# haowenz/chromap

Measured on NVIDIA H100. Metric: paired-end reads mapped/sec (hg38-scale, 2x50bp), higher is better.
Workload: dtype u64

## Files before the change

chromap_b200/csrc/cta_pair_candidates.cuh:

```cuda
#pragma once
#include "pipeline_kernels.cuh"

__device__ __forceinline__ int cta_scan_add(int v, int *s_warp, int *total) {
  const int NT = blockDim.x;
  const int lane = threadIdx.x & 31, wid = threadIdx.x >> 5;
  int x = v;
#pragma unroll
  for (int o = 1; o < 32; o <<= 1) { const int y = __shfl_up_sync(0xffffffffu, x, o); if (lane >= o) x += y; }
  if (lane == 31) s_warp[wid] = x;
  __syncthreads();
  int base = 0, tot = 0;
for (int i = 0; i < (NT >> 5); ++i) { const int w = s_warp[i]; if (i < wid) base += w; tot += w; }
  __syncthreads();
  *total = tot;
  return base + x - v;
}
__device__ __forceinline__ int cta_scan_max(int v, int *s_warp, int *total) {
  const int NT = blockDim.x;
  const int lane = threadIdx.x & 31, wid = threadIdx.x >> 5;
  int x = v;
#pragma unroll
  for (int o = 1; o < 32; o <<= 1) { const int y = __shfl_up_sync(0xffffffffu, x, o); if (lane >= o) x = max(x, y); }
  if (lane == 31) s_warp[wid] = x;
  __syncthreads();
// ... 96 lines not shown
  for (int i = a0; i < a1; ++i) {
    const u8 f = f1[i];
    if (f == 1) run = max(run, (int)c1[i]);
    else if (f == 2) { if ((int)c1[i] >= run) ++nq1; else f1[i] = 0; }
  }
  int run2 = max(6, pm2), nq2 = 0;
  for (int j = b0; j < b1; ++j) {
    const u8 f = f2[j];
    if (f == 1) run2 = max(run2, (int)c2[j]);
    else if (f == 2) { if ((int)c2[j] >= run2) ++nq2; else f2[j] = 0; }
  }
  int totq;
  const int pq = cta_scan_add(nq1 | (nq2 << 16), s_warp, &totq);
  int paired_before = pp & 0xffff, qual_before = pq & 0xffff;
  for (int i = a0; i < a1; ++i) {
    const u8 f = f1[i];
    if (f == 1) { const int at = paired_before + min(qual_before, 5); o1p[at] = p1[i]; o1c[at] = c1[i]; ++paired_before; }
    else if (f == 2) { if (qual_before < 5) { const int at = paired_before + qual_before; o1p[at] = p1[i]; o1c[at] = c1[i]; } ++qual_before; }
  }
  paired_before = pp >> 16; qual_before = pq >> 16;
  for (int j = b0; j < b1; ++j) {
    const u8 f = f2[j];
    if (f == 1) { const int at = paired_before + min(qual_before, 5); o2p[at] = p2[j]; o2c[at] = c2[j]; ++paired_before; }
    else if (f == 2) { if (qual_before < 5) { const int at = paired_before + qual_before; o2p[at] = p2[j]; o2c[at] = c2[j]; } ++qual_before; }
  }
  *na = (tot & 0xffff) + min(totq & 0xffff, 5);
  *nb = (tot >> 16) + min(totq >> 16, 5);
  __syncthreads();
}

#define RESCUE_MAXWIN 300
#define PC_CTA_NT_MAX 512
struct RescueShared {
  u64 win_lo[RESCUE_MAXWIN], win_hi[RESCUE_MAXWIN];
  int i[8];
  int warp[PC_CTA_NT_MAX / 32];
};
__device__ inline int cta_rescue(const DevParams &P, const DevIndex &ix, int strand, u32 range, int n_mm, const u64 *mmv, const u32 *mmp,
                                 const u64 *mate_pos, const u8 *mate_cnt, int n_mate, u32 *rep_len, u64 *hits, int cap, u64 *sm, int sm_cap,
                                 RescueShared &R, int *nh_out) {
  const int NT = blockDim.x;
  const int tid = threadIdx.x, lane = tid & 31, wid = tid >> 5;
  int mx = 0;
  for (int i = tid; i < n_mate; i += NT) mx = max(mx, (int)mate_cnt[i]);
  int max_cnt;
  cta_scan_max(mx, R.warp, &max_cnt);
  int nb = 0;
  for (int i = tid; i < n_mate; i += NT) nb += mate_cnt[i] == max_cnt;
  int n_best;
  cta_scan_add(nb, R.warp, &n_best);
  *nh_out = 0;
  if (n_best >= 300 || n_mate > P.f0 || (max_cnt <= P.min_seeds && n_best >= 200)) return -max_cnt;
  if (tid == 0) {
    int nw = 0;
    for (int i = 0; i < n_mate; ++i) {
      if (mate_cnt[i] != max_cnt) continue;
      const u64 lo = mate_pos[i] < range ? 0 : mate_pos[i] - range, hi = mate_pos[i] + range;
      if (nw > 0 && !(R.win_hi[nw - 1] < lo)) R.win_hi[nw - 1] = hi;
      else { R.win_lo[nw] = lo; R.win_hi[nw] = hi; ++nw; }
    }
    R.i[2] = nw;
    R.i[3] = 0;
  }
  __syncthreads();
  const int nw = R.i[2];
  for (int mi = tid; mi < n_mm; mi += NT) {
    if ((mmp[mi] >> 30) != 1) continue;
    bool same;
    const u64 cp = hit_to_candidate(P.k, mmv[mi], (mmp[mi] & 0x3FFFFFFFu) >> 1, mmp[mi] & 1u, &same);
    if ((same && strand == 0) || (!same && strand == 1)) { const int at = atomicAdd(&R.i[3], 1); if (at < cap) hits[at] = cp; }
  }
  for (int mi = wid; mi < n_mm; mi += (NT >> 5)) {
    if ((mmp[mi] >> 30) != 2) continue;
    const u64 val = mmv[mi];
    const u64 *O = ix.occ + (u32)(val >> 32);
    const int n = (int)(u32)val;
    const u32 rpos = (mmp[mi] & 0x3FFFFFFFu) >> 1, rstrand = mmp[mi] & 1u;
    int c_lb = 0, c_e = 0, c_s = 0;
    for (int b0 = 0; b0 < nw; b0 += 32) {
      const int b = b0 + lane;
      const bool live = b < nw;
      int lb = 0, eq = 0, ub = 0;
      if (live) {
        const u64 lo = R.win_lo[b], hi = R.win_hi[b];
        int a = 0, z = n;
        while (a < z) { const int m = (a + z) >> 1; if ((__ldg(&O[m]) >> 1) < lo) a = m + 1; else z = m; }
        lb = a;
        eq = (lb < n && (__ldg(&O[lb]) >> 1) == lo) ? 1 : 0;
        int step = 1, lo_i = lb + eq, hi_i = lb + eq;
        while (hi_i < n && (__ldg(&O[hi_i]) >> 1) <= hi) { lo_i = hi_i + 1; hi_i += step; step <<= 1; }
        if (hi_i > n) hi_i = n;
        while (lo_i < hi_i) { const int m = (lo_i + hi_i) >> 1; if ((__ldg(&O[m]) >> 1) <= hi) lo_i = m + 1; else hi_i = m; }
        ub = lo_i;
      }
      int p_lb = __shfl_up_sync(0xffffffffu, lb, 1), p_e = __shfl_up_sync(0xffffffffu, eq, 1);
      if (lane == 0) { p_lb = c_lb; p_e = c_e; }
      u32 f = 2u;
      if (live) {
        int o0, o1;
        if (b == 0) o0 = o1 = rescue_replay(0, n, lb, lb + eq);
        else {
          o1 = rescue_replay(p_lb, n, lb, lb + eq);
          o0 = p_e ? o1 : rescue_replay(max(p_lb - 1, 0), n, lb, lb + eq);
        }
        f = (o0 == lb ? 1u : 0u) | (o1 == lb ? 2u : 0u);
      }
#pragma unroll
      for (int o = 1; o < 32; o <<= 1) {
        const u32 g = __shfl_up_sync(0xffffffffu, f, o);
        if (lane >= o) f = (((f >> (g & 1u)) & 1u)) | (((f >> ((g >> 1) & 1u)) & 1u) << 1);
      }
      const int s_out = (int)((f >> c_s) & 1u);
      if (live) {
        const int first = lb - 1 + s_out, end = max(first, ub);
        for (int oi = first; oi < end; ++oi) {
          bool same;
          const u64 cp = hit_to_candidate(P.k, __ldg(&O[oi]), rpos, rstrand, &same);
          if ((same && strand == 0) || (!same && strand == 1)) { const int at = atomicAdd(&R.i[3], 1); if (at < cap) hits[at] = cp; }
        }
      }
      c_lb = __shfl_sync(0xffffffffu, lb, 31); c_e = __shfl_sync(0xffffffffu, eq, 31); c_s = __shfl_sync(0xffffffffu, s_out, 31);
    }
  }
  __syncthreads();
  const int nh = R.i[3];
  *nh_out = nh;
  if (tid == 0) {
    RepStats st = {0u, 0xFFFFFFFFu, 0};
    for (int mi = 0; mi < n_mm; ++mi)
      if ((mmp[mi] >> 30) == 2 && (u32)mmv[mi] >= (u32)P.f0) rep_update(P.k, P.w, (mmp[mi] & 0x3FFFFFFFu) >> 1, st);
    *rep_len = st.len;
  }
  __syncthreads();
  if (nh <= cap) cta_sort_keys(hits, nh, sm, sm_cap);
  return max_cnt;
}

__host__ __device__ inline size_t pair_candidates_cta_smem(int sm_cap, int lcap, int maxmm, int fcap) {
  return (size_t)sm_cap * 11 + (size_t)lcap * 4 * 9 + (size_t)maxmm * 12 + (size_t)fcap * 2 + 64;
}
__device__ inline void pair_candidates_cta_pair(const DevParams &P, const DevIndex &ix, const Scratch &S, Counters *ctr, int sm_cap, int lcap, int fcap,
                                                int slot, u64 *sm, RescueShared &RS) {
  const Caps c = S.caps;
  u8 *aux = (u8 *)(sm + sm_cap);
  u64 *s_lp = (u64 *)(aux + 3 * (size_t)sm_cap);
  u64 *s_mmv = s_lp + 4 * (size_t)lcap;
  u32 *s_mmp = (u32 *)(s_mmv + c.maxmm);
  u8 *s_lc = (u8 *)(s_mmp + c.maxmm);
  u8 *fl_a = s_lc + 4 * (size_t)lcap, *fl_b = fl_a + fcap;
  const int NT = blockDim.x, tid = threadIdx.x;
  PairMeta &pm = S.pmeta[slot];
  if (pm.status != ST_OK) return;
  ReadMeta *rm = S.rmeta + 2 * slot;
  auto CP = [&](int mate, int set, int strand) { return S.cand_pos + ((((size_t)(2 * slot + mate)) * 3 + set) * 2 + strand) * c.cc; };
  auto CC = [&](int mate, int set, int strand) { return S.cand_cnt + ((((size_t)(2 * slot + mate)) * 3 + set) * 2 + strand) * c.cc; };
  if (P.se) {
    const int a1 = rm[0].n_cand[0] + rm[0].n_cand[1];
    __syncthreads();
    if (tid == 0) { if (rm[0].n_mm == 0 || a1 == 0) pm.status = ST_DROP; else atomicAdd(&ctr->n_candidates, (u64)a1); }
    return;
  }
  if (rm[0].n_mm == 0 || rm[1].n_mm == 0) { __syncthreads(); if (tid == 0) pm.status = ST_DROP; return; }
  if (P.split) {
    const int a1 = rm[0].n_cand[0] + rm[0].n_cand[1], a2 = rm[1].n_cand[0] + rm[1].n_cand[1];
    __syncthreads();
    if (tid == 0) { if (!(a1 > 0 && a2 > 0)) pm.status = ST_DROP; else atomicAdd(&ctr->n_candidates, (u64)(a1 + a2)); }
    return;
  }
  int nq[4];
  const u64 *lp[4];
  const u8 *lc[4];
  const int n_mm2[2] = {rm[0].n_mm, rm[1].n_mm};
  auto stage = [&]() {
#pragma unroll
    for (int q = 0; q < 4; ++q) {
      nq[q] = rm[q >> 1].n_cand[q & 1];
      const u64 *gp = CP(q >> 1, 0, q & 1);
      const u8 *gc = CC(q >> 1, 0, q & 1);
      if (nq[q] <= lcap) {
        for (int i = tid; i < nq[q]; i += NT) { s_lp[q * lcap + i] = gp[i]; s_lc[q * lcap + i] = gc[i]; }
        lp[q] = s_lp + q * lcap; lc[q] = s_lc + q * lcap;
      } else { lp[q] = gp; lc[q] = gc; }
    }
    __syncthreads();
  };
  stage();
  bool need[2];
#pragma unroll
  for (int mate = 0; mate < 2; ++mate) {
    const u32 half = (u32)n_mm2[mate] / 2;
    int hit = 0;
#pragma unroll
    for (int s = 0; s < 2; ++s)
      for (int i = tid; i < nq[mate * 2 + s]; i += NT) hit |= lc[mate * 2 + s][i] >= half;
    need[mate] = !__syncthreads_or(hit);
  }
  const u32 range = 2u * (u32)P.max_insert;
  int ret = 0;
  for (int mate = 0; mate < 2; ++mate) {
    if (!need[mate]) continue;
    ReadMeta &me = rm[mate];
    const int n_mm = n_mm2[mate];
    const size_t sr = 2 * slot + mate;
    {
      const size_t mb0 = mm_base(S, slot, mate);
      const int ms = mm_stride(S);
      for (int i = tid; i < n_mm; i += NT) { s_mmv[i] = S.mm_val[mb0 + (size_t)i * ms]; s_mmp[i] = S.mm_pos[mb0 + (size_t)i * ms]; }
    }
    __syncthreads();
    u64 *hp = S.hits + (sr * 2 + 0) * c.hc, *hn = S.hits + (sr * 2 + 1) * c.hc;
    int pr = 0, nr = 0;
    bool ovf = false;
    const int o0 = (1 - mate) * 2;
    if (nq[o0] > 0) {
      int nh;
      pr = cta_rescue(P, ix, 1, range, n_mm, s_mmv, s_mmp, lp[o0], lc[o0], nq[o0], &me.rep_len, hn, c.hc, sm, sm_cap, RS, &nh);
      if (nh > c.hc) ovf = true;
      else {
        const int na = cta_cluster_par(P.e, 1, (u32)n_mm, hn, nh, CP(mate, 2, 1), CC(mate, 2, 1), c.cc, sm, sm_cap, aux, &RS.i[4]);
        if (na > c.cc) ovf = true; else if (tid == 0) me.n_aug[1] = na;
      }
    }
    if (!ovf && nq[o0 + 1] > 0) {
      int nh;
      nr = cta_rescue(P, ix, 0, range, n_mm, s_mmv, s_mmp, lp[o0 + 1], lc[o0 + 1], nq[o0 + 1], &me.rep_len, hp, c.hc, sm, sm_cap, RS, &nh);
      if (nh > c.hc) ovf = true;
      else {
        const int na = cta_cluster_par(P.e, 1, (u32)n_mm, hp, nh, CP(mate, 2, 0), CC(mate, 2, 0), c.cc, sm, sm_cap, aux, &RS.i[4]);
        if (na > c.cc) ovf = true; else if (tid == 0) me.n_aug[0] = na;
      }
    }
    if (ovf) { __syncthreads(); if (tid == 0) pm.status = ST_OVERFLOW; return; }
    if (((pr < 0 && nr > 0 && -pr >= nr) || (pr > 0 && nr < 0 && pr <= -nr)) && nq[mate * 2] + nq[mate * 2 + 1] == 0) ret = 1;
    __syncthreads();
  }
  bool merged = false;
  for (int q = 0; q < 4; ++q) {
    const int mate = q >> 1, s = q & 1;
    if (!need[mate]) continue;
    const int n2 = rm[mate].n_aug[s];
    if (n2 <= 0) continue;
    const int m = nq[q] + n2;
    u64 *mp;
    u8 *mc, *kf;
    if (m <= sm_cap) { mp = sm; mc = aux; kf = aux + sm_cap; }
    else { mp = CP(mate, 1, 0); mc = CC(mate, 1, 0); kf = fl_a; }
    const int n = (m > 2 * c.cc || (m > sm_cap && m > fcap)) ? c.cc + 1
                                                             : cta_merge_cands(P.e, lp[q], lc[q], nq[q], CP(mate, 2, s), CC(mate, 2, s), n2, mp, mc, kf,
                                                                               CP(mate, 0, s), CC(mate, 0, s), c.cc, RS.warp);
    if (n > c.cc) { __syncthreads(); if (tid == 0) pm.status = ST_OVERFLOW; return; }
    if (tid == 0) rm[mate].n_cand[s] = n;
    merged = true;
  }
  if (merged) { __syncthreads(); stage(); }
  int nc1 = nq[0] + nq[1], nc2 = nq[2] + nq[3];
  if (nc1 > 0 && nc2 > 0) {
#pragma unroll
    for (int q = 0; q < 4; ++q)
      if (nq[q] > lcap) {
        u64 *dst = CP(q >> 1, 1, q & 1);
        u8 *dstc = CC(q >> 1, 1, q & 1);
        for (int i = tid; i < nq[q]; i += NT) { dst[i] = lp[q][i]; dstc[i] = lc[q][i]; }
        lp[q] = dst; lc[q] = dstc;
      }
    __syncthreads();
    int a, b, a2, b2;
    cta_pe_filter((u32)P.max_insert, lp[0], lc[0], nq[0], lp[3], lc[3], nq[3], CP(0, 0, 0), CC(0, 0, 0), &a, CP(1, 0, 1), CC(1, 0, 1), &b, fl_a, fl_b, RS.warp);
    cta_pe_filter((u32)P.max_insert, lp[1], lc[1], nq[1], lp[2], lc[2], nq[2], CP(0, 0, 1), CC(0, 0, 1), &a2, CP(1, 0, 0), CC(1, 0, 0), &b2, fl_a, fl_b, RS.warp);
    if (tid == 0) {
      rm[0].n_cand[0] = a; rm[1].n_cand[1] = b; rm[0].n_cand[1] = a2; rm[1].n_cand[0] = b2;
    }
    nc1 = a + a2; nc2 = b + b2;
  }
  if (tid != 0) return;
  pm.sup = ret;
  if (!(nc1 > 0 && nc2 > 0)) { pm.status = ST_DROP; return; }
  atomicAdd(&ctr->n_candidates, (u64)(nc1 + nc2));
}

__global__ void __launch_bounds__(PC_CTA_NT_MAX) pair_candidates_cta_kernel(DevParams P, DevIndex ix, Scratch S, Counters *ctr, int sm_cap, int lcap, int fcap,
                                                                     const int *list, const int *list_count) {
  extern __shared__ u64 sm[];
  __shared__ RescueShared RS;
  if (!list) { pair_candidates_cta_pair(P, ix, S, ctr, sm_cap, lcap, fcap, (int)blockIdx.x, sm, RS); return; }
  const int n = *list_count;
  for (int b = blockIdx.x; b < n; b += gridDim.x) {
    pair_candidates_cta_pair(P, ix, S, ctr, sm_cap, lcap, fcap, list[b], sm, RS);
    __syncthreads();
  }
}
```

chromap_b200/csrc/cta_verify_pairing.cuh:

```cuda
#pragma once
#include "cta_pair_candidates.cuh"

__device__ __forceinline__ Tally tally_merge(const Tally &a, const Tally &b, int sentinel) {
  Tally r;
  r.min_err = min(a.min_err, b.min_err);
  r.n_best = (a.min_err == r.min_err ? a.n_best : 0) + (b.min_err == r.min_err ? b.n_best : 0);
  int s = sentinel;
  if (a.min_err > r.min_err && a.n_best > 0) s = min(s, a.min_err);
  if (b.min_err > r.min_err && b.n_best > 0) s = min(s, b.min_err);
  if (a.n_second_best > 0) s = min(s, a.second_min_err);
  if (b.n_second_best > 0) s = min(s, b.second_min_err);
  r.second_min_err = s;
  int n = 0;
  if (a.min_err == s && a.min_err > r.min_err) n += a.n_best;
  if (b.min_err == s && b.min_err > r.min_err) n += b.n_best;
  if (a.second_min_err == s) n += a.n_second_best;
  if (b.second_min_err == s) n += b.n_second_best;
  r.n_second_best = n;
  return r;
}
__device__ __forceinline__ Tally cta_tally_reduce(Tally t, int sentinel, Tally *s_t ) {
#pragma unroll
  for (int o = 16; o > 0; o >>= 1) {
    Tally u;
    u.min_err = __shfl_down_sync(0xffffffffu, t.min_err, o); u.second_min_err = __shfl_down_sync(0xffffffffu, t.second_min_err, o);
    u.n_best = __shfl_down_sync(0xffffffffu, t.n_best, o); u.n_second_best = __shfl_down_sync(0xffffffffu, t.n_second_best, o);
    t = tally_merge(t, u, sentinel);
  }
  if ((threadIdx.x & 31) == 0) s_t[threadIdx.x >> 5] = t;
  __syncthreads();
  Tally r = s_t[0];
  for (int i = 1; i < (int)(blockDim.x >> 5); ++i) r = tally_merge(r, s_t[i], sentinel);
  __syncthreads();
  return r;
}

#define VERIFY_NT_MAX 256
__global__ void __launch_bounds__(VERIFY_NT_MAX) verify_cta_kernel(DevParams P, DevRef R, DevBatch B, Scratch S, Counters *ctr, int sm_cap) {
  extern __shared__ u64 smk[];
  u8 *smt = (u8 *)(smk + sm_cap);
  u8 *s_fwd = smt + sm_cap, *s_neg = s_fwd + S.caps.maxmm;
  __shared__ int s_i[8];
  __shared__ int s_warp[VERIFY_NT_MAX / 32];
  __shared__ Tally s_t[VERIFY_NT_MAX / 32];
  const int NT = blockDim.x;
  const int sr = blockIdx.x, tid = threadIdx.x;
  const int slot = sr >> 1, mate = sr & 1;
  if (tid == 0) s_i[0] = S.pmeta[slot].status;
  __syncthreads();
  if (s_i[0] != ST_OK || (P.se && mate == 1)) return;
  const int pair = slot_pair(S, slot);
  ReadMeta &rm = S.rmeta[sr];
  const Caps c = S.caps;
  const u8 *read = read_ptr(B, pair, mate);
  const int L = rm.len, e = P.e;
  u64 *mp[2] = {S.map_pos + ((size_t)sr * 2 + 0) * c.mc, S.map_pos + ((size_t)sr * 2 + 1) * c.mc};
  short *me[2] = {S.map_err + ((size_t)sr * 2 + 0) * c.mc, S.map_err + ((size_t)sr * 2 + 1) * c.mc};
  u64 *cp[2] = {S.cand_pos + (((size_t)sr * 3 + 0) * 2 + 0) * c.cc, S.cand_pos + (((size_t)sr * 3 + 0) * 2 + 1) * c.cc};
  u8 *cc[2] = {S.cand_cnt + (((size_t)sr * 3 + 0) * 2 + 0) * c.cc, S.cand_cnt + (((size_t)sr * 3 + 0) * 2 + 1) * c.cc};
  const int nc[2] = {rm.n_cand[0], rm.n_cand[1]};
  if (nc[0] + nc[1] == 1) {
    const int strand = nc[0] == 1 ? 0 : 1;
    if (cc[strand][0] == rm.n_mm) {
      const u64 cpos = cp[strand][0];
      const u32 rid = (u32)(cpos >> 32);
      const u32 pos = strand == 0 ? (u32)cpos : (u32)cpos - (u32)L + 1u;
      const bool ok = valid_cand(e, R.len[rid], pos, (u32)L);
      __syncthreads();
      if (tid == 0) {
        rm.min_err = 0; rm.n_best = 1; rm.second_min_err = e + 1; rm.n_second_best = 0;
        if (ok) {
          mp[strand][0] = strand == 0 ? cpos + (u64)L - 1 : cpos;
          me[strand][0] = 0;
          rm.n_map[strand] = 1; rm.n_map[1 - strand] = 0;
        }
      }
      if (ok) return;
    }
  }
  for (int i = tid; i < L; i += NT) {
    const u32 b = base_code(read[i]);
    s_fwd[i] = (u8)b;
    s_neg[L - 1 - i] = (u8)(b < 4 ? 3u ^ b : 4u);
  }
  auto cless = [](u64 pa, u8 ca, u64 pb, u8 cb) { return ca != cb ? ca > cb : pa < pb; };
  cta_sort_pairs<u8>(cp[0], cc[0], nc[0], ~0ull, (u8)0, cless, smk, smt, sm_cap);
  cta_sort_pairs<u8>(cp[1], cc[1], nc[1], ~0ull, (u8)0, cless, smk, smt, sm_cap);
  unsigned short *vlist = (unsigned short *)smk;
  Tally t = {e + 1, e + 1, 0, 0};
  if (tid == 0 && nc[0] + nc[1] == 1 && cc[nc[0] == 1 ? 0 : 1][0] == rm.n_mm) { t.min_err = 0; t.n_best = 1; }
  u32 n_ver = 0;
  int nm[2] = {0, 0};
  for (int s = 0; s < 2; ++s) {
    const int n = nc[s];
    if (n == 0) continue;
    const int C = (n + NT - 1) / NT;
    const int r0 = min(n, tid * C), r1 = min(n, r0 + C);
    int mine = 0;
    for (int i = r0; i < r1; ++i) {
      const u64 cpos = cp[s][i];
      const u32 pos = s == 0 ? (u32)cpos : (u32)cpos - (u32)L + 1u;
      mine += valid_cand(e, R.len[(u32)(cpos >> 32)], pos, (u32)L) ? 1 : 0;
    }
    int nv;
    int at = cta_scan_add(mine, s_warp, &nv);
    for (int i = r0; i < r1; ++i) {
      const u64 cpos = cp[s][i];
      const u32 pos = s == 0 ? (u32)cpos : (u32)cpos - (u32)L + 1u;
      if (valid_cand(e, R.len[(u32)(cpos >> 32)], pos, (u32)L)) vlist[at++] = (unsigned short)i;
    }
    __syncthreads();
    const bool ruled = n >= P.lanes;
    const int n_full = nv / P.lanes * P.lanes;
    int stop = n;
    int free_until = 0;
    int out_base = 0;
    for (int v0 = 0; v0 < nv; v0 += NT) {
      if ((int)vlist[v0] >= stop && v0 >= free_until) break;
      const int v = v0 + tid;
      int err = e + 1, endp = 0, idx = 0;
      u64 cpos = 0;
      if (v + NT < nv) {
        const u64 nx = cp[s][vlist[v + NT]];
        const u32 npos = s == 0 ? (u32)nx : (u32)nx - (u32)L + 1u;
        prefetch_span(R.seq + R.off[(u32)(nx >> 32)] + npos - e, L + 2 * e);
      }
      if (v < nv) {
        idx = vlist[v];
        if (idx < stop || v < free_until) {
          cpos = cp[s][idx];
          const u32 rid = (u32)(cpos >> 32);
          const u32 pos = s == 0 ? (u32)cpos : (u32)cpos - (u32)L + 1u;
          const u8 *win = R.seq + R.off[rid] + pos - e;
          prefetch_span(win, L + 2 * e);
          const u8 *txt = s == 0 ? s_fwd : s_neg;
          err = banded_align(e, L, [&](int q) { return base_code(__ldg(win + q)); }, [&](int q) { return (u32)txt[q]; }, &endp);
          ++n_ver;
        } else idx = -1;
      } else idx = -1;
      if (ruled && stop == n && free_until == 0) {
        const bool failing = idx >= 0 && v < n_full && err > e;
        const unsigned fm = __ballot_sync(0xffffffffu, failing);
        if ((tid & 31) == 0) s_warp[tid >> 5] = (int)fm;
        __syncthreads();
        int first_fail = -1;
#pragma unroll
        for (int w = 0; w < (NT >> 5); ++w) if (first_fail < 0 && s_warp[w]) first_fail = v0 + w * 32 + __ffs((unsigned)s_warp[w]) - 1;
        if (first_fail >= 0) {
          const int g0 = first_fail / P.lanes * P.lanes, g1 = g0 + P.lanes;
          int last_fail = first_fail;
          for (int q = g0; q < g1; ++q) { const int w = (q - v0) >> 5, b = (q - v0) & 31; if ((s_warp[w] >> b) & 1) last_fail = q; }
          const int T = cc[s][vlist[last_fail]];
          int lo = (int)vlist[g1 - 1] + 1, hi = n;
          while (lo < hi) { const int m = (lo + hi) >> 1; if ((int)cc[s][m] < T) hi = m; else lo = m + 1; }
          stop = lo;
          free_until = g1;
        }
        __syncthreads();
      }
      const bool taken = idx >= 0 && (idx < stop || v < free_until);
      const bool pass = taken && err <= e;
      int tot;
      const int o = out_base + cta_scan_add(pass ? 1 : 0, s_warp, &tot);
      if (pass) {
        tally(t, err);
        if (o < c.mc) {
          mp[s][o] = s == 0 ? cpos - (u64)e + (u64)endp : cpos - (u64)L + 1 - (u64)e + (u64)endp;
          me[s][o] = (short)err;
        }
      }
      out_base += tot;
    }
    nm[s] = out_base;
    __syncthreads();
  }
  const Tally tt = cta_tally_reduce(t, e + 1, s_t);
  if (n_ver) agg_add(&ctr->n_verified, (u64)n_ver);
  if (tid != 0) return;
  if (nm[0] > c.mc || nm[1] > c.mc) { S.pmeta[slot].status = ST_OVERFLOW; return; }
  rm.n_map[0] = nm[0]; rm.n_map[1] = nm[1];
  rm.min_err = tt.min_err; rm.second_min_err = tt.second_min_err; rm.n_best = tt.n_best; rm.n_second_best = tt.n_second_best;
}

struct SweepWindow {
  u64 ins, ovl;
  u32 L1, L2;
  int s1;
  __device__ __forceinline__ bool before(u64 p1, u64 p2) const { return (s1 == 1 && p1 > p2 + ins - L2) || (s1 == 0 && p1 > p2 + L1 - ovl); }
  __device__ __forceinline__ bool within(u64 p1, u64 p2) const { return (s1 == 0 && p2 <= p1 + ins - L1) || (s1 == 1 && p2 <= p1 + L2 - ovl); }
  __device__ __forceinline__ void range(u64 p1, const u64 *p2, int n2, int *lo, int *hi) const {
    int a = 0, b = n2;
    while (a < b) { const int m = (a + b) >> 1; if (before(p1, p2[m])) a = m + 1; else b = m; }
    *lo = a;
    b = n2;
    while (a < b) { const int m = (a + b) >> 1; if (within(p1, p2[m])) a = m + 1; else b = m; }
    *hi = a;
  }
};

__global__ void __launch_bounds__(CTA_NT) pairing_cta_kernel(DevParams P, Scratch S, int *pair_nbest, int sm_cap) {
  extern __shared__ u64 smk[];
  short *smt = (short *)(smk + sm_cap);
  __shared__ Tally s_t[CTA_NT / 32];
  const int slot = blockIdx.x, tid = threadIdx.x;
  PairMeta &pm = S.pmeta[slot];
  const int pair = slot_pair(S, slot);
  if (pm.status != ST_OK) { if (tid == 0 && pm.status == ST_DROP) pair_nbest[pair] = 0; return; }
  const Caps c = S.caps;
  ReadMeta *rm = S.rmeta + 2 * slot;
  if (P.se) {
    __syncthreads();
    if (tid == 0) {
      if (rm[0].n_map[0] + rm[0].n_map[1] == 0) { pm.status = ST_DROP; pair_nbest[pair] = 0; }
      else {
        pm.min_sum = rm[0].min_err; pm.second_min_sum = rm[0].second_min_err; pm.n_best = rm[0].n_best; pm.n_second_best = rm[0].n_second_best;
        pair_nbest[pair] = rm[0].n_best;
      }
    }
    return;
  }
  if (rm[0].n_map[0] + rm[0].n_map[1] == 0 || rm[1].n_map[0] + rm[1].n_map[1] == 0) {
    __syncthreads();
    if (tid == 0) { pm.status = ST_DROP; pair_nbest[pair] = 0; }
    return;
  }
  auto mless = [](u64 pa, short ea, u64 pb, short eb) { return pa != pb ? pa < pb : ea < eb; };
  u64 *mp[2][2];
  short *me[2][2];
  for (int m = 0; m < 2; ++m)
    for (int s = 0; s < 2; ++s) {
      mp[m][s] = S.map_pos + ((size_t)(2 * slot + m) * 2 + s) * c.mc;
      me[m][s] = S.map_err + ((size_t)(2 * slot + m) * 2 + s) * c.mc;
      cta_sort_pairs<short>(mp[m][s], me[m][s], rm[m].n_map[s], ~0ull, (short)32767, mless, smk, smt, sm_cap);
    }
  const int sentinel = 2 * P.e + 1;
  Tally t = {sentinel, sentinel, 0, 0};
  SweepWindow W;
  W.ins = (u64)P.max_insert; W.ovl = (u64)(u32)P.min_read_len; W.L1 = (u32)rm[0].len; W.L2 = (u32)rm[1].len;
  for (int dir = 0; dir < 2; ++dir) {
    W.s1 = dir;
    const u64 *p1 = mp[0][dir], *p2 = mp[1][1 - dir];
    const short *e1 = me[0][dir], *e2 = me[1][1 - dir];
    const int n1 = rm[0].n_map[dir], n2 = rm[1].n_map[1 - dir];
    for (int i1 = tid; i1 < n1; i1 += CTA_NT) {
      int lo, hi;
      W.range(p1[i1], p2, n2, &lo, &hi);
      const int ea = e1[i1];
      for (int j = lo; j < hi; ++j) tally(t, ea + (int)e2[j]);
    }
  }
  const Tally tt = cta_tally_reduce(t, sentinel, s_t);
  if (tid != 0) return;
  pm.min_sum = tt.min_err; pm.second_min_sum = tt.second_min_err; pm.n_best = tt.n_best; pm.n_second_best = tt.n_second_best;
  pair_nbest[pair] = (tt.n_best > P.drop_rep) ? 0 : tt.n_best;
}

__global__ void __launch_bounds__(CTA_NT) emit_cta_kernel(DevParams P, DevRef R, DevBatch B, MapqTables T, Scratch S, const int *pair_sel, OutRecord *out,
                                                          int *out_n, Counters *ctr) {
  __shared__ int s_warp[CTA_NT / 32];
  __shared__ int s_i1[CMX_MAX_BEST], s_j[CMX_MAX_BEST], s_sel[CMX_MAX_BEST];
  const int slot = blockIdx.x, tid = threadIdx.x;
  PairMeta &pm = S.pmeta[slot];
  const int pair = slot_pair(S, slot);
  if (pm.status == ST_OVERFLOW) return;
  if (pm.status != ST_OK || pm.n_best > P.drop_rep || pm.n_best == 0) { if (tid == 0) out_n[pair] = 0; return; }
  const Caps c = S.caps;
  const ReadMeta *rm = S.rmeta + 2 * slot;
  const int mb = P.max_best;
  const int to_report = mb < pm.n_best ? mb : pm.n_best;
  if (tid < to_report) s_sel[tid] = pair_sel[(size_t)pair * mb + tid];
  __syncthreads();
  const int min_sum = pm.min_sum;
  SweepWindow W;
  W.ins = (u64)P.max_insert; W.ovl = (u64)(u32)P.min_read_len; W.L1 = (u32)rm[0].len; W.L2 = (u32)rm[1].len;
  int base = 0;
  for (int dir = 0; dir < 2; ++dir) {
    if (base > s_sel[to_report - 1]) break;
    W.s1 = dir;
    const u64 *p1 = S.map_pos + ((size_t)(2 * slot + 0) * 2 + dir) * c.mc, *p2 = S.map_pos + ((size_t)(2 * slot + 1) * 2 + (1 - dir)) * c.mc;
    const short *e1 = S.map_err + ((size_t)(2 * slot + 0) * 2 + dir) * c.mc, *e2 = S.map_err + ((size_t)(2 * slot + 1) * 2 + (1 - dir)) * c.mc;
    const int n1 = rm[0].n_map[dir], n2 = rm[1].n_map[1 - dir];
    const int C = (n1 + CTA_NT - 1) / CTA_NT;
    const int r0 = min(n1, tid * C), r1 = min(n1, r0 + C);
    int mine = 0;
    for (int i1 = r0; i1 < r1; ++i1) {
      int lo, hi;
      W.range(p1[i1], p2, n2, &lo, &hi);
      const int want = min_sum - (int)e1[i1];
      for (int j = lo; j < hi; ++j) mine += (int)e2[j] == want;
    }
    int total;
    int idx = base + cta_scan_add(mine, s_warp, &total);
    if (mine > 0) {
      int r = 0;
      while (r < to_report && s_sel[r] < idx) ++r;
      if (r < to_report && s_sel[r] < idx + mine) {
        for (int i1 = r0; i1 < r1 && r < to_report; ++i1) {
          int lo, hi;
          W.range(p1[i1], p2, n2, &lo, &hi);
          const int want = min_sum - (int)e1[i1];
          for (int j = lo; j < hi && r < to_report; ++j) {
            if ((int)e2[j] != want) continue;
            if (idx == s_sel[r]) { s_i1[r] = i1 | (dir << 30); s_j[r] = j; ++r; }
            ++idx;
          }
        }
      }
    }
    base += total;
  }
  __syncthreads();
  if (tid < to_report) {
    const int s1 = s_i1[tid] >> 30, i1 = s_i1[tid] & 0x3FFFFFFF, j = s_j[tid];
    const size_t b1 = ((size_t)(2 * slot + 0) * 2 + s1) * c.mc + i1, b2 = ((size_t)(2 * slot + 1) * 2 + (1 - s1)) * c.mc + j;
    out[(size_t)pair * mb + tid] = pe_record(P, R, B, T, pm, rm, pair, s1, S.map_pos[b1], S.map_err[b1], S.map_pos[b2], S.map_err[b2]);
  }
  if (tid != 0) return;
  out_n[pair] = to_report;
  pm.n_rec = to_report;
  atomicAdd(&ctr->n_mapped, 1ull);
  if (pm.n_best == 1) atomicAdd(&ctr->n_unique, 1ull);
}
```

chromap_b200/csrc/device_common.cuh:

```cuda
#pragma once
#include <cuda_runtime.h>
#include <stdint.h>

typedef unsigned long long u64;
typedef unsigned int u32;
typedef unsigned char u8;

#define CMX_W_MAX 64
#define CMX_MAX_BEST 8

struct DevParams {
  int e, min_seeds, f0, f1, max_best, max_insert, min_read_len, drop_rep, trim, k, w, lanes, split;
  int se;
};

struct Caps {
  int maxmm, hc, cc, mc;
};

enum { ST_OK = 0, ST_DROP = 1, ST_OVERFLOW = 2 };

struct ReadMeta {
  int len;
  int n_mm;
  int n_cand[2];
  int n_cand_gen[2];
  u32 rep_len;
  int mm_done;
  int n_map[2];
  int min_err, second_min_err, n_best, n_second_best;
  int n_aug[2];
};
static_assert(sizeof(ReadMeta) == 64, "ReadMeta: two sectors");

struct PairMeta {
  int status;
  int sup;
  int min_sum, second_min_sum, n_best, n_second_best;
  int n_rec;
  int pad;
};

struct DevIndex {
  const ulonglong2 *slots;
  u64 n_slots_mask;
  int shift;
  const u64 *occ;
  u32 n_occ;
  int k, w;
};
#define CMX_EMPTY_KEY 0xFFFFFFFFFFFFFFFFull

struct DevRef {
  const u8 *seq;
  const u64 *off;
  const u32 *len;
  u32 n_seq;
};

struct DevBatch {
  const u8 *seq1;
  const u32 *off1;
  const u8 *seq2;
  const u32 *off2;
  u32 n_pairs;
  u32 first_read_id;
  const u8 *bc_ok;
};

struct Scratch {
  Caps caps;
  int n_slots;
  const int *pair_list;
  int mm_il;
  ReadMeta *rmeta;
  PairMeta *pmeta;
  u64 *mm_hash;
  u64 *mm_val;
  u32 *mm_pos;
  u64 *hits;
  u64 *cand_pos;
  u8 *cand_cnt;
  u64 *map_pos;
  short *map_err;
  int *map_split;
};

#define SCRATCH_ARRAYS 11
inline size_t scratch_layout(const Caps &c, size_t slots, bool interleaved, size_t *off, size_t *size = nullptr) {
  const size_t R = 2 * slots;
  const size_t Rm = interleaved ? 2 * ((slots + 31) / 32 * 32) : R;
  const size_t sz[SCRATCH_ARRAYS] = {R * sizeof(ReadMeta), slots * sizeof(PairMeta),
                                     interleaved ? 0 : R * c.maxmm * 8,
                                     Rm * c.maxmm * 8, Rm * c.maxmm * 4, R * 2 * (size_t)c.hc * 8, R * 6 * (size_t)c.cc * 8, R * 6 * (size_t)c.cc,
                                     R * 2 * (size_t)c.mc * 8, R * 2 * (size_t)c.mc * 2, R * 2 * (size_t)c.mc * 4};
  size_t end = 0;
  for (int i = 0; i < SCRATCH_ARRAYS; ++i) {
    off[i] = end;
    if (size) size[i] = sz[i];
    end = (end + sz[i] + 255) / 256 * 256;
  }
  return end;
}
inline void scratch_bind(Scratch &S, char *const *a) {
  S.rmeta = (ReadMeta *)a[0]; S.pmeta = (PairMeta *)a[1];
  S.mm_hash = (u64 *)a[2]; S.mm_val = (u64 *)a[3]; S.mm_pos = (u32 *)a[4];
  S.hits = (u64 *)a[5]; S.cand_pos = (u64 *)a[6]; S.cand_cnt = (u8 *)a[7];
  S.map_pos = (u64 *)a[8]; S.map_err = (short *)a[9]; S.map_split = (int *)a[10];
}

__device__ __forceinline__ int slot_pair(const Scratch &S, int slot) { return S.pair_list ? S.pair_list[slot] : slot; }

__device__ __forceinline__ u32 base_code(u8 c) {
  const u32 u = (u32)c & 0xDFu;
  const u32 x = (u >> 1) & 3u;
  const u32 code = x ^ (x >> 1);
  const u32 in_row = ((u & 0xE0u) == 0x40u) ? 1u : 0u;
  const u32 is_base = in_row & ((0x0010008Au >> (u & 31u)) & 1u);
  return is_base ? code : 4u;
}

__device__ __forceinline__ u64 mix64(u64 key, u64 mask) {
  key = (~key + (key << 21)) & mask;
  key = key ^ key >> 24;
  key = ((key + (key << 3)) + (key << 8)) & mask;
  key = key ^ key >> 14;
  key = ((key + (key << 2)) + (key << 4)) & mask;
  key = key ^ key >> 28;
  key = (key + (key << 31)) & mask;
  return key;
}

__device__ __forceinline__ int index_lookup(const DevIndex &ix, u64 mm_hash, u64 *val, int *steps) {
  u64 s = (mm_hash * 0x9E3779B97F4A7C15ull) >> ix.shift;
  int n = 0;
  for (;;) {
    const ulonglong2 kv = __ldg(&ix.slots[s]);
    ++n;
    if (kv.x == CMX_EMPTY_KEY) { *steps = n; return 0; }
    if ((kv.x >> 1) == mm_hash) { *val = kv.y; *steps = n; return (kv.x & 1) ? 1 : 2; }
    s = (s + 1) & ix.n_slots_mask;
  }
}

__device__ __forceinline__ void prefetch_span(const void *p, int bytes) {
  const char *a = (const char *)((unsigned long long)p & ~127ull), *z = (const char *)p + bytes;
  for (; a < z; a += 128) asm volatile("prefetch.global.L1 [%0];" ::"l"(a));
}

__device__ __forceinline__ void prefetch_l2(const void *p) { asm volatile("prefetch.global.L2 [%0];" ::"l"(p)); }

__device__ __forceinline__ int occ_lower_bound(const u64 *O, int n, u64 lo) {
  int a = 0, z = n;
  while (z - a > 8) {
    const int q = (z - a) >> 2, m1 = a + q, m2 = m1 + q, m3 = m2 + q;
    const u64 v1 = __ldg(&O[m1]) >> 1, v2 = __ldg(&O[m2]) >> 1, v3 = __ldg(&O[m3]) >> 1;
    if (v3 < lo) a = m3 + 1;
    else if (v2 < lo) { a = m2 + 1; z = m3; }
    else if (v1 < lo) { a = m1 + 1; z = m2; }
    else z = m1;
  }
  int below = 0;
#pragma unroll
  for (int i = 0; i < 8; ++i) below += (a + i < z && (__ldg(&O[a + i]) >> 1) < lo) ? 1 : 0;
  return a + below;
}
__device__ __forceinline__ int rescue_replay(int l, int n, int lb, int ue) {
  int mid = 0, r = n - 1;
  while (l <= r) {
    mid = (l + r) / 2;
    if (mid < lb) l = mid + 1;
    else if (mid >= ue) r = mid - 1;
    else break;
  }
  return mid;
}

__device__ __forceinline__ u64 hit_to_candidate(int k, u64 ref_hit, u32 read_pos, u32 read_strand, bool *same) {
  const u32 rp = (u32)(ref_hit >> 1);
  const bool sm = ((u32)(ref_hit & 1)) == read_strand;
  const u32 start = sm ? rp - read_pos : rp + read_pos - (u32)k + 1u;
  *same = sm;
  return ((ref_hit >> 33) << 32) | start;
}

struct StridedU64 {
  u64 *base;
  int stride;
  __device__ __forceinline__ u64 &operator[](int i) const { return base[i * stride]; }
};

template <typename A>
__device__ inline void sort_u64(A a, int n) {
  if (n <= 24) {
    for (int i = 1; i < n; ++i) {
      const u64 v = a[i];
      int j = i - 1;
      while (j >= 0 && a[j] > v) { a[j + 1] = a[j]; --j; }
      a[j + 1] = v;
    }
    return;
  }
  for (int start = n / 2 - 1; start >= 0; --start) {
    int root = start;
    const u64 v = a[root];
    for (;;) {
      int child = 2 * root + 1;
      if (child >= n) break;
      if (child + 1 < n && a[child] < a[child + 1]) ++child;
      if (a[child] <= v) break;
      a[root] = a[child];
      root = child;
    }
    a[root] = v;
  }
  for (int end = n - 1; end > 0; --end) {
    const u64 v = a[end];
    a[end] = a[0];
    int root = 0;
    for (;;) {
      int child = 2 * root + 1;
      if (child >= end) break;
      if (child + 1 < end && a[child] < a[child + 1]) ++child;
      if (a[child] <= v) break;
      a[root] = a[child];
      root = child;
    }
    a[root] = v;
  }
}

template <typename T, typename Less>
__device__ inline void sort_pairs(u64 *k, T *t, int n, Less less) {
  if (n <= 24) {
    for (int i = 1; i < n; ++i) {
      const u64 kv = k[i];
      const T tv = t[i];
      int j = i - 1;
      while (j >= 0 && less(kv, tv, k[j], t[j])) { k[j + 1] = k[j]; t[j + 1] = t[j]; --j; }
      k[j + 1] = kv; t[j + 1] = tv;
    }
    return;
  }
  auto sift = [&](int root, int end, u64 kv, T tv) {
    for (;;) {
      int child = 2 * root + 1;
      if (child >= end) break;
      if (child + 1 < end && less(k[child], t[child], k[child + 1], t[child + 1])) ++child;
      if (!less(kv, tv, k[child], t[child])) break;
      k[root] = k[child]; t[root] = t[child];
      root = child;
    }
    k[root] = kv; t[root] = tv;
  };
  for (int start = n / 2 - 1; start >= 0; --start) sift(start, n, k[start], t[start]);
  for (int end = n - 1; end > 0; --end) {
    const u64 kv = k[end];
    const T tv = t[end];
    k[end] = k[0]; t[end] = t[0];
    sift(0, end, kv, tv);
  }
}
```

chromap_b200/csrc/minimizers.cuh:

```cuda
#pragma once
#include "device_common.cuh"

template <int K>
__device__ __forceinline__ u64 mix64_k(u64 key) {
  static_assert(K >= 17 && K <= 23, "mix64_k: 2k - 14 must not exceed 32");
  constexpr u64 mask = (((u64)1) << (2 * K)) - 1;
  constexpr u32 mask_hi = (u32)(mask >> 32);
  u32 lo = (u32)key, hi = (u32)(key >> 32);
  auto mul = [&](u32 c, u64 add) {
    const u64 p = (u64)lo * c + add;
    hi = ((u32)(p >> 32) + hi * c) & mask_hi;
    lo = (u32)p;
  };
  mul((1u << 21) - 1u, mask);
  lo ^= __funnelshift_r(lo, hi, 24);
  mul(265u, 0);
  lo ^= __funnelshift_r(lo, hi, 14);
  mul(21u, 0);
  lo ^= __funnelshift_r(lo, hi, 28);
  mul((1u << 31) + 1u, 0);
  return ((u64)hi << 32) | lo;
}

template <int KS, int WS, typename SeqF, typename EmitF>
// ... 66 lines not shown
#pragma unroll
      for (int j = 0; j < WS; ++j)
        if (base + j < len) step(base + j, j);
    }
  } else {
    int slot = 0;
    for (int pos = 0; pos < len; ++pos)
      if (step(pos, slot)) { if (++slot == w) slot = 0; }
  }
  if (best_h != ~0ull) EMIT(best_h, best_p);
}
template <int K, int W, typename SeqF, typename EmitF, typename RingT>
__device__ __forceinline__ void minimizer_scan_packed(SeqF SEQ, int len, EmitF EMIT, RingT ring) {
  static_assert((K & 1) && K >= 17 && K <= 21 && W >= 2, "minimizer_scan_packed: odd k, 2k + 20 <= 62");
  constexpr u64 mask = (((u64)1) << (2 * K)) - 1;
  constexpr int shift = 2 * (K - 1);
  constexpr u64 NONE = ~0ull;
  constexpr u32 PM = 0xFFFFFu;
  u64 fwd = 0, rev = 0;
#pragma unroll
  for (int i = 0; i < W; ++i) ring[i] = NONE;
  u64 best = NONE;
  int run = 0, slot = 0;
  auto emit_key = [&](u64 key) { EMIT(key >> 20, PM - ((u32)key & PM)); };
#pragma unroll 1
  for (int pos = 0; pos < len; ++pos) {
    const u32 b = base_code(SEQ(pos));
    u64 cur = NONE;
    if (b < 4) {
      fwd = ((fwd << 2) | b) & mask;
      rev = (rev >> 2) | (((u64)(3 ^ b)) << shift);
      ++run;
      if (run >= K) {
        const u64 hf = mix64_k<K>(fwd), hr = mix64_k<K>(rev);
        const u32 strand = hf < hr ? 0u : 1u;
        cur = (mix64_k<K>(strand ? hr : hf) << 20) | (u64)(PM - (((u32)pos << 1) | strand));
      }
    } else {
      run = 0;
    }
    if (run == W + K - 1 && best != NONE && (best >> 20) < (cur >> 20)) {
      for (int j = 1; j < W; ++j) {
        int q = slot + j; if (q >= W) q -= W;
        const u64 x = ring[q];
        if ((x >> 20) == (best >> 20) && x != best) emit_key(x);
      }
    }
    const u64 old = ring[slot];
    ring[slot] = cur;
    u64 m = cur;
#pragma unroll
    for (int q = 0; q < W; ++q) m = min(m, (u64)ring[q]);
    u64 out = NONE;
    bool left = false;
    if (cur <= best) {
      if (run >= W + K && best != NONE) out = best;
    } else if (old == best) {
      if (run >= W + K - 1) { out = best; left = m != NONE; }
    }
    if (out != NONE) emit_key(out);
    int same_hi = 0;
    if (left) {
#pragma unroll
      for (int q = 0; q < W; ++q) same_hi += (u32)((u64)ring[q] >> 32) == (u32)(m >> 32);
    }
    if (same_hi > 1) {
      for (int j = 1; j <= W; ++j) {
        int q = slot + j; if (q >= W) q -= W;
        const u64 x = ring[q];
        if ((x >> 20) == (m >> 20) && x != m) emit_key(x);
      }
    }
    best = m;
    if (++slot == W) slot = 0;
  }
  if (best != NONE) emit_key(best);
}
template <int K, int W, typename SeqF, typename EmitF>
__device__ __forceinline__ void minimizer_scan_packed(SeqF SEQ, int len, EmitF EMIT) {
  static_assert((K & 1) && K >= 17 && K <= 21 && W >= 2, "minimizer_scan_packed: odd k, 2k + 20 <= 62");
  constexpr u64 mask = (((u64)1) << (2 * K)) - 1;
  constexpr int shift = 2 * (K - 1);
  constexpr u64 NONE = ~0ull;
  constexpr u32 PM = 0xFFFFFu;
  u64 fwd = 0, rev = 0;
  u64 ring[W];
#pragma unroll
  for (int i = 0; i < W; ++i) ring[i] = NONE;
  u64 best = NONE;
  int run = 0;
  auto emit_key = [&](u64 key) { EMIT(key >> 20, PM - ((u32)key & PM)); };
#pragma unroll 1
  for (int pos = 0; pos < len; ++pos) {
    const u32 b = base_code(SEQ(pos));
    u64 cur = NONE;
    if (b < 4) {
      fwd = ((fwd << 2) | b) & mask;
      rev = (rev >> 2) | (((u64)(3 ^ b)) << shift);
      ++run;
      if (run >= K) {
        const u64 hf = mix64_k<K>(fwd), hr = mix64_k<K>(rev);
        const u32 strand = hf < hr ? 0u : 1u;
        cur = (mix64_k<K>(strand ? hr : hf) << 20) | (u64)(PM - (((u32)pos << 1) | strand));
      }
    } else {
      run = 0;
    }
    if (run == W + K - 1) {
      if (best != NONE && (best >> 20) < (cur >> 20)) {
#pragma unroll
        for (int q = 1; q < W; ++q) {
          const u64 x = ring[q];
          if ((x >> 20) == (best >> 20) && x != best) emit_key(x);
        }
      }
    }
    const u64 old = ring[0];
#pragma unroll
    for (int q = 0; q + 1 < W; ++q) ring[q] = ring[q + 1];
    ring[W - 1] = cur;
    u64 m = ring[0];
#pragma unroll
    for (int q = 1; q < W; ++q) m = min(m, ring[q]);
    u64 out = NONE;
    bool left = false;
    if (cur <= best) {
      if (run >= W + K && best != NONE) out = best;
    } else if (old == best) {
      if (run >= W + K - 1) { out = best; left = m != NONE; }
    }
    if (out != NONE) emit_key(out);
    int same_hi = 0;
    if (left) {
#pragma unroll
      for (int q = 0; q < W; ++q) same_hi += (u32)(ring[q] >> 32) == (u32)(m >> 32);
    }
    if (same_hi > 1) {
#pragma unroll
      for (int q = 0; q < W; ++q) {
        const u64 x = ring[q];
        if ((x >> 20) == (m >> 20) && x != m) emit_key(x);
      }
    }
    best = m;
  }
  if (best != NONE) emit_key(best);
}

template <typename SeqF, typename EmitF>
__device__ __forceinline__ void minimizer_scan_any(SeqF SEQ, int len, int k, int w, EmitF EMIT) {
  if (k == 17 && w == 7 && len < (1 << 18)) minimizer_scan_packed<17, 7>(SEQ, len, EMIT);
  else minimizer_scan<0, 0>(SEQ, len, k, w, EMIT);
}

__device__ __forceinline__ size_t mm_base(const Scratch &S, int slot, int mate) {
  return S.mm_il ? ((size_t)((slot >> 5) * 2 + mate) * S.caps.maxmm) * 32 + (slot & 31) : (size_t)(2 * slot + mate) * S.caps.maxmm;
}
__device__ __forceinline__ int mm_stride(const Scratch &S) { return S.mm_il ? 32 : 1; }
```

chromap_b200/csrc/pipeline_kernels.cuh:

```cuda
#pragma once
#include "device_common.cuh"
#include "minimizers.cuh"

struct MapqTables {
  const double *inv_log;
  const int *pen_thr;
};
inline void mapq_tables_fill(double *inv_log, int *pen_thr) {
  const int coef_frac = log(50);
  inv_log[0] = inv_log[1] = 0.0;
  for (int a = 2; a < 65536; ++a) inv_log[a] = coef_frac / log((unsigned short)a);
  for (int v = 0; v < 96; ++v) {
    long long lo = 0, hi = 0x7ffffffeLL;
    auto pen = [](long long n) { return (int)(4.343 * log((double)(n + 1)) + 0.499); };
    if (pen(hi) < v) { pen_thr[v] = 0x7fffffff; continue; }
    while (lo < hi) { const long long mid = (lo + hi) / 2; if (pen(mid) >= v) hi = mid; else lo = mid + 1; }
    pen_thr[v] = (int)lo;
  }
}

struct Counters {
  u64 n_minimizers, n_probe_steps, n_found, n_occ_reads, n_verified, n_candidates, n_mapped, n_unique, n_overflow;
  u64 n_bc_in_whitelist, n_bc_corrected;
  u64 ovf_reason[8];
};

__device__ __forceinline__ const u8 *read_ptr(const DevBatch &B, int pair, int mate) {
  return mate == 0 ? B.seq1 + B.off1[pair] : B.seq2 + B.off2[pair];
}
__device__ __forceinline__ int read_raw_len(const DevBatch &B, int pair, int mate) {
  return mate == 0 ? (int)(B.off1[pair + 1] - B.off1[pair]) : (int)(B.off2[pair + 1] - B.off2[pair]);
}
__device__ __forceinline__ u32 neg_code(const u8 *read, int L, int i) {
  const u32 c = base_code(read[L - 1 - i]);
  return c < 4 ? 3u ^ c : 4u;
}
__device__ __forceinline__ u8 code_char(u32 c) { return c == 0 ? 'A' : c == 1 ? 'C' : c == 2 ? 'G' : c == 3 ? 'T' : 'N'; }

#ifndef CMX_HOST_EMU
__device__ __forceinline__ void agg_add(u64 *addr, u64 v) {
  const unsigned m = __activemask();
  const unsigned s_ = __reduce_add_sync(m, (unsigned)v);
  if ((int)(threadIdx.x & 31) == __ffs(m) - 1) atomicAdd(addr, (u64)s_);
}
__device__ __forceinline__ int agg_append(int *count) {
  const unsigned m = __activemask();
  const int lane = threadIdx.x & 31, leader = __ffs(m) - 1;
  int base = 0;
  if (lane == leader) base = atomicAdd(count, __popc(m));
  base = __shfl_sync(m, base, leader);
  return base + __popc(m & ((1u << lane) - 1u));
}
#endif

__global__ void prep_kernel(DevParams P, DevBatch B, Scratch S) {
  const int slot = blockIdx.x * blockDim.x + threadIdx.x;
  if (slot >= S.n_slots) return;
  const int pair = slot_pair(S, slot);
  PairMeta pm;
  pm.status = ST_OK; pm.sup = 0; pm.min_sum = 0; pm.second_min_sum = 0; pm.n_best = 0; pm.n_second_best = 0; pm.n_rec = 0; pm.pad = 0;
  int len1 = read_raw_len(B, pair, 0), len2 = P.se ? 0 : read_raw_len(B, pair, 1);
  if (B.bc_ok && !B.bc_ok[pair]) pm.status = ST_DROP;
  else if (len1 < P.min_read_len || (!P.se && len2 < P.min_read_len)) pm.status = ST_DROP;
  else if (len1 > S.caps.maxmm || len2 > S.caps.maxmm) pm.status = ST_OVERFLOW;
  else if (P.trim && !P.se) {
    const u8 *raw1 = read_ptr(B, pair, 0), *raw2 = read_ptr(B, pair, 1);
    const bool swp = !(len1 <= len2);
    const u8 *r1 = swp ? raw2 : raw1;
    const u8 *r2 = swp ? raw1 : raw2;
    const int L1 = swp ? len2 : len1, L2 = swp ? len1 : len2;
    const int min_ovl = P.min_read_len, seed = min_ovl / 2;
    bool merged = false;
    for (int si = 0; si < 2 && !merged; ++si) {
      for (int sp = 0; sp + seed <= L2 && !merged; ++sp) {
        bool hit = true;
        for (int j = 0; j < seed; ++j)
          if (code_char(neg_code(r2, L2, sp + j)) != r1[si * seed + j]) { hit = false; break; }
        if (!hit) continue;
        if (!(sp >= si * seed) || !((int)(L2 - sp + seed * si) >= min_ovl)) continue;
        bool ok = true;
        int ne = 0;
        for (int i = 0; i < seed * si; ++i) {
          if (code_char(neg_code(r2, L2, sp - si * seed + i)) != r1[i]) ++ne;
          if (ne > 1) { ok = false; break; }
        }
        if (ok)
          for (int i = seed; i + sp < L2 && si * seed + i < L1; ++i) {
            if (code_char(neg_code(r2, L2, sp + i)) != r1[si * seed + i]) ++ne;
            if (ne > 1) { ok = false; break; }
          }
        if (!ok) continue;
        int ovl = L2 - sp + si * seed, off2 = 0;
        if (ovl > L1) { off2 = ovl - L1; ovl = L1; }
        const int t1 = swp ? ovl + off2 : ovl, t2 = swp ? ovl : ovl + off2;
        if (t1 < len1) len1 = t1;
        if (t2 < len2) len2 = t2;
        merged = true;
      }
    }
  }
  S.pmeta[slot] = pm;
  ReadMeta z;
  memset(&z, 0, sizeof(z));
  z.len = len1; S.rmeta[2 * slot] = z;
  z.len = len2; S.rmeta[2 * slot + 1] = z;
}

struct RepStats { u32 len, prev; int count; };
__device__ __forceinline__ void rep_update(int k, int w, u32 read_pos, RepStats &st) {
  if (st.prev > read_pos) st.len += k;
  else if (read_pos < st.prev + k + w - 1) st.len += read_pos - st.prev;
  else st.len += k;
  st.prev = read_pos;
  ++st.count;
}

template <typename A>
__device__ inline int cluster_hits(int e, int need, u32 n_mm, A hits, int nh, u64 *cpos, u8 *ccnt, int cap) {
  if (nh == 0) return 0;
  int n = 0, mcount = 1, eq = 1, best_eq = 1;
  u64 prev = hits[0], best = hits[0];
  u32 prev_rid = (u32)(prev >> 32), prev_pos = (u32)prev;
  for (int i = 1; i <= nh; ++i) {
    const u64 h = i < nh ? hits[i] : ~0ull;
    const u32 rid = (u32)(h >> 32), pos = (u32)h;
    if (rid != prev_rid || pos > prev_pos + (u32)e || ((u32)mcount >= n_mm && pos > (u32)best + (u32)e)) {
      if (mcount >= need) { if (n < cap) { cpos[n] = best; ccnt[n] = (u8)best_eq; } ++n; }
      mcount = 1; eq = 1; best_eq = 1; best = h;
    } else {
      if (h == best) { ++eq; ++best_eq; }
      else if (h == prev) { ++eq; if (eq > best_eq) { best = prev; best_eq = eq; } }
      else eq = 1;
      ++mcount;
    }
    prev = h; prev_rid = rid; prev_pos = pos;
  }
  return n;
}

#define CLUSTER_NT 128
__global__ void __launch_bounds__(CLUSTER_NT) cluster_kernel(DevParams P, DevIndex ix, Scratch S, Counters *ctr, int mode, int rows, int *list,
                                                             int *list_count) {
  extern __shared__ u64 sh_hits[];
  const int tid = blockIdx.x * CLUSTER_NT + threadIdx.x;
  int sr = tid;
  if (mode == 1) {
    if (tid >= *list_count) return;
    sr = list[tid];
  } else if (sr >= 2 * S.n_slots) return;
  const int slot = sr >> 1;
  if (S.pmeta[slot].status != ST_OK) return;
  ReadMeta &rm = S.rmeta[sr];
  const Caps c = S.caps;
  const int n_mm = rm.n_mm;
  if (n_mm == 0) return;
  const int ms = mm_stride(S);
  const u64 *mmv = S.mm_val + mm_base(S, slot, sr & 1);
  const u32 *mmp = S.mm_pos + mm_base(S, slot, sr & 1);
  long long cnt1 = 0, cnt2 = 0;
  RepStats st = {0u, 0xFFFFFFFFu, 0};
  for (int i = 0; i < n_mm; ++i) {
    const u32 kind = mmp[(size_t)i * ms] >> 30;
    if (kind == 1) { ++cnt1; ++cnt2; }
    else if (kind == 2) {
      const u64 v_ = mmv[(size_t)i * ms];
      const u32 n = (u32)v_;
      if (n < (u32)P.f1) prefetch_span(&ix.occ[(u32)(v_ >> 32)], (int)min(n, 64u) * 8);
      if (n < (u32)P.f0) cnt1 += n;
      if (n < (u32)P.f1) cnt2 += n;
      if (n >= (u32)P.f0) rep_update(P.k, P.w, (mmp[(size_t)i * ms] & 0x3FFFFFFFu) >> 1, st);
    }
  }
  const bool round2 = cnt1 == 0;
  const long long total = round2 ? cnt2 : cnt1;
  if (total > c.hc) { S.pmeta[slot].status = ST_OVERFLOW; atomicAdd(&ctr->ovf_reason[2], 1ull); return; }
  if (total > rows) { list[agg_append(list_count)] = sr; return; }
  const u32 max_freq = round2 ? (u32)P.f1 : (u32)P.f0;
  const StridedU64 hp = {sh_hits + threadIdx.x, CLUSTER_NT};
  const StridedU64 hn = {sh_hits + (size_t)(rows - 1) * CLUSTER_NT + threadIdx.x, -CLUSTER_NT};
  int np = 0, nn = 0;
  u32 occ_reads = 0;
  for (int i = 0; i < n_mm; ++i) {
    const u32 kind = mmp[(size_t)i * ms] >> 30;
    if (kind == 0) continue;
    const u32 rpos = (mmp[(size_t)i * ms] & 0x3FFFFFFFu) >> 1, rstrand = mmp[(size_t)i * ms] & 1u;
    const u64 val = mmv[(size_t)i * ms];
    bool same;
    if (kind == 1) {
      const u64 cp = hit_to_candidate(P.k, val, rpos, rstrand, &same);
      if (same) hp[np++] = cp; else hn[nn++] = cp;
      continue;
    }
    const u32 n = (u32)val, off = (u32)(val >> 32);
    if (n < max_freq) {
      for (u32 q = 0; q < n; ++q) {
        const u64 rh = __ldg(&ix.occ[off + q]);
        const u64 cp = hit_to_candidate(P.k, rh, rpos, rstrand, &same);
        if (same) hp[np++] = cp; else hn[nn++] = cp;
      }
      occ_reads += n;
    }
  }
  if (occ_reads) agg_add(&ctr->n_occ_reads, (u64)occ_reads);
  sort_u64(hp, np);
  sort_u64(hn, nn);
  rm.rep_len = st.len;
  int need = n_mm - st.count;
  need = need > 1 ? need : 1;
  need = need > P.min_seeds ? P.min_seeds : need;
  if (round2 && np > 0 && nn > 0) need = P.min_seeds;
  u64 *cp0 = S.cand_pos + (((size_t)sr * 3 + 0) * 2 + 0) * c.cc, *cp1 = cp0 + c.cc;
  u8 *cc0 = S.cand_cnt + (((size_t)sr * 3 + 0) * 2 + 0) * c.cc, *cc1 = cc0 + c.cc;
  const int nc0 = cluster_hits(P.e, need, (u32)n_mm, hp, np, cp0, cc0, c.cc);
  const int nc1 = cluster_hits(P.e, need, (u32)n_mm, hn, nn, cp1, cc1, c.cc);
  if (nc0 > c.cc || nc1 > c.cc) { S.pmeta[slot].status = ST_OVERFLOW; atomicAdd(&ctr->ovf_reason[3], 1ull); return; }
  rm.n_cand[0] = nc0; rm.n_cand[1] = nc1;
  rm.n_cand_gen[0] = nc0; rm.n_cand_gen[1] = nc1;
}

__device__ inline int rescue_hits(const DevParams &P, const DevIndex &ix, int strand, u32 range, int n_mm, const u64 *mmv,
                                  const u32 *mmp, int ms, const u64 *mate_pos, const u8 *mate_cnt, int n_mate, u32 *rep_len,
                                  u64 *hits, int cap, int *nh_out) {
  int max_cnt = 0, n_best = 0;
  for (int i = 0; i < n_mate; ++i) {
    const int cnt = mate_cnt[i];
    if (cnt > max_cnt) { max_cnt = cnt; n_best = 1; }
    else if (cnt == max_cnt) ++n_best;
  }
  *nh_out = 0;
  if (n_best >= 300 || n_mate > P.f0 || (max_cnt <= P.min_seeds && n_best >= 200)) return -max_cnt;
  int nh = 0;
  RepStats st = {0u, 0xFFFFFFFFu, 0};
  for (int mi = 0; mi < n_mm; ++mi) {
    const u32 kind = mmp[(size_t)mi * ms] >> 30;
    if (kind == 0) continue;
    const u32 rpos = (mmp[(size_t)mi * ms] & 0x3FFFFFFFu) >> 1, rstrand = mmp[(size_t)mi * ms] & 1u;
    const u64 val = mmv[(size_t)mi * ms];
    bool same;
    if (kind == 1) {
      const u64 cp = hit_to_candidate(P.k, val, rpos, rstrand, &same);
      if ((same && strand == 0) || (!same && strand == 1)) { if (nh < cap) hits[nh] = cp; ++nh; }
      continue;
    }
    const u32 off = (u32)(val >> 32), n = (u32)val;
    int prev_l = 0;
    int ci = 0;
    while (ci < n_mate) {
      while (ci < n_mate && mate_cnt[ci] != max_cnt) ++ci;
      if (ci >= n_mate) break;
      u64 lo = mate_pos[ci] < range ? 0 : mate_pos[ci] - range;
      u64 hi = mate_pos[ci] + range;
      ++ci;
      for (;;) {
        int cj = ci;
        while (cj < n_mate && mate_cnt[cj] != max_cnt) ++cj;
        if (cj >= n_mate) { ci = cj; break; }
        const u64 lo2 = mate_pos[cj] < range ? 0 : mate_pos[cj] - range;
        if (hi < lo2) { ci = cj; break; }
        hi = mate_pos[cj] + range;
        ci = cj + 1;
      }
      const int lbq = occ_lower_bound(ix.occ + off, (int)n, lo);
      const int eqq = (lbq < (int)n && (__ldg(&ix.occ[off + lbq]) >> 1) == lo) ? 1 : 0;
      const int mid = rescue_replay(prev_l, (int)n, lbq, lbq + eqq);
      prev_l = mid;
      for (u32 oi = (u32)mid; oi < n; ++oi) {
        const u64 rh = __ldg(&ix.occ[off + oi]);
        if ((rh >> 1) > hi) break;
        const u64 cp = hit_to_candidate(P.k, rh, rpos, rstrand, &same);
        if ((same && strand == 0) || (!same && strand == 1)) { if (nh < cap) hits[nh] = cp; ++nh; }
      }
    }
    if (n >= (u32)P.f0) rep_update(P.k, P.w, rpos, st);
  }
  *nh_out = nh;
  if (nh <= cap) sort_u64(hits, nh);
  *rep_len = st.len;
  return max_cnt;
}

__device__ inline int merge_cands(int e, u64 *p1, u8 *c1, int n1, const u64 *p2, const u8 *c2, int n2, u64 *po, u8 *co, int cap) {
  if (n1 == 0) {
    for (int i = 0; i < n2 && i < cap; ++i) { p1[i] = p2[i]; c1[i] = c2[i]; }
    return n2;
  }
  int i = 0, j = 0, n = 0;
  u64 last = 0;
#define FAR(p) (n == 0 || (p) > last + (u64)e)
#define PUSH(p, c) do { if (n < cap) { po[n] = (p); co[n] = (c); } last = (p); ++n; } while (0)
  while (i < n1 && j < n2) {
    if (p1[i] == p2[j]) { if (FAR(p1[i])) { if (c1[i] > c2[j]) PUSH(p1[i], c1[i]); else PUSH(p2[j], c2[j]); } ++i; ++j; }
    else if (p1[i] < p2[j]) { if (FAR(p1[i])) PUSH(p1[i], c1[i]); ++i; }
    else { if (FAR(p2[j])) PUSH(p2[j], c2[j]); ++j; }
  }
  for (; i < n1; ++i) if (FAR(p1[i])) PUSH(p1[i], c1[i]);
  for (; j < n2; ++j) if (FAR(p2[j])) PUSH(p2[j], c2[j]);
#undef FAR
#undef PUSH
  for (int t = 0; t < n && t < cap; ++t) { p1[t] = po[t]; c1[t] = co[t]; }
  return n;
}

__device__ inline void pe_filter_dir(u32 dist, const u64 *p1, const u8 *c1, int n1, const u64 *p2, const u8 *c2, int n2,
                                     u64 *f1p, u8 *f1c, int *nf1, u64 *f2p, u8 *f2c, int *nf2) {
  int i1 = 0, i2 = 0, prev_end = 0, a = 0, b = 0;
  int un1 = 0, un2 = 0, max1 = 6, max2 = 6;
  while (i1 < n1 && i2 < n2) {
    if (p1[i1] > p2[i2] + dist) {
      if (i2 >= prev_end && un2 < 5 && (p1[i1] >> 32) == (p2[i2] >> 32) && c2[i2] >= max2) { f2p[b] = p2[i2]; f2c[b] = c2[i2]; ++b; ++un2; }
      ++i2;
    } else if (p2[i2] > p1[i1] + dist) {
      if (un1 < 5 && (p1[i1] >> 32) == (p2[i2] >> 32) && c1[i1] >= max1) { f1p[a] = p1[i1]; f1c[a] = c1[i1]; ++a; ++un1; }
      ++i1;
    } else {
      f1p[a] = p1[i1]; f1c[a] = c1[i1]; ++a;
      if (c1[i1] > max1) max1 = c1[i1];
      int j = i2;
      while (j < n2 && p2[j] <= p1[i1] + dist) {
        if (j >= prev_end) { f2p[b] = p2[j]; f2c[b] = c2[j]; ++b; if (c2[j] > max2) max2 = c2[j]; }
        ++j;
      }
      prev_end = j;
      ++i1;
    }
  }
  *nf1 = a; *nf2 = b;
}

#define PC_SMALL 8
#define PC_RESCUE_HEAVY 48
__global__ void pair_candidates_kernel(DevParams P, DevIndex ix, Scratch S, Counters *ctr, int mode, int *list, int *list_count) {
  const int tid = blockIdx.x * blockDim.x + threadIdx.x;
  int slot = tid;
  if (mode == 1) {
    if (tid >= *list_count) return;
    slot = list[tid];
  } else if (slot >= S.n_slots) return;
  PairMeta &pm = S.pmeta[slot];
  if (pm.status != ST_OK) return;
  const Caps c = S.caps;
  ReadMeta *rm = S.rmeta + 2 * slot;
  auto CP = [&](int mate, int set, int strand) { return S.cand_pos + ((((size_t)(2 * slot + mate)) * 3 + set) * 2 + strand) * c.cc; };
  auto CC = [&](int mate, int set, int strand) { return S.cand_cnt + ((((size_t)(2 * slot + mate)) * 3 + set) * 2 + strand) * c.cc; };
  if (P.se) {
    if (mode != 0) return;
    const int a1 = rm[0].n_cand[0] + rm[0].n_cand[1];
    if (rm[0].n_mm == 0 || a1 == 0) { pm.status = ST_DROP; return; }
    agg_add(&ctr->n_candidates, (u64)a1);
    return;
  }
  if (P.split) {
    if (mode != 0) return;
    if (rm[0].n_mm == 0 || rm[1].n_mm == 0) { pm.status = ST_DROP; return; }
    const int a1 = rm[0].n_cand[0] + rm[0].n_cand[1], a2 = rm[1].n_cand[0] + rm[1].n_cand[1];
    if (!(a1 > 0 && a2 > 0)) { pm.status = ST_DROP; return; }
    agg_add(&ctr->n_candidates, (u64)(a1 + a2));
    return;
  }
  if (mode == 0) {
    if (rm[0].n_mm == 0 || rm[1].n_mm == 0) { pm.status = ST_DROP; return; }
    const int nq[4] = {rm[0].n_cand[0], rm[0].n_cand[1], rm[1].n_cand[0], rm[1].n_cand[1]};
    const bool small = nq[0] <= PC_SMALL && nq[1] <= PC_SMALL && nq[2] <= PC_SMALL && nq[3] <= PC_SMALL;
    u64 lp[4][PC_SMALL];
    u8 lc[4][PC_SMALL];
    if (small) {
#pragma unroll
      for (int q = 0; q < 4; ++q) {
        const u64 *src = CP(q >> 1, 0, q & 1);
        const u8 *srcc = CC(q >> 1, 0, q & 1);
        for (int i = 0; i < nq[q]; ++i) { lp[q][i] = src[i]; lc[q][i] = srcc[i]; }
      }
    }
    bool need = false;
    bool aug[2];
    for (int mate = 0; mate < 2; ++mate) {
      const u32 n_mm = rm[mate].n_mm;
      bool a = true;
      for (int s = 0; s < 2 && a; ++s) {
        const u8 *cc = small ? lc[mate * 2 + s] : CC(mate, 0, s);
        for (int i = 0; i < nq[mate * 2 + s]; ++i) if (cc[i] >= n_mm / 2) { a = false; break; }
      }
      aug[mate] = a;
      if (a && nq[(1 - mate) * 2] + nq[(1 - mate) * 2 + 1] > 0) need = true;
    }
    if (need) {
      u32 searches = 0;
      for (int mate = 0; mate < 2; ++mate) {
        if (!aug[mate]) continue;
        const u32 *mmp = S.mm_pos + mm_base(S, slot, mate);
        const int ms = mm_stride(S);
        u32 n_multi = 0;
        for (int i = 0; i < rm[mate].n_mm; ++i) n_multi += (mmp[(size_t)i * ms] >> 30) == 2;
        searches += n_multi * (u32)(nq[(1 - mate) * 2] + nq[(1 - mate) * 2 + 1]);
      }
      if (searches > PC_RESCUE_HEAVY) { pm.status = ST_OVERFLOW; agg_add(&ctr->ovf_reason[7], 1ull); return; }
      list[agg_append(list_count)] = slot;
      return;
    }
    if (small) {
      int nc1 = nq[0] + nq[1], nc2 = nq[2] + nq[3];
      if (nc1 > 0 && nc2 > 0) {
        int a, b;
        pe_filter_dir((u32)P.max_insert, lp[0], lc[0], nq[0], lp[3], lc[3], nq[3], CP(0, 0, 0), CC(0, 0, 0), &a, CP(1, 0, 1), CC(1, 0, 1), &b);
        rm[0].n_cand[0] = a; rm[1].n_cand[1] = b;
        nc1 = a; nc2 = b;
        pe_filter_dir((u32)P.max_insert, lp[1], lc[1], nq[1], lp[2], lc[2], nq[2], CP(0, 0, 1), CC(0, 0, 1), &a, CP(1, 0, 0), CC(1, 0, 0), &b);
        rm[0].n_cand[1] = a; rm[1].n_cand[0] = b;
        nc1 += a; nc2 += b;
      }
      if (!(nc1 > 0 && nc2 > 0)) { pm.status = ST_DROP; return; }
      agg_add(&ctr->n_candidates, (u64)(nc1 + nc2));
      return;
    }
  } else {
    int ret = 0;
    const u32 range = 2u * (u32)P.max_insert;
    bool ovf = false;
    for (int mate = 0; mate < 2; ++mate) {
      ReadMeta &me = rm[mate];
      const ReadMeta &ot = rm[1 - mate];
      const u32 n_mm = me.n_mm;
      bool a = true;
      for (int s = 0; s < 2 && a; ++s) {
        const u8 *cc = CC(mate, 0, s);
        for (int i = 0; i < me.n_cand[s]; ++i) if (cc[i] >= n_mm / 2) { a = false; break; }
      }
      if (!a) continue;
      const size_t sr = 2 * slot + mate;
      const u64 *mmv = S.mm_val + mm_base(S, slot, mate);
      const u32 *mmp = S.mm_pos + mm_base(S, slot, mate);
      const int ms = mm_stride(S);
      u64 *hp = S.hits + (sr * 2 + 0) * c.hc, *hn = S.hits + (sr * 2 + 1) * c.hc;
      int pr = 0, nr = 0;
      if (ot.n_cand[0] > 0) {
        int nh;
        pr = rescue_hits(P, ix, 1, range, n_mm, mmv, mmp, ms, CP(1 - mate, 0, 0), CC(1 - mate, 0, 0), ot.n_cand[0], &me.rep_len, hn, c.hc, &nh);
        if (nh > c.hc) { ovf = true; atomicAdd(&ctr->ovf_reason[4], 1ull); break; }
        const int na = cluster_hits(P.e, 1, n_mm, hn, nh, CP(mate, 2, 1), CC(mate, 2, 1), c.cc);
        if (na > c.cc) { ovf = true; atomicAdd(&ctr->ovf_reason[5], 1ull); break; }
        me.n_aug[1] = na;
      }
      if (ot.n_cand[1] > 0) {
        int nh;
        nr = rescue_hits(P, ix, 0, range, n_mm, mmv, mmp, ms, CP(1 - mate, 0, 1), CC(1 - mate, 0, 1), ot.n_cand[1], &me.rep_len, hp, c.hc, &nh);
        if (nh > c.hc) { ovf = true; atomicAdd(&ctr->ovf_reason[4], 1ull); break; }
        const int na = cluster_hits(P.e, 1, n_mm, hp, nh, CP(mate, 2, 0), CC(mate, 2, 0), c.cc);
        if (na > c.cc) { ovf = true; atomicAdd(&ctr->ovf_reason[5], 1ull); break; }
        me.n_aug[0] = na;
      }
      if (((pr < 0 && nr > 0 && -pr >= nr) || (pr > 0 && nr < 0 && pr <= -nr)) && me.n_cand[0] + me.n_cand[1] == 0) ret = 1;
    }
    if (ovf) { pm.status = ST_OVERFLOW; return; }
    for (int mate = 0; mate < 2 && !ovf; ++mate)
      for (int s = 0; s < 2; ++s) {
        ReadMeta &me = rm[mate];
        if (me.n_aug[s] > 0) {
          const int n = merge_cands(P.e, CP(mate, 0, s), CC(mate, 0, s), me.n_cand[s], CP(mate, 2, s), CC(mate, 2, s), me.n_aug[s],
                                    CP(mate, 1, s), CC(mate, 1, s), c.cc);
          if (n > c.cc) { ovf = true; atomicAdd(&ctr->ovf_reason[5], 1ull); break; }
          me.n_cand[s] = n;
        }
      }
    if (ovf) { pm.status = ST_OVERFLOW; return; }
    pm.sup = ret;
  }
  int nc1 = rm[0].n_cand[0] + rm[0].n_cand[1], nc2 = rm[1].n_cand[0] + rm[1].n_cand[1];
  if (nc1 > 0 && nc2 > 0) {
    int nbuf[2][2];
    for (int mate = 0; mate < 2; ++mate)
      for (int s = 0; s < 2; ++s) {
        const int n = rm[mate].n_cand[s];
        u64 *src = CP(mate, 0, s), *dst = CP(mate, 1, s);
        u8 *srcc = CC(mate, 0, s), *dstc = CC(mate, 1, s);
        for (int i = 0; i < n; ++i) { dst[i] = src[i]; dstc[i] = srcc[i]; }
        nbuf[mate][s] = n;
      }
    int a, b;
    pe_filter_dir((u32)P.max_insert, CP(0, 1, 0), CC(0, 1, 0), nbuf[0][0], CP(1, 1, 1), CC(1, 1, 1), nbuf[1][1],
                  CP(0, 0, 0), CC(0, 0, 0), &a, CP(1, 0, 1), CC(1, 0, 1), &b);
    rm[0].n_cand[0] = a; rm[1].n_cand[1] = b;
    pe_filter_dir((u32)P.max_insert, CP(0, 1, 1), CC(0, 1, 1), nbuf[0][1], CP(1, 1, 0), CC(1, 1, 0), nbuf[1][0],
                  CP(0, 0, 1), CC(0, 0, 1), &a, CP(1, 0, 0), CC(1, 0, 0), &b);
    rm[0].n_cand[1] = a; rm[1].n_cand[0] = b;
    nc1 = rm[0].n_cand[0] + rm[0].n_cand[1];
    nc2 = rm[1].n_cand[0] + rm[1].n_cand[1];
  }
  if (!(nc1 > 0 && nc2 > 0)) { pm.status = ST_DROP; return; }
  agg_add(&ctr->n_candidates, (u64)(nc1 + nc2));
}

struct PatPlanes { u32 p0, p1, p2; };
__device__ __forceinline__ void planes_or(PatPlanes &w, u32 code, u32 bit) {
  w.p0 |= (0u - (code & 1u)) & bit;
  w.p1 |= (0u - ((code >> 1) & 1u)) & bit;
  w.p2 |= (0u - (code >> 2)) & bit;
}
__device__ __forceinline__ u32 planes_match(const PatPlanes &w, u32 code, u32 band_mask) {
  return ~((w.p0 ^ (0u - (code & 1u))) | (w.p1 ^ (0u - ((code >> 1) & 1u))) | (w.p2 ^ (0u - (code >> 2)))) & band_mask;
}
__device__ __forceinline__ void planes_shift(PatPlanes &w) { w.p0 >>= 1; w.p1 >>= 1; w.p2 >>= 1; }

template <typename PatF, typename TxtF>
__device__ __forceinline__ int banded_align(int e, int L, PatF PAT, TxtF TXT, int *end_pos) {
  PatPlanes W = {0u, 0u, 0u};
  for (int i = 0; i < 2 * e; ++i) planes_or(W, PAT(i), 1u << i);
  const u32 hi = 1u << (2 * e), band = (hi << 1) - 1u;
  u32 VP = 0, VN = 0;
  int err = 0;
  u32 pat_n = L > 0 ? PAT(2 * e) : 0u, txt_n = L > 0 ? TXT(0) : 0u;
  for (int i = 0; i < L; ++i) {
    const u32 pat = pat_n, txt = txt_n;
    if (i + 1 < L) { pat_n = PAT(i + 1 + 2 * e); txt_n = TXT(i + 1); }
    planes_or(W, pat, hi);
    u32 X = VN | planes_match(W, txt, band);
    const u32 D0 = ((VP + (X & VP)) ^ VP) | X;
    const u32 HN = VP & D0;
    const u32 HP = VN | ~(VP | D0);
    X = D0 >> 1;
    VN = X & HP;
    VP = HN | ~(X | HP);
    err += 1 - (int)(D0 & 1u);
    if (err > 3 * e) return e + 1;
    planes_shift(W);
  }
  int best = err;
  *end_pos = L - 1;
  for (int i = 0; i < 2 * e; ++i) {
    err += (int)((VP >> i) & 1u);
    err -= (int)((VN >> i) & 1u);
    if (err < best || (err == best && i + 1 == e)) { best = err; *end_pos = L + i; }
  }
  return best;
}

__device__ __forceinline__ bool valid_cand(int e, u32 ref_len, u32 pos, u32 L) {
  return !(pos < (u32)e || pos >= ref_len || pos + L + (u32)e >= ref_len);
}

struct Tally { int min_err, second_min_err, n_best, n_second_best; };
__device__ __forceinline__ void tally(Tally &t, int err) {
  if (err < t.min_err) { t.second_min_err = t.min_err; t.n_second_best = t.n_best; t.min_err = err; t.n_best = 1; }
  else if (err == t.min_err) t.n_best++;
  else if (err == t.second_min_err) t.n_second_best++;
  else if (err < t.second_min_err) { t.n_second_best = 1; t.second_min_err = err; }
}

__global__ void verify_kernel(DevParams P, DevRef R, DevBatch B, Scratch S, Counters *ctr, int mode, int *list, int *list_count) {
  const int tid = blockIdx.x * blockDim.x + threadIdx.x;
  int sr = tid;
  if (mode == 1) {
    if (tid >= *list_count) return;
    sr = list[tid];
  } else if (sr >= 2 * S.n_slots) return;
  const int slot = sr >> 1, mate = sr & 1;
  if (S.pmeta[slot].status != ST_OK || (P.se && mate == 1)) return;
  const int pair = slot_pair(S, slot);
  ReadMeta &rm = S.rmeta[sr];
  const Caps c = S.caps;
  const u8 *read = read_ptr(B, pair, mate);
  const int L = rm.len, e = P.e;
  Tally t = {e + 1, e + 1, 0, 0};
  u64 *mp[2] = {S.map_pos + ((size_t)sr * 2 + 0) * c.mc, S.map_pos + ((size_t)sr * 2 + 1) * c.mc};
  short *me[2] = {S.map_err + ((size_t)sr * 2 + 0) * c.mc, S.map_err + ((size_t)sr * 2 + 1) * c.mc};
  int nm[2] = {0, 0};
  u64 *cp[2] = {S.cand_pos + (((size_t)sr * 3 + 0) * 2 + 0) * c.cc, S.cand_pos + (((size_t)sr * 3 + 0) * 2 + 1) * c.cc};
  u8 *cc[2] = {S.cand_cnt + (((size_t)sr * 3 + 0) * 2 + 0) * c.cc, S.cand_cnt + (((size_t)sr * 3 + 0) * 2 + 1) * c.cc};
  const int nc[2] = {rm.n_cand[0], rm.n_cand[1]};
  bool done = false;
  if (mode == 0 && nc[0] + nc[1] == 1) {
    int n_all = 0, idx = 0, strand = 0;
    for (int i = 0; i < nc[0]; ++i) if (cc[0][i] == rm.n_mm) { idx = i; ++n_all; }
    for (int i = 0; i < nc[1]; ++i) if (cc[1][i] == rm.n_mm) { idx = i; strand = 1; ++n_all; }
    if (n_all == 1) {
      t.min_err = 0; t.n_best = 1; t.n_second_best = 0;
      const u64 cpos = cp[strand][idx];
      const u32 rid = (u32)(cpos >> 32);
      const u32 pos = strand == 0 ? (u32)cpos : (u32)cpos - (u32)L + 1u;
      if (valid_cand(e, R.len[rid], pos, (u32)L)) {
        mp[strand][0] = strand == 0 ? cpos + (u64)L - 1 : cpos;
        me[strand][0] = 0;
        nm[strand] = 1;
        done = true;
      }
    }
  }
  u64 n_verified = 0;
  if (mode == 0 && !done && nc[0] + nc[1] > 0) { list[agg_append(list_count)] = sr; return; }
  if (!done && nc[0] + nc[1] > 0) {
    auto cless = [](u64 pa, u8 ca, u64 pb, u8 cb) { return ca != cb ? ca > cb : pa < pb; };
    sort_pairs<u8>(cp[0], cc[0], nc[0], cless);
    sort_pairs<u8>(cp[1], cc[1], nc[1], cless);
    extern __shared__ u8 v_codes[];
    const int NTB = blockDim.x;
    u8 *c_fwd = v_codes + threadIdx.x, *c_neg = v_codes + (size_t)c.maxmm * NTB + threadIdx.x;
    for (int i = 0; i < L; ++i) {
      const u32 b = base_code(read[i]);
      c_fwd[(size_t)i * NTB] = (u8)b;
      c_neg[(size_t)(L - 1 - i) * NTB] = (u8)(b < 4 ? 3u ^ b : 4u);
    }
    for (int s = 0; s < 2; ++s) {
      const u8 *txt = s == 0 ? c_fwd : c_neg;
      auto run_one = [&](u64 cpos) -> bool {
        const u32 rid = (u32)(cpos >> 32);
        const u32 pos = s == 0 ? (u32)cpos : (u32)cpos - (u32)L + 1u;
        const u8 *win = R.seq + R.off[rid] + pos - e;
        prefetch_span(win, L + 2 * e);
        int endp = 0;
        const int err = banded_align(e, L, [&](int i) { return base_code(__ldg(win + i)); }, [&](int i) { return (u32)txt[(size_t)i * NTB]; }, &endp);
        ++n_verified;
        if (err > e) return true;
        tally(t, err);
        if (nm[s] < c.mc) {
          mp[s][nm[s]] = s == 0 ? cpos - (u64)e + (u64)endp : cpos - (u64)L + 1 - (u64)e + (u64)endp;
          me[s][nm[s]] = (short)err;
        }
        ++nm[s];
        return false;
      };
      if (nc[s] < P.lanes) {
        for (int i = 0; i < nc[s]; ++i) {
          const u64 cpos = cp[s][i];
          const u32 pos = s == 0 ? (u32)cpos : (u32)cpos - (u32)L + 1u;
          if (!valid_cand(e, R.len[(u32)(cpos >> 32)], pos, (u32)L)) continue;
          run_one(cpos);
        }
        continue;
      }
      int group[8];
      int ng = 0;
      u32 threshold = 0;
      int ci = 0;
      while (ci < nc[s]) {
        if (cc[s][ci] < threshold) break;
        const u64 cpos = cp[s][ci];
        const u32 pos = s == 0 ? (u32)cpos : (u32)cpos - (u32)L + 1u;
        if (!valid_cand(e, R.len[(u32)(cpos >> 32)], pos, (u32)L)) { ++ci; continue; }
        group[ng++] = ci; ++ci;
        if (ng < P.lanes) continue;
        for (int g = 0; g < ng; ++g) if (run_one(cp[s][group[g]])) threshold = cc[s][group[g]];
        ng = 0;
      }
      for (int g = 0; g < ng; ++g) run_one(cp[s][group[g]]);
    }
  }
  if (nm[0] > c.mc || nm[1] > c.mc) { S.pmeta[slot].status = ST_OVERFLOW; atomicAdd(&ctr->ovf_reason[6], 1ull); return; }
  rm.n_map[0] = nm[0]; rm.n_map[1] = nm[1];
  rm.min_err = t.min_err; rm.second_min_err = t.second_min_err; rm.n_best = t.n_best; rm.n_second_best = t.n_second_best;
  if (n_verified) agg_add(&ctr->n_verified, n_verified);
}

template <typename Visit>
__device__ __forceinline__ void pair_sweep(const DevParams &P, int s1, u32 L1, u32 L2, const u64 *p1, const short *e1, int n1,
                                           const u64 *p2, const short *e2, int n2, Visit VISIT) {
  int i1 = 0, i2 = 0;
  const u64 ins = (u64)P.max_insert, ovl = (u64)(u32)P.min_read_len;
  while (i1 < n1 && i2 < n2) {
    if ((s1 == 1 && p1[i1] > p2[i2] + ins - L2) || (s1 == 0 && p1[i1] > p2[i2] + L1 - ovl)) ++i2;
    else if ((s1 == 0 && p2[i2] > p1[i1] + ins - L1) || (s1 == 1 && p2[i2] > p1[i1] + L2 - ovl)) ++i1;
    else {
      int j = i2;
      while (j < n2 && ((s1 == 0 && p2[j] <= p1[i1] + ins - L1) || (s1 == 1 && p2[j] <= p1[i1] + L2 - ovl))) {
        VISIT(i1, j, (int)e1[i1] + (int)e2[j]);
        ++j;
      }
      ++i1;
    }
  }
}
template <typename Visit>
__device__ __forceinline__ void pair_sweep_until(const DevParams &P, int s1, u32 L1, u32 L2, const u64 *p1, const short *e1, int n1,
                                                 const u64 *p2, const short *e2, int n2, Visit VISIT) {
  int i1 = 0, i2 = 0;
  const u64 ins = (u64)P.max_insert, ovl = (u64)(u32)P.min_read_len;
  while (i1 < n1 && i2 < n2) {
    if ((s1 == 1 && p1[i1] > p2[i2] + ins - L2) || (s1 == 0 && p1[i1] > p2[i2] + L1 - ovl)) ++i2;
    else if ((s1 == 0 && p2[i2] > p1[i1] + ins - L1) || (s1 == 1 && p2[i2] > p1[i1] + L2 - ovl)) ++i1;
    else {
      int j = i2;
      while (j < n2 && ((s1 == 0 && p2[j] <= p1[i1] + ins - L1) || (s1 == 1 && p2[j] <= p1[i1] + L2 - ovl))) {
        if (VISIT(i1, j, (int)e1[i1] + (int)e2[j])) return;
        ++j;
      }
      ++i1;
    }
  }
}

__global__ void pairing_kernel(DevParams P, Scratch S, int *pair_nbest) {
  const int slot = blockIdx.x * blockDim.x + threadIdx.x;
  if (slot >= S.n_slots) return;
  PairMeta &pm = S.pmeta[slot];
  const int pair = slot_pair(S, slot);
  if (pm.status != ST_OK) { if (pm.status == ST_DROP) pair_nbest[pair] = 0; return; }
  const Caps c = S.caps;
  ReadMeta *rm = S.rmeta + 2 * slot;
  if (P.se) {
    if (rm[0].n_map[0] + rm[0].n_map[1] == 0) { pm.status = ST_DROP; pair_nbest[pair] = 0; return; }
    pm.min_sum = rm[0].min_err; pm.second_min_sum = rm[0].second_min_err; pm.n_best = rm[0].n_best; pm.n_second_best = rm[0].n_second_best;
    pair_nbest[pair] = rm[0].n_best;
    return;
  }
  if (rm[0].n_map[0] + rm[0].n_map[1] == 0 || rm[1].n_map[0] + rm[1].n_map[1] == 0) { pm.status = ST_DROP; pair_nbest[pair] = 0; return; }
  auto mless = [](u64 pa, short ea, u64 pb, short eb) { return pa != pb ? pa < pb : ea < eb; };
  u64 *mp[2][2];
  short *me[2][2];
  for (int m = 0; m < 2; ++m)
    for (int s = 0; s < 2; ++s) {
      mp[m][s] = S.map_pos + ((size_t)(2 * slot + m) * 2 + s) * c.mc;
      me[m][s] = S.map_err + ((size_t)(2 * slot + m) * 2 + s) * c.mc;
      sort_pairs<short>(mp[m][s], me[m][s], rm[m].n_map[s], mless);
    }
  int min_sum = 2 * P.e + 1, second = 2 * P.e + 1, n_best = 0, n_second = 0;
  auto visit = [&](int, int, int sum) {
    if (sum < min_sum) { second = min_sum; n_second = n_best; min_sum = sum; n_best = 1; }
    else if (sum == min_sum) n_best++;
    else if (sum == second) n_second++;
    else if (sum < second) { second = sum; n_second = 1; }
  };
  pair_sweep(P, 0, (u32)rm[0].len, (u32)rm[1].len, mp[0][0], me[0][0], rm[0].n_map[0], mp[1][1], me[1][1], rm[1].n_map[1], visit);
  pair_sweep(P, 1, (u32)rm[0].len, (u32)rm[1].len, mp[0][1], me[0][1], rm[0].n_map[1], mp[1][0], me[1][0], rm[1].n_map[0], visit);
  pm.min_sum = min_sum; pm.second_min_sum = second; pm.n_best = n_best; pm.n_second_best = n_second;
  pair_nbest[pair] = (n_best > P.drop_rep) ? 0 : n_best;
}

#define MT_N 624
struct WarpMt {
  u32 *mt;
  u32 *out;
  int pos;
};
__device__ __forceinline__ u32 mt_mix(u32 a, u32 b, u32 c) {
  const u32 y = (a & 0x80000000u) | (b & 0x7fffffffu);
  return c ^ (y >> 1) ^ ((y & 1u) ? 0x9908b0dfu : 0u);
}
__device__ __forceinline__ void mt_regen(WarpMt &g, int lane) {
  u32 *mt = g.mt;
  u32 v[8];
  int n = 0;
  for (int i = lane; i < 227; i += 32) v[n++] = mt_mix(mt[i], mt[i + 1], mt[i + 397]);
  __syncwarp();
  n = 0;
  for (int i = lane; i < 227; i += 32) mt[i] = v[n++];
  __syncwarp();
  n = 0;
  for (int i = 227 + lane; i < 454; i += 32) v[n++] = mt_mix(mt[i], mt[i + 1], mt[i - 227]);
  __syncwarp();
  n = 0;
  for (int i = 227 + lane; i < 454; i += 32) mt[i] = v[n++];
  __syncwarp();
  n = 0;
  for (int i = 454 + lane; i < 623; i += 32) v[n++] = mt_mix(mt[i], mt[i + 1], mt[i - 227]);
  __syncwarp();
  n = 0;
  for (int i = 454 + lane; i < 623; i += 32) mt[i] = v[n++];
  __syncwarp();
  if (lane == 0) mt[623] = mt_mix(mt[623], mt[0], mt[396]);
  __syncwarp();
  for (int i = lane; i < MT_N; i += 32) {
    u32 y = mt[i];
    y ^= y >> 11; y ^= (y << 7) & 0x9d2c5680u; y ^= (y << 15) & 0xefc60000u; y ^= y >> 18;
    g.out[i] = y;
  }
  __syncwarp();
  g.pos = 0;
}
__device__ __forceinline__ u32 mt_next(WarpMt &g, int lane) {
  if (g.pos >= MT_N) mt_regen(g, lane);
  return g.out[g.pos++];
}
__device__ __forceinline__ u32 uniform_0_hi(WarpMt &g, int lane, u32 hi) {
  const u32 range = hi + 1u;
  u64 product = (u64)mt_next(g, lane) * (u64)range;
  u32 low = (u32)product;
  if (low < range) {
    const u32 threshold = (0u - range) % range;
    while (low < threshold) { product = (u64)mt_next(g, lane) * (u64)range; low = (u32)product; }
  }
  return (u32)(product >> 32);
}

__global__ void __launch_bounds__(128) select_kernel(DevParams P, int n_chunks, const int *chunk_start, const int *pair_nbest, int *pair_sel,
                                                     const u32 *mt_init) {
  __shared__ u32 s_mt[4][MT_N], s_out[4][MT_N];
  const int ch = (blockIdx.x * blockDim.x + threadIdx.x) >> 5;
  const int lane = threadIdx.x & 31, wid = threadIdx.x >> 5;
  if (ch >= n_chunks) return;
  WarpMt g;
  g.mt = s_mt[wid]; g.out = s_out[wid]; g.pos = MT_N;
  bool seeded = false;
  const int mb = P.max_best;
  const int p0 = chunk_start[ch], p1 = chunk_start[ch + 1];
  for (int base = p0; base < p1; base += 32) {
    const int pair = base + lane;
    int nb = 0;
    if (pair < p1) {
      nb = pair_nbest[pair];
      int *sel = pair_sel + (size_t)pair * mb;
      for (int j = 0; j < mb; ++j) sel[j] = j;
    }
    unsigned m = __ballot_sync(0xffffffffu, nb > mb);
    __syncwarp();
    while (m) {
      const int l = __ffs(m) - 1;
      m &= m - 1;
      const int nbl = __shfl_sync(0xffffffffu, nb, l);
      if (!seeded || P.se) {
        __syncwarp();
        for (int i = lane; i < MT_N; i += 32) g.mt[i] = mt_init[i];
        __syncwarp();
        g.pos = MT_N;
        seeded = true;
      }
      int *sel = pair_sel + (size_t)(base + l) * mb;
      int i = mb;
      while (i < nbl) {
        if (g.pos >= MT_N) mt_regen(g, lane);
        const int cnt = min(min(32, nbl - i), MT_N - g.pos);
        u64 product = 0;
        bool slow = false;
        if (lane < cnt) {
          const u32 range = (u32)(i + lane) + 1u;
          product = (u64)g.out[g.pos + lane] * (u64)range;
          slow = (u32)product < range;
        }
        const unsigned sm_ = __ballot_sync(0xffffffffu, slow);
        const int ok = sm_ ? __ffs(sm_) - 1 : cnt;
        const int j = (int)(product >> 32);
        unsigned hit = __ballot_sync(0xffffffffu, lane < ok && j < mb);
        while (hit) {
          const int t = __ffs(hit) - 1;
          hit &= hit - 1;
          const int jt = __shfl_sync(0xffffffffu, j, t);
          if (lane == 0) sel[jt] = i + t;
        }
        i += ok; g.pos += ok;
        if (ok < cnt) {
          const int jj = (int)uniform_0_hi(g, lane, (u32)i);
          if (jj < mb && lane == 0) sel[jj] = i;
          ++i;
        }
        __syncwarp();
      }
      if (lane == 0) {
        for (int a = 1; a < mb; ++a) {
          const int v = sel[a];
          int b = a - 1;
          while (b >= 0 && sel[b] > v) { sel[b + 1] = sel[b]; --b; }
          sel[b + 1] = v;
        }
      }
      __syncwarp();
    }
  }
}

template <typename PatC, typename TxtC>
__device__ __forceinline__ int banded_traceback_dp(int e, int min_err, int L, PatC PATC, TxtC TXTC) {
  PatPlanes W = {0u, 0u, 0u};
  for (int i = 0; i < 2 * e; ++i) planes_or(W, base_code(PATC(L - 1 + 2 * e - i)), 1u << i);
  const u32 hi = 1u << (2 * e), band = (hi << 1) - 1u;
  u32 VP = 0, VN = 0;
  int err = 0;
  for (int i = 0; i < L; ++i) {
    planes_or(W, base_code(PATC(L - 1 - i)), hi);
    u32 X = VN | planes_match(W, base_code(TXTC(L - 1 - i)), band);
    const u32 D0 = ((VP + (X & VP)) ^ VP) | X;
    const u32 HN = VP & D0;
    const u32 HP = VN | ~(VP | D0);
    X = D0 >> 1;
    VN = X & HP;
    VP = HN | ~(X | HP);
    err += 1 - (int)(D0 & 1u);
    planes_shift(W);
  }
  int start = 2 * e;
  for (int i = 0; i < 2 * e; ++i) {
    err += (int)((VP >> i) & 1u);
    err -= (int)((VN >> i) & 1u);
    if (err == min_err) { start = 2 * e - (1 + i); if (i + 1 == e) return start; }
  }
  return start;
}
template <typename PatC, typename TxtC>
__device__ __forceinline__ int banded_traceback(int e, int min_err, int L, PatC PATC, TxtC TXTC) {
  if (min_err == 0) return e;
  int ham = 0;
  for (int i = 0; i < L; ++i) if (PATC(i + e) != TXTC(i)) ++ham;
  if (ham == min_err) return e;
  return banded_traceback_dp(e, min_err, L, PATC, TXTC);
}

__device__ __forceinline__ double xmul(double a, double b) { return __dmul_rn(a, b); }
__device__ __forceinline__ double xadd(double a, double b) { return __dadd_rn(a, b); }
__device__ __forceinline__ double xsub(double a, double b) { return __dadd_rn(a, -b); }
__device__ __forceinline__ double xdiv(double a, double b) { return __ddiv_rn(a, b); }

__device__ __forceinline__ int second_best_penalty(const MapqTables &T, int n) {
  int v = 0;
  while (v + 1 < 96 && T.pen_thr[v + 1] <= n) ++v;
  return v;
}
__device__ __forceinline__ double rep_scale(double ident, double frac) {
  if (ident <= 0.95) return xsub(1.0, __dsqrt_rn(frac));
  if (ident <= 0.97) return xsub(1.0, frac);
  if (ident >= 0.999) return xsub(1.0, xmul(xmul(xmul(frac, frac), frac), frac));
  return xsub(1.0, xmul(frac, frac));
}
__device__ inline u8 mapq_se(const MapqTables &T, int num_errors, unsigned short aln_len, int read_len, int max_diff, const ReadMeta &rm) {
  const int coef_len = 50;
  aln_len = (unsigned short)((int)aln_len > read_len ? (int)aln_len : read_len);
  const double ident = xsub(1.0, xdiv((double)num_errors, (double)aln_len));
  int mapq = 0;
  int second = rm.second_min_err;
  if (rm.n_best > 1) {
  } else {
    if (second > num_errors + max_diff) second = num_errors + max_diff;
    double tmp = (int)aln_len < coef_len ? 1.0 : T.inv_log[aln_len];
    tmp = xmul(tmp, xmul(ident, ident));
    const double v = xadd(xmul(xmul(xmul(5 * 6.02, (double)(second - num_errors)), tmp), tmp), 0.499);
    mapq = (int)v;
  }
  if (rm.n_second_best > 0) mapq -= second_best_penalty(T, rm.n_second_best);
  if (mapq > 60) mapq = 60;
  if (mapq < 0) mapq = 0;
  if (rm.rep_len > 0) {
    double frac = xdiv((double)rm.rep_len, (double)read_len);
    if (rm.rep_len >= (u32)read_len) frac = 0.999;
    mapq = (int)xadd(xmul((double)mapq, rep_scale(ident, frac)), 0.499);
  }
  return (u8)mapq;
}
__device__ inline u8 mapq_pe(const MapqTables &T, int e1, int e2, unsigned short al1, unsigned short al2, int L1, int L2, int force,
                             const PairMeta &pm, const ReadMeta *rm) {
  u8 pe = 0;
  const int unpaired = rm[0].min_err + rm[1].min_err + 3;
  if (pm.n_best <= 1) {
    const int adj = pm.second_min_sum < unpaired ? pm.second_min_sum : unpaired;
    pe = (u8)(int)xadd(xdiv(xmul(5 * 6.02, (double)(adj - pm.min_sum)), 1.0), .499);
    if (pm.n_second_best > 0) pe = (u8)((int)pe - second_best_penalty(T, pm.n_second_best));
    if (pe > 60) pe = 60;
    const int rep = (int)(rm[0].rep_len + rm[1].rep_len);
    if (rep > 0) {
      const double total = (double)(L1 + L2);
      double frac = xdiv((double)rep, total);
      if ((double)rep >= total) frac = 0.999;
      const double id1 = xsub(1.0, xdiv((double)e1, (double)(L1 > (int)al1 ? L1 : (int)al1)));
      const double id2 = xsub(1.0, xdiv((double)e2, (double)(L2 > (int)al2 ? L2 : (int)al2)));
      const double ident = id1 < id2 ? id1 : id2;
      pe = (u8)xadd(xmul((double)pe, rep_scale(ident, frac)), 0.499);
    }
  }
  u8 q1 = mapq_se(T, e1, al1, L1, 2, rm[0]);
  u8 q2 = mapq_se(T, e2, al2, L2, 2, rm[1]);
  {
    const double a = xadd((double)q1, xmul((double)pe, 0.65));
    q1 = q1 > pe ? q1 : ((double)pe < a ? pe : (u8)a);
    const double b = xadd((double)q2, xmul((double)pe, 0.65));
    q2 = q2 > pe ? q2 : ((double)pe < b ? pe : (u8)b);
  }
  q1 = (u8)xmul((double)q1, 1.2); if (q1 > 60) q1 = 60;
  q2 = (u8)xmul((double)q2, 1.2); if (q2 > 60) q2 = 60;
  u8 q = q1 < q2 ? q1 : q2;
  if (q < 60 && force >= 0 && force < q) q = (u8)force;
  return q;
}

struct OutRecord {
  u32 read_id, rid, fragment_start;
  unsigned short fragment_length;
  u8 mapq, direction, is_unique, num_dups;
  unsigned short positive_alignment_length, negative_alignment_length;
};

__device__ __forceinline__ void mapping_span(const DevRef &R, int e, const u8 *r, int Lm, int s, u64 dpos, int derr, u32 *st, u32 *en) {
  const u32 rid = (u32)(dpos >> 32), rp = (u32)dpos;
  u32 vws = rp + 1u > (u32)(Lm + e) ? rp + 1u - (u32)Lm - (u32)e : 0u;
  if (rp + (u32)e >= R.len[rid]) vws = R.len[rid] - (u32)e - (u32)Lm;
  const u8 *win = R.seq + R.off[rid] + vws;
  if (derr != 0) { prefetch_span(win, Lm + 2 * e); prefetch_span(r, Lm); }
  int s0;
  if (s == 0) s0 = banded_traceback(e, derr, Lm, [&](int i) { return __ldg(win + i); }, [&](int i) { return r[i]; });
  else s0 = banded_traceback(e, derr, Lm, [&](int i) { return __ldg(win + i); }, [&](int i) { return code_char(neg_code(r, Lm, i)); });
  *st = vws + (u32)s0;
  *en = rp;
}
__device__ __forceinline__ OutRecord pe_record(const DevParams &P, const DevRef &R, const DevBatch &B, const MapqTables &T, const PairMeta &pm, const ReadMeta *rm,
                                               int pair, int s1, u64 pos1, int err1, u64 pos2, int err2) {
  const int L0 = rm[0].len, L1 = rm[1].len;
  u32 st1, en1, st2, en2;
  mapping_span(R, P.e, read_ptr(B, pair, 0), L0, s1, pos1, err1, &st1, &en1);
  mapping_span(R, P.e, read_ptr(B, pair, 1), L1, 1 - s1, pos2, err2, &st2, &en2);
  const unsigned short al1 = (unsigned short)(en1 - st1 + 1u), al2 = (unsigned short)(en2 - st2 + 1u);
  OutRecord o;
  o.read_id = B.first_read_id + (u32)pair;
  o.rid = (u32)(pos1 >> 32);
  o.fragment_start = s1 == 0 ? st1 : st2;
  o.fragment_length = (unsigned short)(s1 == 0 ? (int)(en2 - st1 + 1u) : (int)(en1 - st2 + 1u));
  o.mapq = mapq_pe(T, err1, err2, al1, al2, L0, L1, pm.sup != 0 ? 0 : -1, pm, rm);
  o.direction = s1 == 0 ? 1 : 0;
  o.is_unique = (pm.n_best == 1 || rm[0].n_best == 1 || rm[1].n_best == 1) ? 1 : 0;
  o.num_dups = 1;
  o.positive_alignment_length = s1 == 0 ? al1 : al2;
  o.negative_alignment_length = s1 == 1 ? al1 : al2;
  return o;
}

__global__ void emit_kernel(DevParams P, DevRef R, DevBatch B, MapqTables T, Scratch S, const int *pair_sel, OutRecord *out,
                            int *out_n, Counters *ctr, int4 *dp_list, int *dp_count) {
  const int slot = blockIdx.x * blockDim.x + threadIdx.x;
  const int lane = threadIdx.x & 31;
  const bool in_range = slot < S.n_slots;
  const int sl = in_range ? slot : 0;
  PairMeta &pm = S.pmeta[sl];
  const int pair = slot_pair(S, sl);
  const Caps c = S.caps;
  const ReadMeta *rm = S.rmeta + 2 * sl;
  const int mb = P.max_best, e = P.e;
  int reported = 0;
  int ch_i1[CMX_MAX_BEST], ch_j[CMX_MAX_BEST];
  bool live = in_range && pm.status != ST_OVERFLOW;
  if (live && (pm.status != ST_OK || pm.n_best > P.drop_rep || pm.n_best == 0)) { out_n[pair] = 0; live = false; }
  if (live) {
    const int to_report = mb < pm.n_best ? mb : pm.n_best;
    const int *sel = pair_sel + (size_t)pair * mb;
    int idx = 0;
    for (int dir = 0; dir < 2 && reported != to_report; ++dir) {
      const int s1 = dir, s2 = 1 - dir;
      const u64 *p1 = S.map_pos + ((size_t)(2 * slot + 0) * 2 + s1) * c.mc, *p2 = S.map_pos + ((size_t)(2 * slot + 1) * 2 + s2) * c.mc;
      const short *e1 = S.map_err + ((size_t)(2 * slot + 0) * 2 + s1) * c.mc, *e2 = S.map_err + ((size_t)(2 * slot + 1) * 2 + s2) * c.mc;
      pair_sweep_until(P, s1, (u32)rm[0].len, (u32)rm[1].len, p1, e1, rm[0].n_map[s1], p2, e2, rm[1].n_map[s2], [&](int i1, int j, int sum) -> bool {
        if (sum != pm.min_sum) return false;
        if (idx == sel[reported]) { ch_i1[reported] = i1 | (dir << 30); ch_j[reported] = j; ++reported; }
        ++idx;
        return reported == to_report;
      });
    }
  }
  const int L[2] = {live ? rm[0].len : 0, live ? rm[1].len : 0};
  const int max_rep = __reduce_max_sync(0xffffffffu, reported);
  for (int r = 0; r < max_rep; ++r) {
    const bool have = r < reported;
    int s1 = 0;
    u64 dpos[2] = {0, 0};
    int derr[2] = {0, 0};
    u32 vws[2] = {0, 0};
    const u8 *win[2] = {R.seq, R.seq};
    const u8 *rd[2] = {R.seq, R.seq};
    int s0[2] = {e, e};
    if (have) {
      s1 = ch_i1[r] >> 30;
      const size_t b1 = ((size_t)(2 * slot + 0) * 2 + s1) * c.mc + (ch_i1[r] & 0x3FFFFFFF), b2 = ((size_t)(2 * slot + 1) * 2 + (1 - s1)) * c.mc + ch_j[r];
      dpos[0] = S.map_pos[b1]; derr[0] = S.map_err[b1]; dpos[1] = S.map_pos[b2]; derr[1] = S.map_err[b2];
#pragma unroll
      for (int m = 0; m < 2; ++m) {
        const u32 rid = (u32)(dpos[m] >> 32), rp = (u32)dpos[m];
        u32 v = rp + 1u > (u32)(L[m] + e) ? rp + 1u - (u32)L[m] - (u32)e : 0u;
        if (rp + (u32)e >= R.len[rid]) v = R.len[rid] - (u32)e - (u32)L[m];
        vws[m] = v;
        win[m] = R.seq + R.off[rid] + v;
        rd[m] = read_ptr(B, pair, m);
      }
    }
    int ham[2] = {0, 0};
#pragma unroll
    for (int m = 0; m < 2; ++m) {
      unsigned todo = __ballot_sync(0xffffffffu, have && derr[m] > 0);
      while (todo) {
        int src[4], cnt[4];
#pragma unroll
        for (int t = 0; t < 4; ++t) {
          src[t] = todo ? __ffs(todo) - 1 : -1;
          if (todo) todo &= todo - 1;
          cnt[t] = 0;
        }
#pragma unroll
        for (int t = 0; t < 4; ++t) {
          if (src[t] < 0) continue;
          const u8 *w = (const u8 *)__shfl_sync(0xffffffffu, (unsigned long long)win[m], src[t]);
          const u8 *q = (const u8 *)__shfl_sync(0xffffffffu, (unsigned long long)rd[m], src[t]);
          const int Lm = __shfl_sync(0xffffffffu, L[m], src[t]);
          const int neg = __shfl_sync(0xffffffffu, m == 0 ? s1 : 1 - s1, src[t]);
          for (int i = lane; i < Lm; i += 32) {
            const u8 a = __ldg(w + i + e);
            const u8 c0 = neg ? q[Lm - 1 - i] : q[i];
            const u32 bc = base_code(c0);
            const u8 tch = neg ? code_char(bc < 4 ? 3u ^ bc : 4u) : c0;
            cnt[t] += a != tch;
          }
        }
#pragma unroll
        for (int t = 0; t < 4; ++t) {
          if (src[t] < 0) continue;
          const int c_ = __reduce_add_sync(0xffffffffu, cnt[t]);
          if (lane == src[t]) ham[m] = c_;
        }
      }
    }
    const bool deferred = have && ((derr[0] > 0 && ham[0] != derr[0]) || (derr[1] > 0 && ham[1] != derr[1]));
    if (deferred) dp_list[agg_append(dp_count)] = make_int4(slot, r, ch_i1[r], ch_j[r]);
    if (have && !deferred) {
      const u32 st1 = vws[0] + (u32)s0[0], en1 = (u32)dpos[0], st2 = vws[1] + (u32)s0[1], en2 = (u32)dpos[1];
      const unsigned short al1 = (unsigned short)(en1 - st1 + 1u), al2 = (unsigned short)(en2 - st2 + 1u);
      OutRecord o;
      o.read_id = B.first_read_id + (u32)pair;
      o.rid = (u32)(dpos[0] >> 32);
      o.fragment_start = s1 == 0 ? st1 : st2;
      o.fragment_length = (unsigned short)(s1 == 0 ? (int)(en2 - st1 + 1u) : (int)(en1 - st2 + 1u));
      o.mapq = mapq_pe(T, derr[0], derr[1], al1, al2, L[0], L[1], pm.sup != 0 ? 0 : -1, pm, rm);
      o.direction = s1 == 0 ? 1 : 0;
      o.is_unique = (pm.n_best == 1 || rm[0].n_best == 1 || rm[1].n_best == 1) ? 1 : 0;
      o.num_dups = 1;
      o.positive_alignment_length = s1 == 0 ? al1 : al2;
      o.negative_alignment_length = s1 == 1 ? al1 : al2;
      out[(size_t)pair * mb + r] = o;
    }
  }
  if (!live) return;
  out_n[pair] = reported;
  pm.n_rec = reported;
  if (reported > 0) { agg_add(&ctr->n_mapped, 1ull); if (pm.n_best == 1) agg_add(&ctr->n_unique, 1ull); }
}

__global__ void emit_dp_kernel(DevParams P, DevRef R, DevBatch B, MapqTables T, Scratch S, OutRecord *out, const int4 *dp_list, const int *dp_count) {
  const int t = blockIdx.x * blockDim.x + threadIdx.x;
  if (t >= *dp_count) return;
  const int4 q = dp_list[t];
  const int slot = q.x, r = q.y, s1 = q.z >> 30, i1 = q.z & 0x3FFFFFFF, j = q.w;
  const Caps c = S.caps;
  const size_t b1 = ((size_t)(2 * slot + 0) * 2 + s1) * c.mc + i1, b2 = ((size_t)(2 * slot + 1) * 2 + (1 - s1)) * c.mc + j;
  const int pair = slot_pair(S, slot);
  out[(size_t)pair * P.max_best + r] = pe_record(P, R, B, T, S.pmeta[slot], S.rmeta + 2 * slot, pair, s1, S.map_pos[b1], S.map_err[b1], S.map_pos[b2], S.map_err[b2]);
}

__global__ void emit_se_kernel(DevParams P, DevRef R, DevBatch B, MapqTables T, Scratch S, const int *pair_sel, OutRecord *out, int *out_n,
                               Counters *ctr) {
  const int slot = blockIdx.x * blockDim.x + threadIdx.x;
  if (slot >= S.n_slots) return;
  PairMeta &pm = S.pmeta[slot];
  const int pair = slot_pair(S, slot);
  if (pm.status == ST_OVERFLOW) return;
  if (pm.status != ST_OK || pm.n_best == 0) { out_n[pair] = 0; return; }
  const Caps c = S.caps;
  const ReadMeta &rm = S.rmeta[2 * slot];
  const int mb = P.max_best, e = P.e, L = rm.len;
  const int to_report = mb < rm.n_best ? mb : rm.n_best;
  const int *sel = pair_sel + (size_t)pair * mb;
  const u8 *r = read_ptr(B, pair, 0);
  int idx = 0, reported = 0;
  for (int s = 0; s < 2 && reported != to_report; ++s) {
    const u64 *mp = S.map_pos + ((size_t)(2 * slot) * 2 + s) * c.mc;
    const short *me = S.map_err + ((size_t)(2 * slot) * 2 + s) * c.mc;
    for (int mi = 0; mi < rm.n_map[s]; ++mi) {
      if ((int)me[mi] > rm.min_err) continue;
      if (idx == sel[reported]) {
        const u64 dpos = mp[mi];
        const u32 rid = (u32)(dpos >> 32), rp = (u32)dpos;
        u32 vws = rp + 1u > (u32)(L + e) ? rp + 1u - (u32)L - (u32)e : 0u;
        if (rp + (u32)e >= R.len[rid]) vws = R.len[rid] - (u32)e - (u32)L;
        const u8 *win = R.seq + R.off[rid] + vws;
        int s0;
        if (s == 0) s0 = banded_traceback(e, (int)me[mi], L, [&](int i) { return __ldg(win + i); }, [&](int i) { return r[i]; });
        else s0 = banded_traceback(e, (int)me[mi], L, [&](int i) { return __ldg(win + i); }, [&](int i) { return code_char(neg_code(r, L, i)); });
        const u32 st = vws + (u32)s0;
        const unsigned short al = (unsigned short)(rp - st + 1u);
        OutRecord o;
        o.read_id = B.first_read_id + (u32)pair;
        o.rid = rid;
        o.fragment_start = st;
        o.fragment_length = al;
        o.mapq = mapq_se(T, (int)me[mi], al, L, e, rm);
        o.direction = s == 0 ? 1 : 0;
        o.is_unique = rm.n_best == 1 ? 1 : 0;
        o.num_dups = 1;
        o.positive_alignment_length = 0;
        o.negative_alignment_length = 0;
        out[(size_t)pair * mb + reported] = o;
        if (++reported == to_report) break;
      }
      ++idx;
    }
  }
  out_n[pair] = reported;
  pm.n_rec = reported;
  if (reported > 0) { agg_add(&ctr->n_mapped, 1ull); if (rm.n_best == 1) agg_add(&ctr->n_unique, 1ull); }
}

__global__ void compact_kernel(int n_pairs, int mb, const OutRecord *in, const int *n_rec, const u64 *offs, OutRecord *out) {
  const int pair = blockIdx.x * blockDim.x + threadIdx.x;
  if (pair >= n_pairs) return;
  const int n = n_rec[pair];
  for (int j = 0; j < n; ++j) out[offs[pair] + j] = in[(size_t)pair * mb + j];
}

__global__ void collect_overflow_kernel(Scratch S, int *list, int *count) {
  const int slot = blockIdx.x * blockDim.x + threadIdx.x;
  if (slot >= S.n_slots) return;
  if (S.pmeta[slot].status == ST_OVERFLOW) list[agg_append(count)] = slot_pair(S, slot);
}

#define CTA_NT 128
#define CTA_SORT_SMEM_MAX 4096
#define CTA_MM_SMEM 1024

__device__ inline void cta_sort_keys(u64 *a, int n, u64 *sm, int sm_cap) {
  const int NT = blockDim.x;
  int np2 = 1;
  while (np2 < n) np2 <<= 1;
  const int tid = threadIdx.x;
  if (n <= 1) { __syncthreads(); return; }
  if (np2 <= sm_cap) {
    for (int i = tid; i < np2; i += NT) sm[i] = i < n ? a[i] : ~0ull;
    __syncthreads();
    for (int k = 2; k <= np2; k <<= 1)
      for (int j = k >> 1; j > 0; j >>= 1) {
        for (int p = tid; p < (np2 >> 1); p += NT) {
          const int i = ((p & ~(j - 1)) << 1) | (p & (j - 1)), l = i + j;
          const u64 x = sm[i], y = sm[l];
          const bool up = (i & k) == 0;
          if ((x > y) == up) { sm[i] = y; sm[l] = x; }
        }
        __syncthreads();
      }
    for (int i = tid; i < n; i += NT) a[i] = sm[i];
    __syncthreads();
    return;
  }
  for (int i = n + tid; i < np2; i += NT) a[i] = ~0ull;
  __syncthreads();
  for (int k = 2; k <= np2; k <<= 1) {
    int j = k >> 1;
    for (; j >= sm_cap; j >>= 1) {
      for (int p = tid; p < (np2 >> 1); p += NT) {
        const int i = ((p & ~(j - 1)) << 1) | (p & (j - 1)), l = i + j;
        const u64 x = a[i], y = a[l];
        const bool up = (i & k) == 0;
        if ((x > y) == up) { a[i] = y; a[l] = x; }
      }
      __syncthreads();
    }
    const bool fuse = k <= sm_cap;
    for (int base = 0; base < np2; base += sm_cap) {
      for (int i = tid; i < sm_cap; i += NT) sm[i] = a[base + i];
      __syncthreads();
      const int k_lo = fuse ? 2 : k, k_hi = fuse ? sm_cap : k;
      for (int kk = k_lo; kk <= k_hi; kk <<= 1)
        for (int jj = fuse ? (kk >> 1) : j; jj > 0; jj >>= 1) {
          for (int p = tid; p < (sm_cap >> 1); p += NT) {
            const int i = ((p & ~(jj - 1)) << 1) | (p & (jj - 1)), l = i + jj;
            const u64 x = sm[i], y = sm[l];
            const bool up = ((base + i) & kk) == 0;
            if ((x > y) == up) { sm[i] = y; sm[l] = x; }
          }
          __syncthreads();
        }
      for (int i = tid; i < sm_cap; i += NT) a[base + i] = sm[i];
      __syncthreads();
    }
    if (fuse) k = sm_cap;
  }
}

template <typename T, typename Less>
__device__ inline void cta_sort_pairs(u64 *k_, T *t_, int n, u64 pad_key, T pad_tag, Less less, u64 *smk, T *smt, int sm_cap) {
  const int NT = blockDim.x;
  int np2 = 1;
  while (np2 < n) np2 <<= 1;
  const int tid = threadIdx.x;
  if (n <= 1) { __syncthreads(); return; }
  if (np2 <= sm_cap) {
    for (int i = tid; i < np2; i += NT) { smk[i] = i < n ? k_[i] : pad_key; smt[i] = i < n ? t_[i] : pad_tag; }
    __syncthreads();
    for (int k = 2; k <= np2; k <<= 1)
      for (int j = k >> 1; j > 0; j >>= 1) {
        for (int p = tid; p < (np2 >> 1); p += NT) {
          const int i = ((p & ~(j - 1)) << 1) | (p & (j - 1)), l = i + j;
          const u64 xk = smk[i], yk = smk[l];
          const T xt = smt[i], yt = smt[l];
          const bool up = (i & k) == 0;
          const bool sw = up ? less(yk, yt, xk, xt) : less(xk, xt, yk, yt);
          if (sw) { smk[i] = yk; smt[i] = yt; smk[l] = xk; smt[l] = xt; }
        }
        __syncthreads();
      }
    for (int i = tid; i < n; i += NT) { k_[i] = smk[i]; t_[i] = smt[i]; }
    __syncthreads();
    return;
  }
  for (int i = n + tid; i < np2; i += NT) { k_[i] = pad_key; t_[i] = pad_tag; }
  __syncthreads();
  for (int k = 2; k <= np2; k <<= 1) {
    int j = k >> 1;
    for (; j >= sm_cap; j >>= 1) {
      for (int p = tid; p < (np2 >> 1); p += NT) {
        const int i = ((p & ~(j - 1)) << 1) | (p & (j - 1)), l = i + j;
        const u64 xk = k_[i], yk = k_[l];
        const T xt = t_[i], yt = t_[l];
        const bool up = (i & k) == 0;
        const bool sw = up ? less(yk, yt, xk, xt) : less(xk, xt, yk, yt);
        if (sw) { k_[i] = yk; t_[i] = yt; k_[l] = xk; t_[l] = xt; }
      }
      __syncthreads();
    }
    const bool fuse = k <= sm_cap;
    for (int base = 0; base < np2; base += sm_cap) {
// ... 164 lines not shown
  for (int i = tid; i < nh; i += NT) {
    bool b = i == 0;
    if (!b) {
      const u64 h = sm[i], q = sm[i - 1];
      b = (u32)(h >> 32) != (u32)(q >> 32) || (u32)h > (u32)q + (u32)e;
    }
    flag[i] = b; vld[i] = 0;
  }
  __syncthreads();
  const int C = (nh + NT - 1) / NT;
  const int r0 = tid * C, r1 = min(nh, r0 + C);
  for (int i = r0; i < r1; ++i) {
    if (!flag[i]) continue;
    int out = i, mcount = 1, eq = 1, best_eq = 1;
    u64 prev = sm[i], best = prev;
    int q = i + 1;
    for (; q < nh && !flag[q]; ++q) {
      const u64 h = sm[q];
      if ((u32)mcount >= n_mm && (u32)h > (u32)best + (u32)e) {
        if (mcount >= need) { sm[out] = best; cnt[out] = (u8)best_eq; vld[out] = 1; ++out; }
        mcount = 1; eq = 1; best_eq = 1; best = h;
      } else {
        if (h == best) { ++eq; ++best_eq; }
        else if (h == prev) { ++eq; if (eq > best_eq) { best = prev; best_eq = eq; } }
        else eq = 1;
        ++mcount;
      }
      prev = h;
    }
    if (mcount >= need) { sm[out] = best; cnt[out] = (u8)best_eq; vld[out] = 1; ++out; }
  }
  __syncthreads();
  int mine = 0;
  for (int i = r0; i < r1; ++i) mine += vld[i];
  __shared__ int s_warp[32];
  int total;
  int at = cta_excl_scan(mine, s_warp, &total);
  for (int i = r0; i < r1; ++i)
    if (vld[i]) { if (at < cap) { cpos[at] = sm[i]; ccnt[at] = cnt[i]; } ++at; }
  __syncthreads();
  return total;
}

__global__ void __launch_bounds__(CTA_NT) seed_cta_kernel(DevParams P, DevIndex ix, DevBatch B, Scratch S, Scratch S0, Counters *ctr, int sm_cap) {
  extern __shared__ u64 sm[];
  int *s_off = (int *)(sm + sm_cap);
  u32 *s_c1 = (u32 *)(s_off + S.caps.maxmm + 1), *s_c2 = s_c1 + S.caps.maxmm;
  __shared__ int s_i[8];
  __shared__ unsigned long long s_steps;
  const int sr = blockIdx.x, tid = threadIdx.x;
  const int slot = sr >> 1, mate = sr & 1;
  if (tid == 0) s_i[7] = S.pmeta[slot].status;
  __syncthreads();
  if (s_i[7] != ST_OK || (P.se && mate == 1)) return;
  const int pair = slot_pair(S, slot);
  ReadMeta &rm = S.rmeta[sr];
  const Caps c = S.caps;
  u64 *mmh = S.mm_hash + (size_t)sr * c.maxmm;
  u64 *mmv = S.mm_val + (size_t)sr * c.maxmm;
  u32 *mmp = S.mm_pos + (size_t)sr * c.maxmm;
  const ReadMeta &r0 = S0.rmeta[2 * pair + mate];
  const bool reuse = r0.mm_done == 1 && r0.n_mm <= c.maxmm && r0.len == rm.len;
  if (reuse) {
    if (tid == 0) { rm.n_mm = r0.n_mm; s_i[0] = r0.n_mm; s_steps = 0; s_i[5] = 0; }
  } else {
    const int n0 = cta_minimizers(read_ptr(B, pair, mate), rm.len, P.k, P.w, mmh, mmp, c.maxmm, sm, &s_i[6]);
    if (tid == 0) {
      rm.n_mm = n0;
      s_i[0] = n0;
      s_steps = 0;
      s_i[5] = 0;
    }
  }
  __syncthreads();
  const int n_mm = s_i[0];
  if (n_mm > c.maxmm) { if (tid == 0) atomicExch(&S.pmeta[slot].status, ST_OVERFLOW); return; }
  if (n_mm == 0) return;
  const size_t b0 = mm_base(S0, pair, mate);
  const int ms0 = mm_stride(S0);
  for (int i = tid; i < n_mm; i += CTA_NT) {
    u64 val = 0;
    int steps = 0, kind;
    if (reuse) {
      val = S0.mm_val[b0 + (size_t)i * ms0];
      const u32 pw = S0.mm_pos[b0 + (size_t)i * ms0];
      kind = (int)(pw >> 30);
      mmv[i] = val; mmp[i] = pw;
    } else {
      kind = index_lookup(ix, mmh[i], &val, &steps);
      mmv[i] = val;
      mmp[i] = (mmp[i] & 0x3FFFFFFFu) | ((u32)kind << 30);
      atomicAdd(&s_steps, (unsigned long long)steps);
      if (kind) atomicAdd(&s_i[5], 1);
    }
    u32 c1 = 0, c2 = 0;
    if (kind == 1) { c1 = c2 = 1; }
    else if (kind == 2) { const u32 n = (u32)val; if (n < (u32)P.f0) c1 = n; if (n < (u32)P.f1) c2 = n; }
    s_c1[i] = c1; s_c2[i] = c2;
  }
  __syncthreads();
  if (tid == 0) {
    long long cnt1 = 0;
    for (int i = 0; i < n_mm; ++i) cnt1 += s_c1[i];
    const bool round2 = cnt1 == 0;
    long long tot = 0;
    RepStats st = {0u, 0xFFFFFFFFu, 0};
    for (int i = 0; i < n_mm; ++i) {
      s_off[i] = (int)tot;
      tot += round2 ? s_c2[i] : s_c1[i];
      if ((mmp[i] >> 30) == 2 && (u32)mmv[i] >= (u32)P.f0) rep_update(P.k, P.w, (mmp[i] & 0x3FFFFFFFu) >> 1, st);
      if (tot > 2ll * c.hc) break;
    }
    s_off[n_mm] = (int)(tot > 2ll * c.hc ? 2ll * c.hc + 1 : tot);
    s_i[1] = round2;
    s_i[2] = st.count;
    rm.rep_len = st.len;
    if (!reuse) {
      atomicAdd(&ctr->n_minimizers, (u64)n_mm);
      atomicAdd(&ctr->n_probe_steps, (u64)s_steps);
      atomicAdd(&ctr->n_found, (u64)s_i[5]);
    }
  }
  __syncthreads();
  const int T = s_off[n_mm];
  if (T > 2 * c.hc) { if (tid == 0) atomicExch(&S.pmeta[slot].status, ST_OVERFLOW); return; }
  u64 *hits = S.hits + (size_t)sr * 2 * c.hc;
  for (int j = tid; j < T; j += CTA_NT) {
    int lo = 0, hi = n_mm;
    while (hi - lo > 1) { const int mid = (lo + hi) >> 1; if (s_off[mid] <= j) lo = mid; else hi = mid; }
    const int i = lo;
    const u32 rpos = (mmp[i] & 0x3FFFFFFFu) >> 1, rstrand = mmp[i] & 1u;
    const u64 val = mmv[i];
    const u64 rh = (mmp[i] >> 30) == 1 ? val : __ldg(&ix.occ[(u32)(val >> 32) + (u32)(j - s_off[i])]);
    bool same;
    const u64 cp = hit_to_candidate(P.k, rh, rpos, rstrand, &same);
    hits[j] = cp | (same ? 0ull : (1ull << 63));
  }
  if (tid == 0) { u64 occ_reads = 0; for (int i = 0; i < n_mm; ++i) if ((mmp[i] >> 30) == 2) occ_reads += s_off[i + 1] - s_off[i]; atomicAdd(&ctr->n_occ_reads, occ_reads); }
  __syncthreads();
  cta_sort_keys(hits, T, sm, sm_cap);
  if (tid == 0) {
    int lo = 0, hi = T;
    while (lo < hi) { const int mid = (lo + hi) >> 1; if (hits[mid] >> 63) hi = mid; else lo = mid + 1; }
    s_i[3] = lo;
  }
  __syncthreads();
  const int np = s_i[3], nn = T - np;
  for (int j = np + tid; j < T; j += CTA_NT) hits[j] &= ~(1ull << 63);
  __syncthreads();
  int need = n_mm - s_i[2];
  need = need > 1 ? need : 1;
  need = need > P.min_seeds ? P.min_seeds : need;
  if (s_i[1] && np > 0 && nn > 0) need = P.min_seeds;
  u64 *cp0 = S.cand_pos + (((size_t)sr * 3 + 0) * 2 + 0) * c.cc, *cp1 = cp0 + c.cc;
  u8 *cc0 = S.cand_cnt + (((size_t)sr * 3 + 0) * 2 + 0) * c.cc, *cc1 = cc0 + c.cc;
  u8 *aux = (u8 *)(s_c2 + S.caps.maxmm);
  const int nc0 = cta_cluster_par(P.e, need, (u32)n_mm, hits, np, cp0, cc0, c.cc, sm, sm_cap, aux, &s_i[4]);
  const int nc1 = cta_cluster_par(P.e, need, (u32)n_mm, hits + np, nn, cp1, cc1, c.cc, sm, sm_cap, aux, &s_i[4]);
  if (tid == 0) {
    if (nc0 > c.cc || nc1 > c.cc) atomicExch(&S.pmeta[slot].status, ST_OVERFLOW);
    else {
          rm.n_cand[0] = nc0; rm.n_cand[1] = nc1; rm.n_cand_gen[0] = nc0; rm.n_cand_gen[1] = nc1;
    }
  }
}



template <typename PatF, typename TxtF>
__device__ __forceinline__ int banded_align_dropoff(int e, int L, bool from3, PatF PAT, TxtF TXT, int *end_pos, int *read_len_out) {
  PatPlanes W = {0u, 0u, 0u};
  for (int i = 0; i < 2 * e; ++i) planes_or(W, from3 ? PAT(L + 2 * e - 1 - i) : PAT(i), 1u << i);
  const u32 hi = 1u << (2 * e), band = (hi << 1) - 1u;
  u32 VP = 0, VN = 0, pVP = 0, pVN = 0;
  int err = 0, perr = 0, i = 0, fail_beginning = 0;
  for (; i < L; ++i) {
    planes_or(W, from3 ? PAT(L - 1 - i) : PAT(i + 2 * e), hi);
    u32 X = VN | planes_match(W, from3 ? TXT(L - 1 - i) : TXT(i), band);
    const u32 D0 = ((VP + (X & VP)) ^ VP) | X;
    const u32 HN = VP & D0;
    const u32 HP = VN | ~(VP | D0);
    X = D0 >> 1;
    pVN = VN; pVP = VP;
    VN = X & HP;
    VP = HN | ~(X | HP);
    perr = err;
    err += 1 - (int)(D0 & 1u);
    if (err > 2 * e) { if (i < 4 * e && i < L / 2) fail_beginning = 1; break; }
    planes_shift(W);
  }
  if (i < L) { err = perr; VN = pVN; VP = pVP; }
  const int band_start = i - 1;
  int best = err;
  *read_len_out = i;
  int ep = band_start;
  for (int j = 0; j < 2 * e; ++j) {
    err += (int)((VP >> j) & 1u);
    err -= (int)((VN >> j) & 1u);
    if (err < best || (err == best && j + 1 == e)) { best = err; ep = band_start + 1 + j; }
  }
  if (fail_beginning || (L > 60 && ep + 1 - e - best < 30)) ep = -ep;
  *end_pos = ep;
  return best;
}

struct SplitResult { int nerr, actual, endp, gap, rml; };
template <typename TxtF>
__device__ __forceinline__ SplitResult verify_split_candidate(int e, const u8 *win, TxtF TXT, int L, int s) {
  SplitResult r;
  int endp = L, gap = 0, nerr, rml = 0;
  const int allow_gap = 20 - e;
  const bool from3 = s != 0;
  nerr = banded_align_dropoff(e, L, from3, [&](int i) { return base_code(__ldg(win + i)); }, TXT, &endp, &rml);
  if (endp < 0 && allow_gap > 0) {
    const int b_err = nerr, b_end = -endp, b_rml = rml;
    const int sh = from3 ? 0 : allow_gap;
    nerr = banded_align_dropoff(e, L - allow_gap, from3, [&](int i) { return base_code(__ldg(win + sh + i)); }, [&](int i) { return TXT(sh + i); }, &endp, &rml);
    if (nerr > e || endp < 0) { nerr = b_err; endp = b_end; rml = b_rml; }
    else { gap = allow_gap; endp += gap; rml += gap; }
  }
  if (endp + 1 - e - nerr - gap >= 30) { r.actual = nerr; r.nerr = -(endp - e - nerr - gap); }
  else { r.nerr = e + 1; r.actual = e + 1; }
  r.endp = endp; r.gap = gap; r.rml = rml;
  return r;
}

__global__ void verify_split_kernel(DevParams P, DevRef R, DevBatch B, Scratch S, Counters *ctr) {
  const int sr = blockIdx.x * blockDim.x + threadIdx.x;
  if (sr >= 2 * S.n_slots) return;
  const int slot = sr >> 1, mate = sr & 1;
  if (S.pmeta[slot].status != ST_OK || (P.se && mate == 1)) return;
  const int pair = slot_pair(S, slot);
  ReadMeta &rm = S.rmeta[sr];
  const Caps c = S.caps;
  const u8 *read = read_ptr(B, pair, mate);
  const int L = rm.len, e = P.e;
  Tally t = {e + 1, e + 1, 0, 0};
  auto cless = [](u64 pa, u8 ca, u64 pb, u8 cb) { return ca != cb ? ca > cb : pa < pb; };
  u64 n_verified = 0;
  int nm0 = 0, nm1 = 0;
  prefetch_span(read, L);
  u64 *const cp0 = S.cand_pos + (((size_t)sr * 3 + 0) * 2 + 0) * c.cc, *const cp1 = cp0 + c.cc;
  u8 *const cc0 = S.cand_cnt + (((size_t)sr * 3 + 0) * 2 + 0) * c.cc, *const cc1 = cc0 + c.cc;
  const int nc0 = rm.n_cand[0], nc1 = rm.n_cand[1];
  sort_pairs<u8>(cp0, cc0, nc0, cless);
  sort_pairs<u8>(cp1, cc1, nc1, cless);
  int s = 0, ci = 0;
  u32 threshold = 0;
  for (;;) {
    if (s >= 2) break;
    const int nc = s ? nc1 : nc0;
    const u32 cnt = ci < nc ? (u32)(s ? cc1 : cc0)[ci] : 0u;
    if (ci >= nc || cnt < threshold) { ++s; ci = 0; threshold = 0; continue; }
    const u64 cpos = (s ? cp1 : cp0)[ci];
    ++ci;
    const u32 rid = (u32)(cpos >> 32);
    const u32 pos = s == 0 ? (u32)cpos : (u32)cpos - (u32)L + 1u;
    if (!valid_cand(e, R.len[rid], pos, (u32)L)) continue;
    prefetch_span(R.seq + R.off[rid] + pos - e, L + 2 * e);
    const SplitResult r = verify_split_candidate(e, R.seq + R.off[rid] + pos - e, [&](int i) -> u32 {
      const u32 b = base_code(read[s ? L - 1 - i : i]);
      return s ? (b < 4 ? 3u ^ b : 4u) : b;
    }, L, s);
    ++n_verified;
    if (r.nerr <= e) {
      if (r.nerr < t.min_err) {
        t.second_min_err = t.min_err; t.n_second_best = t.n_best; t.min_err = r.nerr; t.n_best = 1;
        threshold = nc > 50 ? cnt : cnt / 2;
      } else if (r.nerr == t.min_err) t.n_best++;
      else if (r.nerr == t.second_min_err) t.n_second_best++;
      else if (r.nerr < t.second_min_err) { t.n_second_best = 1; t.second_min_err = r.nerr; }
      const int k = s ? nm1 : nm0;
      if (k < c.mc) {
        const size_t mo = ((size_t)sr * 2 + s) * c.mc + k;
        S.map_pos[mo] = s == 0 ? cpos - (u64)e + (u64)r.endp : cpos - (u64)r.gap;
        S.map_err[mo] = (short)r.nerr;
        S.map_split[mo] = ((r.actual & 0xff) << 24) | ((r.gap & 0xff) << 16) | (r.rml & 0xffff);
      }
      if (s) ++nm1; else ++nm0;
    }
  }
  if (nm0 > c.mc || nm1 > c.mc) { S.pmeta[slot].status = ST_OVERFLOW; atomicAdd(&ctr->ovf_reason[6], 1ull); return; }
  rm.n_map[0] = nm0; rm.n_map[1] = nm1;
  rm.min_err = t.min_err; rm.second_min_err = t.second_min_err; rm.n_best = t.n_best; rm.n_second_best = t.n_second_best;
  if (n_verified) agg_add(&ctr->n_verified, n_verified);
}

__global__ void __launch_bounds__(CTA_NT) verify_split_cta_kernel(DevParams P, DevRef R, DevBatch B, Scratch S, Counters *ctr, int sm_cap) {
  extern __shared__ u64 smk[];
  u8 *smt = (u8 *)(smk + sm_cap);
  __shared__ int s_status;
  const int sr = blockIdx.x, tid = threadIdx.x;
  const int slot = sr >> 1, mate = sr & 1;
  if (tid == 0) s_status = S.pmeta[slot].status;
  __syncthreads();
  if (s_status != ST_OK) return;
  const int pair = slot_pair(S, slot);
  ReadMeta &rm = S.rmeta[sr];
  const Caps c = S.caps;
  const u8 *read = read_ptr(B, pair, mate);
  const int L = rm.len, e = P.e;
  auto cless = [](u64 pa, u8 ca, u64 pb, u8 cb) { return ca != cb ? ca > cb : pa < pb; };
  u64 *cp[2], *res[2];
  u8 *cc[2], *vld[2];
  for (int s = 0; s < 2; ++s) {
    cp[s] = S.cand_pos + (((size_t)sr * 3 + 0) * 2 + s) * c.cc; cc[s] = S.cand_cnt + (((size_t)sr * 3 + 0) * 2 + s) * c.cc;
    res[s] = S.cand_pos + (((size_t)sr * 3 + 2) * 2 + s) * c.cc; vld[s] = S.cand_cnt + (((size_t)sr * 3 + 2) * 2 + s) * c.cc;
  }
  const int nc[2] = {rm.n_cand[0], rm.n_cand[1]};
  cta_sort_pairs<u8>(cp[0], cc[0], nc[0], ~0ull, (u8)0, cless, smk, smt, sm_cap);
  cta_sort_pairs<u8>(cp[1], cc[1], nc[1], ~0ull, (u8)0, cless, smk, smt, sm_cap);
  u64 n_ver = 0;
  for (int s = 0; s < 2; ++s)
    for (int i = tid; i < nc[s]; i += CTA_NT) {
      const u64 cpos = cp[s][i];
      const u32 rid = (u32)(cpos >> 32);
      const u32 pos = s == 0 ? (u32)cpos : (u32)cpos - (u32)L + 1u;
      if (!valid_cand(e, R.len[rid], pos, (u32)L)) { vld[s][i] = 0; continue; }
      const SplitResult r = s == 0 ? verify_split_candidate(e, R.seq + R.off[rid] + pos - e, [&](int q) { return base_code(read[q]); }, L, 0)
                                   : verify_split_candidate(e, R.seq + R.off[rid] + pos - e, [&](int q) { return neg_code(read, L, q); }, L, 1);
      vld[s][i] = 1;
      res[s][i] = ((u64)(u32)(r.nerr + 1024) << 48) | ((u64)(r.actual & 0xff) << 40) | ((u64)(r.gap & 0xff) << 32) | ((u64)(r.rml & 0xffff) << 16) | (u64)(r.endp & 0xffff);
      ++n_ver;
    }
  if (n_ver) atomicAdd(&ctr->n_verified, n_ver);
  __syncthreads();
  if (tid != 0) return;
  Tally t = {e + 1, e + 1, 0, 0};
  int nm[2] = {0, 0};
  for (int s = 0; s < 2; ++s) {
    u64 *mp = S.map_pos + ((size_t)sr * 2 + s) * c.mc;
    short *me = S.map_err + ((size_t)sr * 2 + s) * c.mc;
    int *ms = S.map_split + ((size_t)sr * 2 + s) * c.mc;
    u32 threshold = 0;
    for (int ci = 0; ci < nc[s]; ++ci) {
      if (cc[s][ci] < threshold) break;
      if (!vld[s][ci]) continue;
      const u64 w = res[s][ci];
      const int nerr = (int)(w >> 48) - 1024, actual = (int)((w >> 40) & 0xff), gap = (int)((w >> 32) & 0xff), rml = (int)((w >> 16) & 0xffff), endp = (int)(w & 0xffff);
      if (nerr <= e) {
        if (nerr < t.min_err) {
          t.second_min_err = t.min_err; t.n_second_best = t.n_best; t.min_err = nerr; t.n_best = 1;
          threshold = nc[s] > 50 ? (u32)cc[s][ci] : (u32)cc[s][ci] / 2;
        } else if (nerr == t.min_err) t.n_best++;
        else if (nerr == t.second_min_err) t.n_second_best++;
        else if (nerr < t.second_min_err) { t.n_second_best = 1; t.second_min_err = nerr; }
        const u64 cpos = cp[s][ci];
        if (nm[s] < c.mc) {
          mp[nm[s]] = s == 0 ? cpos - (u64)e + (u64)endp : cpos - (u64)gap;
          me[nm[s]] = (short)nerr;
          ms[nm[s]] = ((actual & 0xff) << 24) | ((gap & 0xff) << 16) | (rml & 0xffff);
        }
        ++nm[s];
      }
    }
  }
  if (nm[0] > c.mc || nm[1] > c.mc) { S.pmeta[slot].status = ST_OVERFLOW; return; }
  rm.n_map[0] = nm[0]; rm.n_map[1] = nm[1];
  rm.min_err = t.min_err; rm.second_min_err = t.second_min_err; rm.n_best = t.n_best; rm.n_second_best = t.n_second_best;
}

__global__ void pairing_split_kernel(DevParams P, Scratch S, int *pair_nbest) {
  const int slot = blockIdx.x * blockDim.x + threadIdx.x;
  if (slot >= S.n_slots) return;
  PairMeta &pm = S.pmeta[slot];
  const int pair = slot_pair(S, slot);
  if (pm.status != ST_OK) { if (pm.status == ST_DROP) pair_nbest[pair] = 0; return; }
  const Caps c = S.caps;
  ReadMeta *rm = S.rmeta + 2 * slot;
  if (rm[0].n_map[0] + rm[0].n_map[1] == 0 || rm[1].n_map[0] + rm[1].n_map[1] == 0) { pm.status = ST_DROP; pair_nbest[pair] = 0; return; }
  int cnt[2][2];
  for (int m = 0; m < 2; ++m)
    for (int s = 0; s < 2; ++s) {
      const short *me = S.map_err + ((size_t)(2 * slot + m) * 2 + s) * c.mc;
      const int want = rm[m].min_err;
      int k = 0;
      for (int i = 0; i < rm[m].n_map[s]; ++i) k += me[i] == want;
      cnt[m][s] = k;
    }
  const long long nb = (long long)cnt[0][0] * cnt[1][1] + (long long)cnt[0][1] * cnt[1][0] + (long long)cnt[0][0] * cnt[1][0] + (long long)cnt[0][1] * cnt[1][1];
  const int n_best = nb > 0x7fffffffLL ? 0x7fffffff : (int)nb;
  pm.min_sum = n_best > 0 ? rm[0].min_err + rm[1].min_err : 2 * P.e + 1;
  pm.second_min_sum = 2 * P.e + 1; pm.n_best = n_best; pm.n_second_best = 0;
  pair_nbest[pair] = (n_best > P.drop_rep) ? 0 : n_best;
}

__device__ __forceinline__ int sgn_char(u8 c) { return (int)(signed char)c; }
template <typename ReadC>
__device__ __forceinline__ int adjust_gap_beginning(int strand, const u8 *ref, ReadC RD, int *gap, int read_end, int ref_start, int ref_end) {
  int i, j;
  if (strand == 0) {
    if (*gap <= 0) return ref_start;
    for (i = *gap - 1, j = ref_start - 1; i >= 0 && j >= 0; --i, --j) {
      const int a = sgn_char(RD(i)), b = sgn_char(__ldg(ref + j));
      if (a != b && a != b - 'a' + 'A') break;
    }
    *gap = i + 1;
    return j + 1;
  }
  if (*gap <= 0) return ref_end;
  for (i = read_end + 1, j = ref_end + 1; RD(i) && __ldg(ref + j); ++i, ++j) {
    const int a = sgn_char(RD(i)), b = sgn_char(__ldg(ref + j));
    if (a != b && a != b - 'a' + 'A') break;
  }
  *gap = *gap + i - (read_end + 1);
  return j - 1;
}

__device__ inline u8 mapq_se_split(const MapqTables &T, const DevParams &P, int n_cand_strand, int num_errors, unsigned short aln_len, int read_len,
                                   int max_diff, const ReadMeta &rm) {
  const int coef_len = 50;
  double ident = xdiv((double)(-num_errors), (double)aln_len);
  if (ident > 1) ident = 1;
  int mapq = 0;
  int second = rm.second_min_err;
  if (rm.n_best > 1) {
  } else {
    if (second > num_errors + max_diff) second = num_errors + max_diff;
    double tmp = (int)aln_len < coef_len ? 1.0 : T.inv_log[aln_len];
    tmp = xmul(tmp, xmul(ident, ident));
    mapq = (int)xadd(xmul(xmul(xmul(5 * 6.02, (double)(second - num_errors)), tmp), tmp), 0.499);
  }
  if (rm.n_second_best > 0) mapq -= second_best_penalty(T, rm.n_second_best);
  if (mapq > 60) mapq = 60;
  if (mapq < 0) mapq = 0;
  if (rm.rep_len > 0) {
    double frac = xdiv((double)rm.rep_len, (double)read_len);
    if (rm.rep_len >= (u32)read_len) frac = 0.999;
    mapq = (int)xadd(xmul((double)mapq, rep_scale(ident, frac)), 0.499);
  }
  if ((int)aln_len < read_len - P.e && second != num_errors) {
    if (rm.rep_len >= (u32)aln_len && rm.rep_len < (u32)read_len && (int)aln_len < read_len / 3) mapq = 0;
    const int diff = second - num_errors;
    const u32 num_candidates = (u32)n_cand_strand;
    if (second - num_errors <= P.e * 3 / 4 && num_candidates >= 5) mapq -= (num_candidates / 5 / diff);
    if (mapq < 0) mapq = 0;
    if (rm.n_second_best > 0 && second - num_errors <= P.e * 3 / 4) mapq /= (rm.n_second_best / diff + 1);
  }
  return (u8)mapq;
}

struct OutPairs {
  u32 read_id, rid1, rid2, pos1, pos2;
  u8 strand1, strand2, mapq, is_unique;
};

__global__ void emit_split_kernel(DevParams P, DevRef R, DevBatch B, MapqTables T, Scratch S, const int *pair_sel, OutPairs *out, int *out_n, Counters *ctr) {
  const int slot = blockIdx.x * blockDim.x + threadIdx.x;
  if (slot >= S.n_slots) return;
  PairMeta &pm = S.pmeta[slot];
  const int pair = slot_pair(S, slot);
  if (pm.status == ST_OVERFLOW) return;
  if (pm.status != ST_OK || pm.n_best > P.drop_rep || pm.n_best == 0) { out_n[pair] = 0; return; }
  const Caps c = S.caps;
  const ReadMeta *rm = S.rmeta + 2 * slot;
  const int mb = P.max_best;
  const int to_report = mb < pm.n_best ? mb : pm.n_best;
  const int *sel = pair_sel + (size_t)pair * mb;
  const u8 uniq = (pm.n_best == 1 || rm[0].n_best == 1 || rm[1].n_best == 1) ? 1 : 0;
  const int e = P.e;
  const int L[2] = {rm[0].len, rm[1].len};
  const u8 *rd[2] = {read_ptr(B, pair, 0), read_ptr(B, pair, 1)};
  auto span = [&](int m, int s, u64 dpos, int split_word, u32 *st, u32 *en) {
    const u32 rid = (u32)(dpos >> 32), rp = (u32)dpos;
    const int full = L[m];
    const int split_site = split_word & 0xffff;
    int gap = (split_word >> 16) & 0xff;
    const int actual = (split_word >> 24) & 0xff;
    const int Ls = split_site - gap;
    u32 vws = rp + 1u > (u32)(Ls + e) ? rp + 1u - (u32)Ls - (u32)e : 0u;
    if (rp + (u32)e >= R.len[rid]) vws = R.len[rid] - (u32)e - (u32)Ls;
    const u8 *rseq = R.seq + R.off[rid];
    const u8 *win = rseq + vws;
    const u8 *r = rd[m];
    if (s == 0) {
      int s0 = banded_traceback(e, actual, Ls, [&](int i) { return __ldg(win + i); }, [&](int i) { return r[gap + i]; });
      if (gap > 0) s0 = adjust_gap_beginning(0, rseq, [&](int i) { return i < full ? r[i] : (u8)0; }, &gap, Ls - 1, (int)vws + s0, (int)rp) - (int)vws;
      *st = vws + (u32)s0;
      *en = rp;
      return;
    }
    const int rss = full - split_site;
    const int s0 = e;
    int en0 = (int)(rp - vws + 1u);
    banded_align(e, Ls, [&](int i) { return base_code(__ldg(win + i)); }, [&](int i) { return neg_code(r, full, rss + i); }, &en0);
    en0 += 1;
    if (gap > 0)
      en0 = adjust_gap_beginning(1, rseq, [&](int i) { return (rss + i) < full ? code_char(neg_code(r, full, rss + i)) : (u8)0; }, &gap, Ls - 1, (int)vws + s0,
                                 (int)vws + en0) - (int)vws + 1;
    *st = vws + (u32)s0;
    *en = vws + (u32)en0 - 1u;
  };
  int idx = 0, reported = 0;
  const int DS1[4] = {0, 1, 0, 1}, DS2[4] = {1, 0, 0, 1};
  int ch_dir[CMX_MAX_BEST], ch_i1[CMX_MAX_BEST], ch_i2[CMX_MAX_BEST];
  for (int dir = 0; dir < 4 && reported != to_report; ++dir) {
    const int s1 = DS1[dir], s2 = DS2[dir];
    const short *e1 = S.map_err + ((size_t)(2 * slot + 0) * 2 + s1) * c.mc, *e2 = S.map_err + ((size_t)(2 * slot + 1) * 2 + s2) * c.mc;
    const int want1 = rm[0].min_err, want2 = rm[1].min_err;
    if (rm[0].n_map[s1] == 0 || rm[1].n_map[s2] == 0) continue;
    for (int i1 = 0; i1 < rm[0].n_map[s1] && reported != to_report; ++i1) {
      if (e1[i1] != want1) continue;
      for (int i2 = 0; i2 < rm[1].n_map[s2]; ++i2) {
        if (e2[i2] != want2) continue;
        if (idx == sel[reported]) {
          ch_dir[reported] = dir; ch_i1[reported] = i1; ch_i2[reported] = i2;
          ++reported;
          if (reported == to_report) break;
        }
        ++idx;
      }
    }
  }
  for (int r = 0; r < reported; ++r) {
    const int s1 = DS1[ch_dir[r]], s2 = DS2[ch_dir[r]], i1 = ch_i1[r], i2 = ch_i2[r];
    const u64 *p1 = S.map_pos + ((size_t)(2 * slot + 0) * 2 + s1) * c.mc, *p2 = S.map_pos + ((size_t)(2 * slot + 1) * 2 + s2) * c.mc;
    const int *w1 = S.map_split + ((size_t)(2 * slot + 0) * 2 + s1) * c.mc, *w2 = S.map_split + ((size_t)(2 * slot + 1) * 2 + s2) * c.mc;
    u32 st1, en1, st2, en2;
    span(0, s1, p1[i1], w1[i1], &st1, &en1);
    span(1, s2, p2[i2], w2[i2], &st2, &en2);
    const unsigned short al1 = (unsigned short)(en1 - st1 + 1u), al2 = (unsigned short)(en2 - st2 + 1u);
    u8 q1 = mapq_se_split(T, P, rm[0].n_cand[s1], rm[0].min_err, al1, L[0], 2, rm[0]);
    u8 q2 = mapq_se_split(T, P, rm[1].n_cand[s2], rm[1].min_err, al2, L[1], 2, rm[1]);
    q1 = (u8)xmul((double)q1, 1.2); if (q1 > 60) q1 = 60;
    q2 = (u8)xmul((double)q2, 1.2); if (q2 > 60) q2 = 60;
    const u8 q = q1 < q2 ? q1 : q2;
    int rid1 = (int)(u32)(p1[i1] >> 32), rid2 = (int)(u32)(p2[i2] >> 32);
    int pos1 = (int)(s1 == 0 ? st1 : en1), pos2 = (int)(s2 == 0 ? st2 : en2);
    u8 str1 = s1 == 0 ? 1 : 0, str2 = s2 == 0 ? 1 : 0;
    const bool smaller = rid1 < rid2 || (rid1 == rid2 && pos1 < pos2);
    if (!smaller) { int tt = rid1; rid1 = rid2; rid2 = tt; tt = pos1; pos1 = pos2; pos2 = tt; const u8 ts = str1; str1 = str2; str2 = ts; }
    OutPairs o;
    o.read_id = B.first_read_id + (u32)pair; o.rid1 = (u32)rid1; o.rid2 = (u32)rid2; o.pos1 = (u32)pos1; o.pos2 = (u32)pos2;
    o.strand1 = str1; o.strand2 = str2; o.mapq = q; o.is_unique = uniq;
    out[(size_t)pair * mb + r] = o;
  }
  out_n[pair] = reported;
  pm.n_rec = reported;
  if (reported > 0) { agg_add(&ctr->n_mapped, 1ull); if (pm.n_best == 1) agg_add(&ctr->n_unique, 1ull); }
}


struct DevWhitelist {
  const ulonglong2 *slots;
  u64 mask;
  int shift;
  double num_sample;
  const double *pow_tab;
  int err_threshold;
  double prob_threshold;
  int output_not_in_whitelist;
  int active;
};
__device__ __forceinline__ bool wl_find(const DevWhitelist &W, u64 key, u64 *count) {
  u64 s = (key * 0x9E3779B97F4A7C15ull) >> W.shift;
  for (;;) {
    const ulonglong2 kv = __ldg(&W.slots[s]);
    if (kv.x == CMX_EMPTY_KEY) return false;
    if (kv.x == key) { *count = kv.y; return true; }
    s = (s + 1) & W.mask;
  }
}
__global__ void wl_insert_kernel(const u64 *keys, const u32 *counts, u64 n, ulonglong2 *slots, u64 mask, int shift) {
  const u64 i = (u64)blockIdx.x * blockDim.x + threadIdx.x;
  if (i >= n) return;
  const u64 key = keys[i];
  u64 s = (key * 0x9E3779B97F4A7C15ull) >> shift;
  for (;;) {
    const u64 old = atomicCAS((unsigned long long *)&slots[s].x, (unsigned long long)CMX_EMPTY_KEY, (unsigned long long)key);
    if (old == CMX_EMPTY_KEY || old == key) { slots[s].y = counts[i]; return; }
    s = (s + 1) & mask;
  }
}
__device__ __forceinline__ u64 barcode_seed(const u8 *s, int len) {
  u64 seed = 0;
  for (int i = 0; i < len; ++i) { const u32 b = base_code(s[i]); seed = b < 4 ? (seed << 2) | b : seed << 2; }
  return seed;
}
__global__ void barcode_kernel(DevWhitelist W, const u8 *bc_seq, const u8 *bc_qual, int bc_len, int n, u64 *bc_key, u8 *bc_ok, Counters *ctr) {
  const int i = blockIdx.x * blockDim.x + threadIdx.x;
  if (i >= n) return;
  const u8 *bc = bc_seq + (size_t)i * bc_len, *qual = bc_qual + (size_t)i * bc_len;
  const u64 key = barcode_seed(bc, bc_len);
  if (!W.active) { bc_key[i] = key; bc_ok[i] = 1; return; }
  int n_n = 0, first_n = 0;
  for (int p = bc_len - 1; p >= 0; --p) if (bc[p] == 'N') { if (n_n == 0) first_n = bc_len - 1 - p; ++n_n; }
  u64 cnt;
  bool ok = false;
  u64 out_key = key;
  if (n_n > W.err_threshold) ok = false;
  else if (n_n == 0 && wl_find(W, key, &cnt)) { ok = true; agg_add(&ctr->n_bc_in_whitelist, 1ull); }
  else if (W.err_threshold > 0) {
    double sc[128];
    u8 ci[128], cb[128];
    int nc = 0;
    int i_start = 0, i_end = bc_len, ti_limit = 3;
    if (n_n > 0) { i_start = first_n; i_end = first_n + 1; ti_limit = 4; }
    for (int p = i_start; p < i_end; ++p) {
      const u64 keep = ~(3ull << (2 * p)) & key;
      u64 b1 = (key >> (2 * p)) & 3ull;
      for (int ti = 0; ti < ti_limit; ++ti) {
        b1 = (b1 + 1) & 3ull;
        if (wl_find(W, keep | (b1 << (2 * p)), &cnt)) {
          const double abundance = xdiv((double)cnt, W.num_sample);
          int q = (int)(signed char)qual[bc_len - 1 - p] - 33;
          q = q > 40 ? 40 : q; q = q < 3 ? 3 : q;
          if (nc < 128) { sc[nc] = xmul(W.pow_tab[q], abundance); ci[nc] = (u8)(bc_len - 1 - p); cb[nc] = (u8)b1; }
          ++nc;
        }
      }
    }
    if (nc >= 1) {
      int best = 0;
      bool accept = true;
      if (nc > 1) {
        for (int a = 1; a < nc; ++a) {
          const double s_ = sc[a]; const u8 i_ = ci[a], b_ = cb[a];
          int b = a - 1;
          while (b >= 0 && (sc[b] < s_ || (sc[b] == s_ && (ci[b] < i_ || (ci[b] == i_ && cb[b] < b_))))) { sc[b + 1] = sc[b]; ci[b + 1] = ci[b]; cb[b + 1] = cb[b]; --b; }
          sc[b + 1] = s_; ci[b + 1] = i_; cb[b + 1] = b_;
        }
        double sum = 0;
        for (int a = 0; a < nc; ++a) sum = xadd(sum, sc[a]);
        accept = xdiv(sc[0], sum) > W.prob_threshold;
      }
      if (accept) {
        const int p = bc_len - 1 - (int)ci[best];
        out_key = (key & ~(3ull << (2 * p))) | ((u64)cb[best] << (2 * p));
        ok = true;
        atomicAdd(&ctr->n_bc_corrected, 1ull);
      }
    }
  }
  bc_key[i] = out_key;
  bc_ok[i] = (ok || W.output_not_in_whitelist) ? 1 : 0;
}

__global__ void barcode_gate_kernel(Scratch S, const u8 *bc_ok) {
  const int slot = blockIdx.x * blockDim.x + threadIdx.x;
  if (slot >= S.n_slots) return;
  if (!bc_ok[slot_pair(S, slot)] && S.pmeta[slot].status == ST_OK) S.pmeta[slot].status = ST_DROP;
}

__global__ void compact_bc_kernel(int n_pairs, const int *n_rec, const u64 *offs, const u64 *bc_key, u64 *out) {
  const int pair = blockIdx.x * blockDim.x + threadIdx.x;
  if (pair >= n_pairs) return;
  const int n = n_rec[pair];
  for (int j = 0; j < n; ++j) out[offs[pair] + j] = bc_key[pair];
}
```

chromap_b200/csrc/sam_kernels.cuh:

```cuda
#pragma once
#ifdef __CUDACC__
#include "device_common.cuh"
#endif

#define SAM_MAX_L 160
#define SAM_MAX_E 8
#define SAM_MAX_CIGAR 24

#ifdef __CUDACC__
#define SAM_HD __host__ __device__ __forceinline__
#else
#define SAM_HD inline
#endif

#define SAM_BAND (2 * SAM_MAX_E + 2)
template <typename WinF, typename ReadF>
SAM_HD int sam_band_align(int rlen, int e, int match, int mismatch, int o_del, int e_del, int o_ins, int e_ins, WinF WIN, ReadF RD, unsigned int *cigar, int cap,
                          int *start, int *end) {
  const int NEG = -0x40000000;
  const int w = 2 * e + 1, wlen = rlen + 2 * e;
  const int oe_del = o_del + e_del, oe_ins = o_ins + e_ins;
  int hd[SAM_BAND], ed[SAM_BAND + 1];
  unsigned char dirs[SAM_BAND * SAM_MAX_L];
#pragma unroll
  for (int d = 0; d < SAM_BAND; ++d) { hd[d] = 0; ed[d] = NEG; }
  ed[SAM_BAND] = NEG;
  for (int i = 0; i < rlen; ++i) {
    const unsigned int rc = RD(i);
    unsigned char *row = &dirs[i * (w + 1)];
    int f = NEG;
#pragma unroll
    for (int d = 0; d < SAM_BAND; ++d) {
      if (d > w || i + d >= wlen) break;
      const unsigned int wc = WIN(i + d);
      const int m = hd[d] + ((rc < 4u && wc < 4u) ? (rc == wc ? match : -mismatch) : 0);
      int ev = d < w ? ed[d + 1] : NEG;
      unsigned char dir = m >= ev ? 0 : 1;
      int h = m >= ev ? m : ev;
      if (!(h >= f)) { dir = 2; h = f; }
      hd[d] = h;
      const int td = m - oe_del, ti = m - oe_ins;
      ev -= e_del;
      if (ev > td) dir |= 1 << 2; else ev = td;
      ed[d] = ev;
      f -= e_ins;
      if (f > ti) dir |= 2 << 4; else f = ti;
      row[d] = dir;
    }
  }
  int score = hd[w - 1], best = wlen;
  for (int j = 1; j < w; ++j) if (hd[w - 1 - j] > score) { score = hd[w - 1 - j]; best = wlen - j; }
  *end = best;
  int n = 0, i = rlen - 1, k = best - 1, which = 0;
  bool ovf = false;
  auto push = [&](unsigned int op, unsigned int len) {
    if (n > 0 && (cigar[n - 1] & 0xfu) == op) cigar[n - 1] += len << 4;
    else if (n < cap) cigar[n++] = (len << 4) | op;
    else ovf = true;
  };
  while (i >= 0 && k >= 0) {
    which = dirs[i * (w + 1) + (k - i)] >> (which << 1) & 3;
    if (which == 0) { push(0u, 1u); --i; --k; }
    else if (which == 1) { push(1u, 1u); --i; }
    else { push(2u, 1u); --k; }
  }
  if (i >= 0) push(1u, (unsigned int)(i + 1));
  *start = k + 1;
  if (ovf) return -1;
  for (int a = 0, b = n - 1; a < b; ++a, --b) { const unsigned int t = cigar[a]; cigar[a] = cigar[b]; cigar[b] = t; }
  return n;
}

#if defined(__CUDACC__) || defined(CMX_HOST_EMU)
struct OutSam {
  u32 read_id, rid;
  u32 pos[2], end[2];
  u8 strand[2];
  u8 mapq, is_unique, secondary;
  u8 n_cigar[2];
  u8 overflow;
  u32 cigar[2][SAM_MAX_CIGAR];
};

__device__ __noinline__ bool sam_span(const DevParams &P, const DevRef &R, const u8 *read, int L, int strand, u64 dpos, u32 *st, u32 *en, u32 *cigar,
                                         u8 *n_cigar) {
  const int e = P.e;
  const u32 rid = (u32)(dpos >> 32), rp = (u32)dpos;
  u32 vws = rp + 1u > (u32)(L + e) ? rp + 1u - (u32)L - (u32)e : 0u;
  if (rp + (u32)e >= R.len[rid]) vws = R.len[rid] - (u32)e - (u32)L;
  *st = vws; *en = vws; *n_cigar = 0;
  if (L > SAM_MAX_L || e > SAM_MAX_E) return false;
  const u8 *win = R.seq + R.off[rid] + vws;
  int s0 = 0, e0 = 0, n;
  if (strand == 0)
    n = sam_band_align(L, e, 1, 4, 6, 1, 6, 1, [&](int j) { return base_code(__ldg(win + j)); }, [&](int i) { return base_code(read[i]); }, cigar, SAM_MAX_CIGAR, &s0,
                       &e0);
  else
    n = sam_band_align(L, e, 1, 4, 6, 1, 6, 1, [&](int j) { return base_code(__ldg(win + j)); }, [&](int i) { return neg_code(read, L, i); }, cigar, SAM_MAX_CIGAR, &s0,
                       &e0);
  *st = vws + (u32)s0;
  *en = vws + (u32)e0 - 1u;
  if (n < 0) return false;
  *n_cigar = (u8)n;
  return true;
}

__global__ void emit_sam_kernel(DevParams P, DevRef R, DevBatch B, MapqTables T, Scratch S, const int *pair_sel, OutSam *out, int *out_n, Counters *ctr) {
  const int slot = blockIdx.x * blockDim.x + threadIdx.x;
  if (slot >= S.n_slots) return;
  PairMeta &pm = S.pmeta[slot];
  const int pair = slot_pair(S, slot);
  if (pm.status == ST_OVERFLOW) return;
  if (pm.status != ST_OK || pm.n_best > P.drop_rep || pm.n_best == 0) { out_n[pair] = 0; return; }
  const Caps c = S.caps;
  const ReadMeta *rm = S.rmeta + 2 * slot;
  const int mb = P.max_best;
  const int to_report = mb < pm.n_best ? mb : pm.n_best;
  const int *sel = pair_sel + (size_t)pair * mb;
  const u8 uniq = (pm.n_best == 1 || rm[0].n_best == 1 || rm[1].n_best == 1) ? 1 : 0;
  const int force = pm.sup != 0 ? 0 : -1;
  int idx = 0, reported = 0;
  const int L[2] = {rm[0].len, rm[1].len};
  const u8 *rd[2] = {read_ptr(B, pair, 0), read_ptr(B, pair, 1)};
  for (int dir = 0; dir < 2 && reported != to_report; ++dir) {
    const int s1 = dir, s2 = 1 - dir;
    const u64 *p1 = S.map_pos + ((size_t)(2 * slot + 0) * 2 + s1) * c.mc, *p2 = S.map_pos + ((size_t)(2 * slot + 1) * 2 + s2) * c.mc;
    const short *e1 = S.map_err + ((size_t)(2 * slot + 0) * 2 + s1) * c.mc, *e2 = S.map_err + ((size_t)(2 * slot + 1) * 2 + s2) * c.mc;
    pair_sweep_until(P, s1, (u32)L[0], (u32)L[1], p1, e1, rm[0].n_map[s1], p2, e2, rm[1].n_map[s2], [&](int i1, int j, int sum) -> bool {
      if (sum != pm.min_sum) return false;
      if (idx == sel[reported]) {
        OutSam &o = out[(size_t)pair * mb + reported];
        u32 st1, en1, st2, en2;
        const bool ok1 = sam_span(P, R, rd[0], L[0], s1, p1[i1], &st1, &en1, o.cigar[0], &o.n_cigar[0]);
        const bool ok2 = sam_span(P, R, rd[1], L[1], s2, p2[j], &st2, &en2, o.cigar[1], &o.n_cigar[1]);
        const unsigned short al1 = (unsigned short)(en1 - st1 + 1u), al2 = (unsigned short)(en2 - st2 + 1u);
        o.read_id = B.first_read_id + (u32)pair;
        o.rid = (u32)(p1[i1] >> 32);
        o.pos[0] = st1; o.end[0] = en1; o.pos[1] = st2; o.end[1] = en2;
        o.strand[0] = s1 == 0 ? 1 : 0; o.strand[1] = s2 == 0 ? 1 : 0;
        o.mapq = mapq_pe(T, e1[i1], e2[j], al1, al2, L[0], L[1], force, pm, rm);
        o.is_unique = uniq;
        o.secondary = reported >= 1 ? 1 : 0;
        o.overflow = (ok1 && ok2) ? 0 : 1;
        if (o.overflow) agg_add(&ctr->n_overflow, 1ull);
        ++reported;
      }
      ++idx;
      return reported == to_report;
    });
  }
  out_n[pair] = reported;
  pm.n_rec = reported;
  if (reported > 0) { agg_add(&ctr->n_mapped, 1ull); if (pm.n_best == 1) agg_add(&ctr->n_unique, 1ull); }
}

__global__ void emit_sam_se_kernel(DevParams P, DevRef R, DevBatch B, MapqTables T, Scratch S, const int *pair_sel, OutSam *out, int *out_n, Counters *ctr) {
  const int slot = blockIdx.x * blockDim.x + threadIdx.x;
  if (slot >= S.n_slots) return;
  PairMeta &pm = S.pmeta[slot];
  const int pair = slot_pair(S, slot);
  if (pm.status == ST_OVERFLOW) return;
  if (pm.status != ST_OK || pm.n_best == 0) { out_n[pair] = 0; return; }
  const Caps c = S.caps;
  const ReadMeta &rm = S.rmeta[2 * slot];
  const int mb = P.max_best, e = P.e, L = rm.len;
  const int to_report = mb < rm.n_best ? mb : rm.n_best;
  const int *sel = pair_sel + (size_t)pair * mb;
  const u8 *r = read_ptr(B, pair, 0);
  int idx = 0, reported = 0;
  for (int s = 0; s < 2 && reported != to_report; ++s) {
    const u64 *mp = S.map_pos + ((size_t)(2 * slot) * 2 + s) * c.mc;
    const short *me = S.map_err + ((size_t)(2 * slot) * 2 + s) * c.mc;
    for (int mi = 0; mi < rm.n_map[s]; ++mi) {
      if ((int)me[mi] > rm.min_err) continue;
      if (idx == sel[reported]) {
        OutSam &o = out[(size_t)pair * mb + reported];
        u32 st, en;
        const bool ok = sam_span(P, R, r, L, s, mp[mi], &st, &en, o.cigar[0], &o.n_cigar[0]);
        const unsigned short al = (unsigned short)(en - st + 1u);
        o.read_id = B.first_read_id + (u32)pair;
        o.rid = (u32)(mp[mi] >> 32);
        o.pos[0] = st; o.end[0] = en; o.pos[1] = 0; o.end[1] = 0;
        o.strand[0] = s == 0 ? 1 : 0; o.strand[1] = 0;
        o.mapq = mapq_se(T, (int)me[mi], al, L, e, rm);
        o.is_unique = rm.n_best == 1 ? 1 : 0;
        o.secondary = reported >= 1 ? 1 : 0;
        o.n_cigar[1] = 0;
        o.overflow = ok ? 0 : 1;
        if (o.overflow) agg_add(&ctr->n_overflow, 1ull);
        if (++reported == to_report) break;
      }
      ++idx;
    }
  }
  out_n[pair] = reported;
  pm.n_rec = reported;
  if (reported > 0) { agg_add(&ctr->n_mapped, 1ull); if (rm.n_best == 1) agg_add(&ctr->n_unique, 1ull); }
}

__global__ void compact_words_kernel(int n_pairs, int mb, int rec_words, const u32 *in, const int *n_rec, const u64 *offs, u32 *out) {
  const int p = blockIdx.x * blockDim.x + threadIdx.x;
  if (p >= n_pairs) return;
  const int n = n_rec[p];
  const u32 *src = in + (size_t)p * mb * rec_words;
  u32 *dst = out + (size_t)offs[p] * rec_words;
  for (int i = 0; i < n * rec_words; ++i) dst[i] = src[i];
}
#endif
```

Before: 124.4 million.

## Interleave candidate and mapping scratch arrays across 32 slots for coalesced access

Extends the interleaved scratch layout, already used for minimizers, to the candidate position/count and mapping position/error/split arrays. When the interleave flag is set, consecutive reads in a warp get adjacent elements, so per-thread kernels see coalesced accesses. Strided accessor templates replace raw pointers in the per-thread kernels, while CTA kernels are pinned to the non-interleaved form with il=0. This adds index arithmetic and risks a mismatch wherever a CTA kernel and a thread kernel share the same buffer while the flag is on.

```diff
diff --git a/chromap_b200/csrc/cta_pair_candidates.cuh b/chromap_b200/csrc/cta_pair_candidates.cuh
--- a/chromap_b200/csrc/cta_pair_candidates.cuh
+++ b/chromap_b200/csrc/cta_pair_candidates.cuh
@@ -272,8 +272,8 @@
   PairMeta &pm = S.pmeta[slot];
   if (pm.status != ST_OK) return;
   ReadMeta *rm = S.rmeta + 2 * slot;
-  auto CP = [&](int mate, int set, int strand) { return S.cand_pos + ((((size_t)(2 * slot + mate)) * 3 + set) * 2 + strand) * c.cc; };
-  auto CC = [&](int mate, int set, int strand) { return S.cand_cnt + ((((size_t)(2 * slot + mate)) * 3 + set) * 2 + strand) * c.cc; };
+  auto CP = [&](int mate, int set, int strand) { return S.cand_pos + cand_base(0, c, 2 * slot + mate, set, strand); };
+  auto CC = [&](int mate, int set, int strand) { return S.cand_cnt + cand_base(0, c, 2 * slot + mate, set, strand); };
   if (P.se) {
     const int a1 = rm[0].n_cand[0] + rm[0].n_cand[1];
     __syncthreads();
diff --git a/chromap_b200/csrc/cta_verify_pairing.cuh b/chromap_b200/csrc/cta_verify_pairing.cuh
--- a/chromap_b200/csrc/cta_verify_pairing.cuh
+++ b/chromap_b200/csrc/cta_verify_pairing.cuh
@@ -54,10 +54,10 @@
   const Caps c = S.caps;
   const u8 *read = read_ptr(B, pair, mate);
   const int L = rm.len, e = P.e;
-  u64 *mp[2] = {S.map_pos + ((size_t)sr * 2 + 0) * c.mc, S.map_pos + ((size_t)sr * 2 + 1) * c.mc};
-  short *me[2] = {S.map_err + ((size_t)sr * 2 + 0) * c.mc, S.map_err + ((size_t)sr * 2 + 1) * c.mc};
-  u64 *cp[2] = {S.cand_pos + (((size_t)sr * 3 + 0) * 2 + 0) * c.cc, S.cand_pos + (((size_t)sr * 3 + 0) * 2 + 1) * c.cc};
-  u8 *cc[2] = {S.cand_cnt + (((size_t)sr * 3 + 0) * 2 + 0) * c.cc, S.cand_cnt + (((size_t)sr * 3 + 0) * 2 + 1) * c.cc};
+  u64 *mp[2] = {S.map_pos + map_base(0, c, sr, 0), S.map_pos + map_base(0, c, sr, 1)};
+  short *me[2] = {S.map_err + map_base(0, c, sr, 0), S.map_err + map_base(0, c, sr, 1)};
+  u64 *cp[2] = {S.cand_pos + cand_base(0, c, sr, 0, 0), S.cand_pos + cand_base(0, c, sr, 0, 1)};
+  u8 *cc[2] = {S.cand_cnt + cand_base(0, c, sr, 0, 0), S.cand_cnt + cand_base(0, c, sr, 0, 1)};
   const int nc[2] = {rm.n_cand[0], rm.n_cand[1]};
   if (nc[0] + nc[1] == 1) {
     const int strand = nc[0] == 1 ? 0 : 1;
@@ -229,8 +229,8 @@
   short *me[2][2];
   for (int m = 0; m < 2; ++m)
     for (int s = 0; s < 2; ++s) {
-      mp[m][s] = S.map_pos + ((size_t)(2 * slot + m) * 2 + s) * c.mc;
-      me[m][s] = S.map_err + ((size_t)(2 * slot + m) * 2 + s) * c.mc;
+      mp[m][s] = S.map_pos + map_base(0, c, 2 * slot + m, s);
+      me[m][s] = S.map_err + map_base(0, c, 2 * slot + m, s);
       cta_sort_pairs<short>(mp[m][s], me[m][s], rm[m].n_map[s], ~0ull, (short)32767, mless, smk, smt, sm_cap);
     }
   const int sentinel = 2 * P.e + 1;
@@ -277,8 +277,8 @@
   for (int dir = 0; dir < 2; ++dir) {
     if (base > s_sel[to_report - 1]) break;
     W.s1 = dir;
-    const u64 *p1 = S.map_pos + ((size_t)(2 * slot + 0) * 2 + dir) * c.mc, *p2 = S.map_pos + ((size_t)(2 * slot + 1) * 2 + (1 - dir)) * c.mc;
-    const short *e1 = S.map_err + ((size_t)(2 * slot + 0) * 2 + dir) * c.mc, *e2 = S.map_err + ((size_t)(2 * slot + 1) * 2 + (1 - dir)) * c.mc;
+    const u64 *p1 = S.map_pos + map_base(0, c, 2 * slot, dir), *p2 = S.map_pos + map_base(0, c, 2 * slot + 1, 1 - dir);
+    const short *e1 = S.map_err + map_base(0, c, 2 * slot, dir), *e2 = S.map_err + map_base(0, c, 2 * slot + 1, 1 - dir);
     const int n1 = rm[0].n_map[dir], n2 = rm[1].n_map[1 - dir];
     const int C = (n1 + CTA_NT - 1) / CTA_NT;
     const int r0 = min(n1, tid * C), r1 = min(n1, r0 + C);
@@ -312,7 +312,7 @@
   __syncthreads();
   if (tid < to_report) {
     const int s1 = s_i1[tid] >> 30, i1 = s_i1[tid] & 0x3FFFFFFF, j = s_j[tid];
-    const size_t b1 = ((size_t)(2 * slot + 0) * 2 + s1) * c.mc + i1, b2 = ((size_t)(2 * slot + 1) * 2 + (1 - s1)) * c.mc + j;
+    const size_t b1 = map_base(0, c, 2 * slot, s1) + i1, b2 = map_base(0, c, 2 * slot + 1, 1 - s1) + j;
     out[(size_t)pair * mb + tid] = pe_record(P, R, B, T, pm, rm, pair, s1, S.map_pos[b1], S.map_err[b1], S.map_pos[b2], S.map_err[b2]);
   }
   if (tid != 0) return;
diff --git a/chromap_b200/csrc/device_common.cuh b/chromap_b200/csrc/device_common.cuh
--- a/chromap_b200/csrc/device_common.cuh
+++ b/chromap_b200/csrc/device_common.cuh
@@ -89,11 +89,11 @@
 #define SCRATCH_ARRAYS 11
 inline size_t scratch_layout(const Caps &c, size_t slots, bool interleaved, size_t *off, size_t *size = nullptr) {
   const size_t R = 2 * slots;
-  const size_t Rm = interleaved ? 2 * ((slots + 31) / 32 * 32) : R;
+  const size_t Ri = interleaved ? 2 * ((slots + 31) / 32 * 32) : R;
   const size_t sz[SCRATCH_ARRAYS] = {R * sizeof(ReadMeta), slots * sizeof(PairMeta),
                                      interleaved ? 0 : R * c.maxmm * 8,
-                                     Rm * c.maxmm * 8, Rm * c.maxmm * 4, R * 2 * (size_t)c.hc * 8, R * 6 * (size_t)c.cc * 8, R * 6 * (size_t)c.cc,
-                                     R * 2 * (size_t)c.mc * 8, R * 2 * (size_t)c.mc * 2, R * 2 * (size_t)c.mc * 4};
+                                     Ri * c.maxmm * 8, Ri * c.maxmm * 4, R * 2 * (size_t)c.hc * 8, Ri * 6 * (size_t)c.cc * 8, Ri * 6 * (size_t)c.cc,
+                                     Ri * 2 * (size_t)c.mc * 8, Ri * 2 * (size_t)c.mc * 2, Ri * 2 * (size_t)c.mc * 4};
   size_t end = 0;
   for (int i = 0; i < SCRATCH_ARRAYS; ++i) {
     off[i] = end;
@@ -107,6 +107,42 @@
   S.mm_hash = (u64 *)a[2]; S.mm_val = (u64 *)a[3]; S.mm_pos = (u32 *)a[4];
   S.hits = (u64 *)a[5]; S.cand_pos = (u64 *)a[6]; S.cand_cnt = (u8 *)a[7];
   S.map_pos = (u64 *)a[8]; S.map_err = (short *)a[9]; S.map_split = (int *)a[10];
+}
+
+template <typename T>
+struct Strided {
+  T *base;
+  int stride;
+  __device__ __forceinline__ T &operator[](int i) const { return base[i * stride]; }
+};
+
+__device__ __forceinline__ size_t il_read(int il, int sr) { return il ? (size_t)((sr >> 6) * 2 + (sr & 1)) : (size_t)sr; }
+__device__ __forceinline__ size_t il_place(int il, int sr, size_t e) { return il ? e * 32 + ((sr >> 1) & 31) : e; }
+__device__ __forceinline__ int il_stride(int il) { return il ? 32 : 1; }
+__device__ __forceinline__ size_t mm_base(const Scratch &S, int slot, int mate) {
+  return S.mm_il ? ((size_t)((slot >> 5) * 2 + mate) * S.caps.maxmm) * 32 + (slot & 31) : (size_t)(2 * slot + mate) * S.caps.maxmm;
+}
+__device__ __forceinline__ int mm_stride(const Scratch &S) { return il_stride(S.mm_il); }
+__device__ __forceinline__ size_t cand_base(int il, const Caps &c, int sr, int set, int strand) {
+  return il_place(il, sr, ((il_read(il, sr) * 3 + set) * 2 + strand) * c.cc);
+}
+__device__ __forceinline__ size_t map_base(int il, const Caps &c, int sr, int strand) {
+  return il_place(il, sr, (il_read(il, sr) * 2 + strand) * c.mc);
+}
+__device__ __forceinline__ Strided<u64> cand_pos_of(const Scratch &S, int sr, int set, int strand) {
+  return {S.cand_pos + cand_base(S.mm_il, S.caps, sr, set, strand), il_stride(S.mm_il)};
+}
+__device__ __forceinline__ Strided<u8> cand_cnt_of(const Scratch &S, int sr, int set, int strand) {
+  return {S.cand_cnt + cand_base(S.mm_il, S.caps, sr, set, strand), il_stride(S.mm_il)};
+}
+__device__ __forceinline__ Strided<u64> map_pos_of(const Scratch &S, int sr, int strand) {
+  return {S.map_pos + map_base(S.mm_il, S.caps, sr, strand), il_stride(S.mm_il)};
+}
+__device__ __forceinline__ Strided<short> map_err_of(const Scratch &S, int sr, int strand) {
+  return {S.map_err + map_base(S.mm_il, S.caps, sr, strand), il_stride(S.mm_il)};
+}
+__device__ __forceinline__ Strided<int> map_split_of(const Scratch &S, int sr, int strand) {
+  return {S.map_split + map_base(S.mm_il, S.caps, sr, strand), il_stride(S.mm_il)};
 }
 
 __device__ __forceinline__ int slot_pair(const Scratch &S, int slot) { return S.pair_list ? S.pair_list[slot] : slot; }
@@ -183,12 +219,6 @@
   *same = sm;
   return ((ref_hit >> 33) << 32) | start;
 }
-
-struct StridedU64 {
-  u64 *base;
-  int stride;
-  __device__ __forceinline__ u64 &operator[](int i) const { return base[i * stride]; }
-};
 
 template <typename A>
 __device__ inline void sort_u64(A a, int n) {
@@ -230,8 +260,8 @@
   }
 }
 
-template <typename T, typename Less>
-__device__ inline void sort_pairs(u64 *k, T *t, int n, Less less) {
+template <typename T, typename K, typename V, typename Less>
+__device__ inline void sort_pairs(K k, V t, int n, Less less) {
   if (n <= 24) {
     for (int i = 1; i < n; ++i) {
       const u64 kv = k[i];
diff --git a/chromap_b200/csrc/minimizers.cuh b/chromap_b200/csrc/minimizers.cuh
--- a/chromap_b200/csrc/minimizers.cuh
+++ b/chromap_b200/csrc/minimizers.cuh
@@ -242,8 +242,3 @@
   if (k == 17 && w == 7 && len < (1 << 18)) minimizer_scan_packed<17, 7>(SEQ, len, EMIT);
   else minimizer_scan<0, 0>(SEQ, len, k, w, EMIT);
 }
-
-__device__ __forceinline__ size_t mm_base(const Scratch &S, int slot, int mate) {
-  return S.mm_il ? ((size_t)((slot >> 5) * 2 + mate) * S.caps.maxmm) * 32 + (slot & 31) : (size_t)(2 * slot + mate) * S.caps.maxmm;
-}
-__device__ __forceinline__ int mm_stride(const Scratch &S) { return S.mm_il ? 32 : 1; }
diff --git a/chromap_b200/csrc/pipeline_kernels.cuh b/chromap_b200/csrc/pipeline_kernels.cuh
--- a/chromap_b200/csrc/pipeline_kernels.cuh
+++ b/chromap_b200/csrc/pipeline_kernels.cuh
@@ -115,8 +115,8 @@
   ++st.count;
 }
 
-template <typename A>
-__device__ inline int cluster_hits(int e, int need, u32 n_mm, A hits, int nh, u64 *cpos, u8 *ccnt, int cap) {
+template <typename A, typename PA, typename CA>
+__device__ inline int cluster_hits(int e, int need, u32 n_mm, A hits, int nh, PA cpos, CA ccnt, int cap) {
   if (nh == 0) return 0;
   int n = 0, mcount = 1, eq = 1, best_eq = 1;
   u64 prev = hits[0], best = hits[0];
@@ -176,8 +176,8 @@
   if (total > c.hc) { S.pmeta[slot].status = ST_OVERFLOW; atomicAdd(&ctr->ovf_reason[2], 1ull); return; }
   if (total > rows) { list[agg_append(list_count)] = sr; return; }
   const u32 max_freq = round2 ? (u32)P.f1 : (u32)P.f0;
-  const StridedU64 hp = {sh_hits + threadIdx.x, CLUSTER_NT};
-  const StridedU64 hn = {sh_hits + (size_t)(rows - 1) * CLUSTER_NT + threadIdx.x, -CLUSTER_NT};
+  const Strided<u64> hp = {sh_hits + threadIdx.x, CLUSTER_NT};
+  const Strided<u64> hn = {sh_hits + (size_t)(rows - 1) * CLUSTER_NT + threadIdx.x, -CLUSTER_NT};
   int np = 0, nn = 0;
   u32 occ_reads = 0;
   for (int i = 0; i < n_mm; ++i) {
@@ -209,17 +209,16 @@
   need = need > 1 ? need : 1;
   need = need > P.min_seeds ? P.min_seeds : need;
   if (round2 && np > 0 && nn > 0) need = P.min_seeds;
-  u64 *cp0 = S.cand_pos + (((size_t)sr * 3 + 0) * 2 + 0) * c.cc, *cp1 = cp0 + c.cc;
-  u8 *cc0 = S.cand_cnt + (((size_t)sr * 3 + 0) * 2 + 0) * c.cc, *cc1 = cc0 + c.cc;
-  const int nc0 = cluster_hits(P.e, need, (u32)n_mm, hp, np, cp0, cc0, c.cc);
-  const int nc1 = cluster_hits(P.e, need, (u32)n_mm, hn, nn, cp1, cc1, c.cc);
+  const int nc0 = cluster_hits(P.e, need, (u32)n_mm, hp, np, cand_pos_of(S, sr, 0, 0), cand_cnt_of(S, sr, 0, 0), c.cc);
+  const int nc1 = cluster_hits(P.e, need, (u32)n_mm, hn, nn, cand_pos_of(S, sr, 0, 1), cand_cnt_of(S, sr, 0, 1), c.cc);
   if (nc0 > c.cc || nc1 > c.cc) { S.pmeta[slot].status = ST_OVERFLOW; atomicAdd(&ctr->ovf_reason[3], 1ull); return; }
   rm.n_cand[0] = nc0; rm.n_cand[1] = nc1;
   rm.n_cand_gen[0] = nc0; rm.n_cand_gen[1] = nc1;
 }
 
+template <typename PA, typename CA>
 __device__ inline int rescue_hits(const DevParams &P, const DevIndex &ix, int strand, u32 range, int n_mm, const u64 *mmv,
-                                  const u32 *mmp, int ms, const u64 *mate_pos, const u8 *mate_cnt, int n_mate, u32 *rep_len,
+                                  const u32 *mmp, int ms, PA mate_pos, CA mate_cnt, int n_mate, u32 *rep_len,
                                   u64 *hits, int cap, int *nh_out) {
   int max_cnt = 0, n_best = 0;
   for (int i = 0; i < n_mate; ++i) {
@@ -279,7 +278,8 @@
   return max_cnt;
 }
 
-__device__ inline int merge_cands(int e, u64 *p1, u8 *c1, int n1, const u64 *p2, const u8 *c2, int n2, u64 *po, u8 *co, int cap) {
+template <typename PA, typename CA>
+__device__ inline int merge_cands(int e, PA p1, CA c1, int n1, PA p2, CA c2, int n2, PA po, CA co, int cap) {
   if (n1 == 0) {
     for (int i = 0; i < n2 && i < cap; ++i) { p1[i] = p2[i]; c1[i] = c2[i]; }
     return n2;
@@ -301,8 +301,8 @@
   return n;
 }
 
-__device__ inline void pe_filter_dir(u32 dist, const u64 *p1, const u8 *c1, int n1, const u64 *p2, const u8 *c2, int n2,
-                                     u64 *f1p, u8 *f1c, int *nf1, u64 *f2p, u8 *f2c, int *nf2) {
+template <typename IP, typename IC, typename OP, typename OC>
+__device__ inline void pe_filter_dir(u32 dist, IP p1, IC c1, int n1, IP p2, IC c2, int n2, OP f1p, OC f1c, int *nf1, OP f2p, OC f2c, int *nf2) {
   int i1 = 0, i2 = 0, prev_end = 0, a = 0, b = 0;
   int un1 = 0, un2 = 0, max1 = 6, max2 = 6;
   while (i1 < n1 && i2 < n2) {
@@ -340,8 +340,8 @@
   if (pm.status != ST_OK) return;
   const Caps c = S.caps;
   ReadMeta *rm = S.rmeta + 2 * slot;
-  auto CP = [&](int mate, int set, int strand) { return S.cand_pos + ((((size_t)(2 * slot + mate)) * 3 + set) * 2 + strand) * c.cc; };
-  auto CC = [&](int mate, int set, int strand) { return S.cand_cnt + ((((size_t)(2 * slot + mate)) * 3 + set) * 2 + strand) * c.cc; };
+  auto CP = [&](int mate, int set, int strand) { return cand_pos_of(S, 2 * slot + mate, set, strand); };
+  auto CC = [&](int mate, int set, int strand) { return cand_cnt_of(S, 2 * slot + mate, set, strand); };
   if (P.se) {
     if (mode != 0) return;
     const int a1 = rm[0].n_cand[0] + rm[0].n_cand[1];
@@ -366,8 +366,8 @@
     if (small) {
 #pragma unroll
       for (int q = 0; q < 4; ++q) {
-        const u64 *src = CP(q >> 1, 0, q & 1);
-        const u8 *srcc = CC(q >> 1, 0, q & 1);
+        const Strided<u64> src = CP(q >> 1, 0, q & 1);
+        const Strided<u8> srcc = CC(q >> 1, 0, q & 1);
         for (int i = 0; i < nq[q]; ++i) { lp[q][i] = src[i]; lc[q][i] = srcc[i]; }
       }
     }
@@ -377,8 +377,8 @@
       const u32 n_mm = rm[mate].n_mm;
       bool a = true;
       for (int s = 0; s < 2 && a; ++s) {
-        const u8 *cc = small ? lc[mate * 2 + s] : CC(mate, 0, s);
-        for (int i = 0; i < nq[mate * 2 + s]; ++i) if (cc[i] >= n_mm / 2) { a = false; break; }
+        const Strided<u8> cc = CC(mate, 0, s);
+        for (int i = 0; i < nq[mate * 2 + s]; ++i) if ((small ? lc[mate * 2 + s][i] : cc[i]) >= n_mm / 2) { a = false; break; }
       }
       aug[mate] = a;
       if (a && nq[(1 - mate) * 2] + nq[(1 - mate) * 2 + 1] > 0) need = true;
@@ -422,7 +422,7 @@
       const u32 n_mm = me.n_mm;
       bool a = true;
       for (int s = 0; s < 2 && a; ++s) {
-        const u8 *cc = CC(mate, 0, s);
+        const Strided<u8> cc = CC(mate, 0, s);
         for (int i = 0; i < me.n_cand[s]; ++i) if (cc[i] >= n_mm / 2) { a = false; break; }
       }
       if (!a) continue;
@@ -470,8 +470,8 @@
     for (int mate = 0; mate < 2; ++mate)
       for (int s = 0; s < 2; ++s) {
         const int n = rm[mate].n_cand[s];
-        u64 *src = CP(mate, 0, s), *dst = CP(mate, 1, s);
-        u8 *srcc = CC(mate, 0, s), *dstc = CC(mate, 1, s);
+        const Strided<u64> src = CP(mate, 0, s), dst = CP(mate, 1, s);
+        const Strided<u8> srcc = CC(mate, 0, s), dstc = CC(mate, 1, s);
         for (int i = 0; i < n; ++i) { dst[i] = src[i]; dstc[i] = srcc[i]; }
         nbuf[mate][s] = n;
       }
@@ -560,25 +560,25 @@
   const u8 *read = read_ptr(B, pair, mate);
   const int L = rm.len, e = P.e;
   Tally t = {e + 1, e + 1, 0, 0};
-  u64 *mp[2] = {S.map_pos + ((size_t)sr * 2 + 0) * c.mc, S.map_pos + ((size_t)sr * 2 + 1) * c.mc};
-  short *me[2] = {S.map_err + ((size_t)sr * 2 + 0) * c.mc, S.map_err + ((size_t)sr * 2 + 1) * c.mc};
+  auto MP = [&](int s) { return map_pos_of(S, sr, s); };
+  auto ME = [&](int s) { return map_err_of(S, sr, s); };
   int nm[2] = {0, 0};
-  u64 *cp[2] = {S.cand_pos + (((size_t)sr * 3 + 0) * 2 + 0) * c.cc, S.cand_pos + (((size_t)sr * 3 + 0) * 2 + 1) * c.cc};
-  u8 *cc[2] = {S.cand_cnt + (((size_t)sr * 3 + 0) * 2 + 0) * c.cc, S.cand_cnt + (((size_t)sr * 3 + 0) * 2 + 1) * c.cc};
+  auto CP = [&](int s) { return cand_pos_of(S, sr, 0, s); };
+  auto CC = [&](int s) { return cand_cnt_of(S, sr, 0, s); };
   const int nc[2] = {rm.n_cand[0], rm.n_cand[1]};
   bool done = false;
   if (mode == 0 && nc[0] + nc[1] == 1) {
     int n_all = 0, idx = 0, strand = 0;
-    for (int i = 0; i < nc[0]; ++i) if (cc[0][i] == rm.n_mm) { idx = i; ++n_all; }
-    for (int i = 0; i < nc[1]; ++i) if (cc[1][i] == rm.n_mm) { idx = i; strand = 1; ++n_all; }
+    for (int i = 0; i < nc[0]; ++i) if (CC(0)[i] == rm.n_mm) { idx = i; ++n_all; }
+    for (int i = 0; i < nc[1]; ++i) if (CC(1)[i] == rm.n_mm) { idx = i; strand = 1; ++n_all; }
     if (n_all == 1) {
       t.min_err = 0; t.n_best = 1; t.n_second_best = 0;
-      const u64 cpos = cp[strand][idx];
+      const u64 cpos = CP(strand)[idx];
       const u32 rid = (u32)(cpos >> 32);
       const u32 pos = strand == 0 ? (u32)cpos : (u32)cpos - (u32)L + 1u;
       if (valid_cand(e, R.len[rid], pos, (u32)L)) {
-        mp[strand][0] = strand == 0 ? cpos + (u64)L - 1 : cpos;
-        me[strand][0] = 0;
+        MP(strand)[0] = strand == 0 ? cpos + (u64)L - 1 : cpos;
+        ME(strand)[0] = 0;
         nm[strand] = 1;
         done = true;
       }
@@ -588,8 +588,8 @@
   if (mode == 0 && !done && nc[0] + nc[1] > 0) { list[agg_append(list_count)] = sr; return; }
   if (!done && nc[0] + nc[1] > 0) {
     auto cless = [](u64 pa, u8 ca, u64 pb, u8 cb) { return ca != cb ? ca > cb : pa < pb; };
-    sort_pairs<u8>(cp[0], cc[0], nc[0], cless);
-    sort_pairs<u8>(cp[1], cc[1], nc[1], cless);
+    sort_pairs<u8>(CP(0), CC(0), nc[0], cless);
+    sort_pairs<u8>(CP(1), CC(1), nc[1], cless);
     extern __shared__ u8 v_codes[];
     const int NTB = blockDim.x;
     u8 *c_fwd = v_codes + threadIdx.x, *c_neg = v_codes + (size_t)c.maxmm * NTB + threadIdx.x;
@@ -611,15 +611,15 @@
         if (err > e) return true;
         tally(t, err);
         if (nm[s] < c.mc) {
-          mp[s][nm[s]] = s == 0 ? cpos - (u64)e + (u64)endp : cpos - (u64)L + 1 - (u64)e + (u64)endp;
-          me[s][nm[s]] = (short)err;
+          MP(s)[nm[s]] = s == 0 ? cpos - (u64)e + (u64)endp : cpos - (u64)L + 1 - (u64)e + (u64)endp;
+          ME(s)[nm[s]] = (short)err;
         }
         ++nm[s];
         return false;
       };
       if (nc[s] < P.lanes) {
         for (int i = 0; i < nc[s]; ++i) {
-          const u64 cpos = cp[s][i];
+          const u64 cpos = CP(s)[i];
           const u32 pos = s == 0 ? (u32)cpos : (u32)cpos - (u32)L + 1u;
           if (!valid_cand(e, R.len[(u32)(cpos >> 32)], pos, (u32)L)) continue;
           run_one(cpos);
@@ -631,16 +631,16 @@
       u32 threshold = 0;
       int ci = 0;
       while (ci < nc[s]) {
-        if (cc[s][ci] < threshold) break;
-        const u64 cpos = cp[s][ci];
+        if (CC(s)[ci] < threshold) break;
+        const u64 cpos = CP(s)[ci];
         const u32 pos = s == 0 ? (u32)cpos : (u32)cpos - (u32)L + 1u;
         if (!valid_cand(e, R.len[(u32)(cpos >> 32)], pos, (u32)L)) { ++ci; continue; }
         group[ng++] = ci; ++ci;
         if (ng < P.lanes) continue;
-        for (int g = 0; g < ng; ++g) if (run_one(cp[s][group[g]])) threshold = cc[s][group[g]];
+        for (int g = 0; g < ng; ++g) if (run_one(CP(s)[group[g]])) threshold = CC(s)[group[g]];
         ng = 0;
       }
-      for (int g = 0; g < ng; ++g) run_one(cp[s][group[g]]);
+      for (int g = 0; g < ng; ++g) run_one(CP(s)[group[g]]);
     }
   }
   if (nm[0] > c.mc || nm[1] > c.mc) { S.pmeta[slot].status = ST_OVERFLOW; atomicAdd(&ctr->ovf_reason[6], 1ull); return; }
@@ -649,9 +649,8 @@
   if (n_verified) agg_add(&ctr->n_verified, n_verified);
 }
 
-template <typename Visit>
-__device__ __forceinline__ void pair_sweep(const DevParams &P, int s1, u32 L1, u32 L2, const u64 *p1, const short *e1, int n1,
-                                           const u64 *p2, const short *e2, int n2, Visit VISIT) {
+template <typename PA, typename EA, typename Visit>
+__device__ __forceinline__ void pair_sweep(const DevParams &P, int s1, u32 L1, u32 L2, PA p1, EA e1, int n1, PA p2, EA e2, int n2, Visit VISIT) {
   int i1 = 0, i2 = 0;
   const u64 ins = (u64)P.max_insert, ovl = (u64)(u32)P.min_read_len;
   while (i1 < n1 && i2 < n2) {
@@ -667,9 +666,8 @@
     }
   }
 }
-template <typename Visit>
-__device__ __forceinline__ void pair_sweep_until(const DevParams &P, int s1, u32 L1, u32 L2, const u64 *p1, const short *e1, int n1,
-                                                 const u64 *p2, const short *e2, int n2, Visit VISIT) {
+template <typename PA, typename EA, typename Visit>
+__device__ __forceinline__ void pair_sweep_until(const DevParams &P, int s1, u32 L1, u32 L2, PA p1, EA e1, int n1, PA p2, EA e2, int n2, Visit VISIT) {
   int i1 = 0, i2 = 0;
   const u64 ins = (u64)P.max_insert, ovl = (u64)(u32)P.min_read_len;
   while (i1 < n1 && i2 < n2) {
@@ -692,7 +690,6 @@
   PairMeta &pm = S.pmeta[slot];
   const int pair = slot_pair(S, slot);
   if (pm.status != ST_OK) { if (pm.status == ST_DROP) pair_nbest[pair] = 0; return; }
-  const Caps c = S.caps;
   ReadMeta *rm = S.rmeta + 2 * slot;
   if (P.se) {
     if (rm[0].n_map[0] + rm[0].n_map[1] == 0) { pm.status = ST_DROP; pair_nbest[pair] = 0; return; }
@@ -702,14 +699,10 @@
   }
   if (rm[0].n_map[0] + rm[0].n_map[1] == 0 || rm[1].n_map[0] + rm[1].n_map[1] == 0) { pm.status = ST_DROP; pair_nbest[pair] = 0; return; }
   auto mless = [](u64 pa, short ea, u64 pb, short eb) { return pa != pb ? pa < pb : ea < eb; };
-  u64 *mp[2][2];
-  short *me[2][2];
+  auto MP = [&](int m, int s) { return map_pos_of(S, 2 * slot + m, s); };
+  auto ME = [&](int m, int s) { return map_err_of(S, 2 * slot + m, s); };
   for (int m = 0; m < 2; ++m)
-    for (int s = 0; s < 2; ++s) {
-      mp[m][s] = S.map_pos + ((size_t)(2 * slot + m) * 2 + s) * c.mc;
-      me[m][s] = S.map_err + ((size_t)(2 * slot + m) * 2 + s) * c.mc;
-      sort_pairs<short>(mp[m][s], me[m][s], rm[m].n_map[s], mless);
-    }
+    for (int s = 0; s < 2; ++s) sort_pairs<short>(MP(m, s), ME(m, s), rm[m].n_map[s], mless);
   int min_sum = 2 * P.e + 1, second = 2 * P.e + 1, n_best = 0, n_second = 0;
   auto visit = [&](int, int, int sum) {
     if (sum < min_sum) { second = min_sum; n_second = n_best; min_sum = sum; n_best = 1; }
@@ -717,8 +710,8 @@
     else if (sum == second) n_second++;
     else if (sum < second) { second = sum; n_second = 1; }
   };
-  pair_sweep(P, 0, (u32)rm[0].len, (u32)rm[1].len, mp[0][0], me[0][0], rm[0].n_map[0], mp[1][1], me[1][1], rm[1].n_map[1], visit);
-  pair_sweep(P, 1, (u32)rm[0].len, (u32)rm[1].len, mp[0][1], me[0][1], rm[0].n_map[1], mp[1][0], me[1][0], rm[1].n_map[0], visit);
+  pair_sweep(P, 0, (u32)rm[0].len, (u32)rm[1].len, MP(0, 0), ME(0, 0), rm[0].n_map[0], MP(1, 1), ME(1, 1), rm[1].n_map[1], visit);
+  pair_sweep(P, 1, (u32)rm[0].len, (u32)rm[1].len, MP(0, 1), ME(0, 1), rm[0].n_map[1], MP(1, 0), ME(1, 0), rm[1].n_map[0], visit);
   pm.min_sum = min_sum; pm.second_min_sum = second; pm.n_best = n_best; pm.n_second_best = n_second;
   pair_nbest[pair] = (n_best > P.drop_rep) ? 0 : n_best;
 }
@@ -1013,7 +1006,6 @@
   const int sl = in_range ? slot : 0;
   PairMeta &pm = S.pmeta[sl];
   const int pair = slot_pair(S, sl);
-  const Caps c = S.caps;
   const ReadMeta *rm = S.rmeta + 2 * sl;
   const int mb = P.max_best, e = P.e;
   int reported = 0;
@@ -1026,9 +1018,8 @@
     int idx = 0;
     for (int dir = 0; dir < 2 && reported != to_report; ++dir) {
       const int s1 = dir, s2 = 1 - dir;
-      const u64 *p1 = S.map_pos + ((size_t)(2 * slot + 0) * 2 + s1) * c.mc, *p2 = S.map_pos + ((size_t)(2 * slot + 1) * 2 + s2) * c.mc;
-      const short *e1 = S.map_err + ((size_t)(2 * slot + 0) * 2 + s1) * c.mc, *e2 = S.map_err + ((size_t)(2 * slot + 1) * 2 + s2) * c.mc;
-      pair_sweep_until(P, s1, (u32)rm[0].len, (u32)rm[1].len, p1, e1, rm[0].n_map[s1], p2, e2, rm[1].n_map[s2], [&](int i1, int j, int sum) -> bool {
+      pair_sweep_until(P, s1, (u32)rm[0].len, (u32)rm[1].len, map_pos_of(S, 2 * slot, s1), map_err_of(S, 2 * slot, s1), rm[0].n_map[s1], map_pos_of(S, 2 * slot + 1, s2),
+                       map_err_of(S, 2 * slot + 1, s2), rm[1].n_map[s2], [&](int i1, int j, int sum) -> bool {
         if (sum != pm.min_sum) return false;
         if (idx == sel[reported]) { ch_i1[reported] = i1 | (dir << 30); ch_j[reported] = j; ++reported; }
         ++idx;
@@ -1049,8 +1040,9 @@
     int s0[2] = {e, e};
     if (have) {
       s1 = ch_i1[r] >> 30;
-      const size_t b1 = ((size_t)(2 * slot + 0) * 2 + s1) * c.mc + (ch_i1[r] & 0x3FFFFFFF), b2 = ((size_t)(2 * slot + 1) * 2 + (1 - s1)) * c.mc + ch_j[r];
-      dpos[0] = S.map_pos[b1]; derr[0] = S.map_err[b1]; dpos[1] = S.map_pos[b2]; derr[1] = S.map_err[b2];
+      const int i1 = ch_i1[r] & 0x3FFFFFFF, j = ch_j[r];
+      dpos[0] = map_pos_of(S, 2 * slot, s1)[i1]; derr[0] = map_err_of(S, 2 * slot, s1)[i1];
+      dpos[1] = map_pos_of(S, 2 * slot + 1, 1 - s1)[j]; derr[1] = map_err_of(S, 2 * slot + 1, 1 - s1)[j];
 #pragma unroll
       for (int m = 0; m < 2; ++m) {
         const u32 rid = (u32)(dpos[m] >> 32), rp = (u32)dpos[m];
@@ -1126,10 +1118,9 @@
   if (t >= *dp_count) return;
   const int4 q = dp_list[t];
   const int slot = q.x, r = q.y, s1 = q.z >> 30, i1 = q.z & 0x3FFFFFFF, j = q.w;
-  const Caps c = S.caps;
-  const size_t b1 = ((size_t)(2 * slot + 0) * 2 + s1) * c.mc + i1, b2 = ((size_t)(2 * slot + 1) * 2 + (1 - s1)) * c.mc + j;
   const int pair = slot_pair(S, slot);
-  out[(size_t)pair * P.max_best + r] = pe_record(P, R, B, T, S.pmeta[slot], S.rmeta + 2 * slot, pair, s1, S.map_pos[b1], S.map_err[b1], S.map_pos[b2], S.map_err[b2]);
+  out[(size_t)pair * P.max_best + r] = pe_record(P, R, B, T, S.pmeta[slot], S.rmeta + 2 * slot, pair, s1, map_pos_of(S, 2 * slot, s1)[i1], map_err_of(S, 2 * slot, s1)[i1],
+                                                 map_pos_of(S, 2 * slot + 1, 1 - s1)[j], map_err_of(S, 2 * slot + 1, 1 - s1)[j]);
 }
 
 __global__ void emit_se_kernel(DevParams P, DevRef R, DevBatch B, MapqTables T, Scratch S, const int *pair_sel, OutRecord *out, int *out_n,
@@ -1140,7 +1131,6 @@
   const int pair = slot_pair(S, slot);
   if (pm.status == ST_OVERFLOW) return;
   if (pm.status != ST_OK || pm.n_best == 0) { out_n[pair] = 0; return; }
-  const Caps c = S.caps;
   const ReadMeta &rm = S.rmeta[2 * slot];
   const int mb = P.max_best, e = P.e, L = rm.len;
   const int to_report = mb < rm.n_best ? mb : rm.n_best;
@@ -1148,8 +1138,8 @@
   const u8 *r = read_ptr(B, pair, 0);
   int idx = 0, reported = 0;
   for (int s = 0; s < 2 && reported != to_report; ++s) {
-    const u64 *mp = S.map_pos + ((size_t)(2 * slot) * 2 + s) * c.mc;
-    const short *me = S.map_err + ((size_t)(2 * slot) * 2 + s) * c.mc;
+    const Strided<u64> mp = map_pos_of(S, 2 * slot, s);
+    const Strided<short> me = map_err_of(S, 2 * slot, s);
     for (int mi = 0; mi < rm.n_map[s]; ++mi) {
       if ((int)me[mi] > rm.min_err) continue;
       if (idx == sel[reported]) {
@@ -1620,8 +1610,8 @@
   need = need > 1 ? need : 1;
   need = need > P.min_seeds ? P.min_seeds : need;
   if (s_i[1] && np > 0 && nn > 0) need = P.min_seeds;
-  u64 *cp0 = S.cand_pos + (((size_t)sr * 3 + 0) * 2 + 0) * c.cc, *cp1 = cp0 + c.cc;
-  u8 *cc0 = S.cand_cnt + (((size_t)sr * 3 + 0) * 2 + 0) * c.cc, *cc1 = cc0 + c.cc;
+  u64 *cp0 = S.cand_pos + cand_base(0, c, sr, 0, 0), *cp1 = cp0 + c.cc;
+  u8 *cc0 = S.cand_cnt + cand_base(0, c, sr, 0, 0), *cc1 = cc0 + c.cc;
   u8 *aux = (u8 *)(s_c2 + S.caps.maxmm);
   const int nc0 = cta_cluster_par(P.e, need, (u32)n_mm, hits, np, cp0, cc0, c.cc, sm, sm_cap, aux, &s_i[4]);
   const int nc1 = cta_cluster_par(P.e, need, (u32)n_mm, hits + np, nn, cp1, cc1, c.cc, sm, sm_cap, aux, &s_i[4]);
@@ -1708,19 +1698,19 @@
   u64 n_verified = 0;
   int nm0 = 0, nm1 = 0;
   prefetch_span(read, L);
-  u64 *const cp0 = S.cand_pos + (((size_t)sr * 3 + 0) * 2 + 0) * c.cc, *const cp1 = cp0 + c.cc;
-  u8 *const cc0 = S.cand_cnt + (((size_t)sr * 3 + 0) * 2 + 0) * c.cc, *const cc1 = cc0 + c.cc;
+  auto CP = [&](int s) { return cand_pos_of(S, sr, 0, s); };
+  auto CC = [&](int s) { return cand_cnt_of(S, sr, 0, s); };
   const int nc0 = rm.n_cand[0], nc1 = rm.n_cand[1];
-  sort_pairs<u8>(cp0, cc0, nc0, cless);
-  sort_pairs<u8>(cp1, cc1, nc1, cless);
+  sort_pairs<u8>(CP(0), CC(0), nc0, cless);
+  sort_pairs<u8>(CP(1), CC(1), nc1, cless);
   int s = 0, ci = 0;
   u32 threshold = 0;
   for (;;) {
     if (s >= 2) break;
     const int nc = s ? nc1 : nc0;
-    const u32 cnt = ci < nc ? (u32)(s ? cc1 : cc0)[ci] : 0u;
+    const u32 cnt = ci < nc ? (u32)CC(s)[ci] : 0u;
     if (ci >= nc || cnt < threshold) { ++s; ci = 0; threshold = 0; continue; }
-    const u64 cpos = (s ? cp1 : cp0)[ci];
+    const u64 cpos = CP(s)[ci];
     ++ci;
     const u32 rid = (u32)(cpos >> 32);
     const u32 pos = s == 0 ? (u32)cpos : (u32)cpos - (u32)L + 1u;
@@ -1740,10 +1730,9 @@
       else if (r.nerr < t.second_min_err) { t.n_second_best = 1; t.second_min_err = r.nerr; }
       const int k = s ? nm1 : nm0;
       if (k < c.mc) {
-        const size_t mo = ((size_t)sr * 2 + s) * c.mc + k;
-        S.map_pos[mo] = s == 0 ? cpos - (u64)e + (u64)r.endp : cpos - (u64)r.gap;
-        S.map_err[mo] = (short)r.nerr;
-        S.map_split[mo] = ((r.actual & 0xff) << 24) | ((r.gap & 0xff) << 16) | (r.rml & 0xffff);
+        map_pos_of(S, sr, s)[k] = s == 0 ? cpos - (u64)e + (u64)r.endp : cpos - (u64)r.gap;
+        map_err_of(S, sr, s)[k] = (short)r.nerr;
+        map_split_of(S, sr, s)[k] = ((r.actual & 0xff) << 24) | ((r.gap & 0xff) << 16) | (r.rml & 0xffff);
       }
       if (s) ++nm1; else ++nm0;
     }
@@ -1772,8 +1761,8 @@
   u64 *cp[2], *res[2];
   u8 *cc[2], *vld[2];
   for (int s = 0; s < 2; ++s) {
-    cp[s] = S.cand_pos + (((size_t)sr * 3 + 0) * 2 + s) * c.cc; cc[s] = S.cand_cnt + (((size_t)sr * 3 + 0) * 2 + s) * c.cc;
-    res[s] = S.cand_pos + (((size_t)sr * 3 + 2) * 2 + s) * c.cc; vld[s] = S.cand_cnt + (((size_t)sr * 3 + 2) * 2 + s) * c.cc;
+    cp[s] = S.cand_pos + cand_base(0, c, sr, 0, s); cc[s] = S.cand_cnt + cand_base(0, c, sr, 0, s);
+    res[s] = S.cand_pos + cand_base(0, c, sr, 2, s); vld[s] = S.cand_cnt + cand_base(0, c, sr, 2, s);
   }
   const int nc[2] = {rm.n_cand[0], rm.n_cand[1]};
   cta_sort_pairs<u8>(cp[0], cc[0], nc[0], ~0ull, (u8)0, cless, smk, smt, sm_cap);
@@ -1797,9 +1786,9 @@
   Tally t = {e + 1, e + 1, 0, 0};
   int nm[2] = {0, 0};
   for (int s = 0; s < 2; ++s) {
-    u64 *mp = S.map_pos + ((size_t)sr * 2 + s) * c.mc;
-    short *me = S.map_err + ((size_t)sr * 2 + s) * c.mc;
-    int *ms = S.map_split + ((size_t)sr * 2 + s) * c.mc;
+    u64 *mp = S.map_pos + map_base(0, c, sr, s);
+    short *me = S.map_err + map_base(0, c, sr, s);
+    int *ms = S.map_split + map_base(0, c, sr, s);
     u32 threshold = 0;
     for (int ci = 0; ci < nc[s]; ++ci) {
       if (cc[s][ci] < threshold) break;
@@ -1834,13 +1823,12 @@
   PairMeta &pm = S.pmeta[slot];
   const int pair = slot_pair(S, slot);
   if (pm.status != ST_OK) { if (pm.status == ST_DROP) pair_nbest[pair] = 0; return; }
-  const Caps c = S.caps;
   ReadMeta *rm = S.rmeta + 2 * slot;
   if (rm[0].n_map[0] + rm[0].n_map[1] == 0 || rm[1].n_map[0] + rm[1].n_map[1] == 0) { pm.status = ST_DROP; pair_nbest[pair] = 0; return; }
   int cnt[2][2];
   for (int m = 0; m < 2; ++m)
     for (int s = 0; s < 2; ++s) {
-      const short *me = S.map_err + ((size_t)(2 * slot + m) * 2 + s) * c.mc;
+      const Strided<short> me = map_err_of(S, 2 * slot + m, s);
       const int want = rm[m].min_err;
       int k = 0;
       for (int i = 0; i < rm[m].n_map[s]; ++i) k += me[i] == want;
@@ -1920,7 +1908,6 @@
   const int pair = slot_pair(S, slot);
   if (pm.status == ST_OVERFLOW) return;
   if (pm.status != ST_OK || pm.n_best > P.drop_rep || pm.n_best == 0) { out_n[pair] = 0; return; }
-  const Caps c = S.caps;
   const ReadMeta *rm = S.rmeta + 2 * slot;
   const int mb = P.max_best;
   const int to_report = mb < pm.n_best ? mb : pm.n_best;
@@ -1964,7 +1951,7 @@
   int ch_dir[CMX_MAX_BEST], ch_i1[CMX_MAX_BEST], ch_i2[CMX_MAX_BEST];
   for (int dir = 0; dir < 4 && reported != to_report; ++dir) {
     const int s1 = DS1[dir], s2 = DS2[dir];
-    const short *e1 = S.map_err + ((size_t)(2 * slot + 0) * 2 + s1) * c.mc, *e2 = S.map_err + ((size_t)(2 * slot + 1) * 2 + s2) * c.mc;
+    const Strided<short> e1 = map_err_of(S, 2 * slot, s1), e2 = map_err_of(S, 2 * slot + 1, s2);
     const int want1 = rm[0].min_err, want2 = rm[1].min_err;
     if (rm[0].n_map[s1] == 0 || rm[1].n_map[s2] == 0) continue;
     for (int i1 = 0; i1 < rm[0].n_map[s1] && reported != to_report; ++i1) {
@@ -1982,8 +1969,8 @@
   }
   for (int r = 0; r < reported; ++r) {
     const int s1 = DS1[ch_dir[r]], s2 = DS2[ch_dir[r]], i1 = ch_i1[r], i2 = ch_i2[r];
-    const u64 *p1 = S.map_pos + ((size_t)(2 * slot + 0) * 2 + s1) * c.mc, *p2 = S.map_pos + ((size_t)(2 * slot + 1) * 2 + s2) * c.mc;
-    const int *w1 = S.map_split + ((size_t)(2 * slot + 0) * 2 + s1) * c.mc, *w2 = S.map_split + ((size_t)(2 * slot + 1) * 2 + s2) * c.mc;
+    const Strided<u64> p1 = map_pos_of(S, 2 * slot, s1), p2 = map_pos_of(S, 2 * slot + 1, s2);
+    const Strided<int> w1 = map_split_of(S, 2 * slot, s1), w2 = map_split_of(S, 2 * slot + 1, s2);
     u32 st1, en1, st2, en2;
     span(0, s1, p1[i1], w1[i1], &st1, &en1);
     span(1, s2, p2[i2], w2[i2], &st2, &en2);
diff --git a/chromap_b200/csrc/sam_kernels.cuh b/chromap_b200/csrc/sam_kernels.cuh
--- a/chromap_b200/csrc/sam_kernels.cuh
+++ b/chromap_b200/csrc/sam_kernels.cuh
@@ -112,7 +112,6 @@
   const int pair = slot_pair(S, slot);
   if (pm.status == ST_OVERFLOW) return;
   if (pm.status != ST_OK || pm.n_best > P.drop_rep || pm.n_best == 0) { out_n[pair] = 0; return; }
-  const Caps c = S.caps;
   const ReadMeta *rm = S.rmeta + 2 * slot;
   const int mb = P.max_best;
   const int to_report = mb < pm.n_best ? mb : pm.n_best;
@@ -124,8 +123,8 @@
   const u8 *rd[2] = {read_ptr(B, pair, 0), read_ptr(B, pair, 1)};
   for (int dir = 0; dir < 2 && reported != to_report; ++dir) {
     const int s1 = dir, s2 = 1 - dir;
-    const u64 *p1 = S.map_pos + ((size_t)(2 * slot + 0) * 2 + s1) * c.mc, *p2 = S.map_pos + ((size_t)(2 * slot + 1) * 2 + s2) * c.mc;
-    const short *e1 = S.map_err + ((size_t)(2 * slot + 0) * 2 + s1) * c.mc, *e2 = S.map_err + ((size_t)(2 * slot + 1) * 2 + s2) * c.mc;
+    const Strided<u64> p1 = map_pos_of(S, 2 * slot, s1), p2 = map_pos_of(S, 2 * slot + 1, s2);
+    const Strided<short> e1 = map_err_of(S, 2 * slot, s1), e2 = map_err_of(S, 2 * slot + 1, s2);
     pair_sweep_until(P, s1, (u32)L[0], (u32)L[1], p1, e1, rm[0].n_map[s1], p2, e2, rm[1].n_map[s2], [&](int i1, int j, int sum) -> bool {
       if (sum != pm.min_sum) return false;
       if (idx == sel[reported]) {
@@ -161,7 +160,6 @@
   const int pair = slot_pair(S, slot);
   if (pm.status == ST_OVERFLOW) return;
   if (pm.status != ST_OK || pm.n_best == 0) { out_n[pair] = 0; return; }
-  const Caps c = S.caps;
   const ReadMeta &rm = S.rmeta[2 * slot];
   const int mb = P.max_best, e = P.e, L = rm.len;
   const int to_report = mb < rm.n_best ? mb : rm.n_best;
@@ -169,8 +167,8 @@
   const u8 *r = read_ptr(B, pair, 0);
   int idx = 0, reported = 0;
   for (int s = 0; s < 2 && reported != to_report; ++s) {
-    const u64 *mp = S.map_pos + ((size_t)(2 * slot) * 2 + s) * c.mc;
-    const short *me = S.map_err + ((size_t)(2 * slot) * 2 + s) * c.mc;
+    const Strided<u64> mp = map_pos_of(S, 2 * slot, s);
+    const Strided<short> me = map_err_of(S, 2 * slot, s);
     for (int mi = 0; mi < rm.n_map[s]; ++mi) {
       if ((int)me[mi] > rm.min_err) continue;
       if (idx == sel[reported]) {
```

Measured after the change: 144.6 million (median of 6 runs). +16.2%, better.
